# abiswas-odu/Disco

Measured on AMD Instinct MI355X. Metric: overlaps/sec (BuildGraph stage), 150 bp reads, higher is better.
Workload: dtype u64; 1 GPU; 50000000 x 150 bp synthetic reads, 30x of 50 x 5000000 bp uniform-random contigs, both strands, error-free, min-overlap 40 (k=39), transitive reduction on, seed 42; reads=50000000, read_len=150, min_overlap=40, parallelism=1 GPU, e_pre=903537181, e_out=45314794, n_contained=4685156, cap_bind_sites=0, asymmetric_pairs=0, probes=5550000000, kmer_hits=2220071992

## Files before the change

### disco_amd/build.py

```python
from __future__ import annotations

import os
import shutil
import subprocess

HERE = os.path.dirname(os.path.abspath(__file__))
ROOT = os.path.dirname(HERE)
LIB = os.path.join(HERE, "libdisco_hip.so")
BUILDG = os.path.join(HERE, "bin", "buildG")

HIP_SOURCES = [os.path.join(HERE, "csrc", "disco_hip.hip")]
HIP_DEPS = HIP_SOURCES + [os.path.join(HERE, "csrc", f) for f in sorted(f for f in os.listdir(os.path.join(HERE, "csrc")) if f.endswith(".h"))] + [
    os.path.join(ROOT, "include", "disco_hip.h"), os.path.join(ROOT, "include", "disco_hip_test.h"), os.path.join(ROOT, "include", "disco_hip_inspect.h")]
HOST_SOURCES = [os.path.join(HERE, "host", f) for f in ("buildg_main.cpp", "fastx.cpp", "writer.cpp", "parsimple.cpp")]


def _hipcc() -> str:
    for cand in (shutil.which("hipcc"), "/opt/rocm/bin/hipcc"):
        if cand and os.path.exists(cand):
            return cand
    raise RuntimeError("hipcc not found: the HIP extension cannot be built")


def _stale(target: str, deps) -> bool:
    if not os.path.exists(target):
        return True
    t = os.path.getmtime(target)
    return any(os.path.exists(d) and os.path.getmtime(d) > t for d in deps)


def vgpr_spills(remarks: str) -> dict:
    out, name = {}, None
    for line in remarks.splitlines():
        if "Function Name:" in line:
            name = line.split("Function Name:")[1].split("[")[0].strip()
        elif "VGPRs Spill:" in line and name:
            n = int(line.split("VGPRs Spill:")[1].split("[")[0])
            if n:
                out[name] = n
    return out


def build_lib(force: bool = False, verbose: bool = False) -> str:
    if force or _stale(LIB, HIP_DEPS):
        tmp = LIB + ".tmp"
        cmd = [_hipcc(), "--offload-arch=gfx950", "-O3", "-std=c++17", "-fPIC", "-shared", "-pthread", "-Rpass-analysis=kernel-resource-usage",
               "-o", tmp] + HIP_SOURCES + ["-L/opt/rocm/lib", "-lrccl", "-lrocprofiler-sdk-roctx", "-Wl,-rpath,/opt/rocm/lib"]
        if verbose:
            print(" ".join(cmd))
        r = subprocess.run(cmd, stdout=subprocess.PIPE, stderr=subprocess.PIPE, text=True)
        if r.returncode != 0:
            raise RuntimeError("hipcc failed:\n" + "\n".join(l for l in r.stderr.splitlines() if "-Rpass-analysis" not in l)[-4000:])
        spills = vgpr_spills(r.stderr)
        if spills and not os.environ.get("DISCO_ALLOW_SPILLS"):
            os.unlink(tmp)
            raise RuntimeError(f"kernels spill vector registers (cross-lane reads would return garbage): {spills}")
        os.replace(tmp, LIB)
    return LIB


def build_host(force: bool = False, verbose: bool = False) -> str:
    srcs = [s for s in HOST_SOURCES if os.path.exists(s)]
    if not srcs:
        return ""
    deps = srcs + [os.path.join(HERE, "host", f) for f in os.listdir(os.path.join(HERE, "host")) if f.endswith(".h")] + [LIB]
    if force or _stale(BUILDG, deps):
        os.makedirs(os.path.dirname(BUILDG), exist_ok=True)
        cmd = ["g++", "-O2", "-std=c++17", "-fopenmp", "-Wall", "-I", os.path.join(ROOT, "include"), "-o", BUILDG] + srcs + [
            "-L", HERE, "-ldisco_hip", "-lz", "-Wl,-rpath,$ORIGIN/..", "-Wl,-rpath," + HERE]
        if verbose:
            print(" ".join(cmd))
        subprocess.check_call(cmd)
    dump = os.path.join(HERE, "bin", "fastx_dump")
    dsrc = [os.path.join(HERE, "host", "fastx_dump.cpp"), os.path.join(HERE, "host", "fastx.cpp")]
    if force or _stale(dump, dsrc + [os.path.join(HERE, "host", "fastx.h")]):
        cmd = ["g++", "-O2", "-std=c++17", "-fopenmp", "-Wall", "-o", dump] + dsrc + ["-lz"]
        if verbose:
            print(" ".join(cmd))
        subprocess.check_call(cmd)
    ps = os.path.join(HERE, "bin", "parsimplify")
    psrc = [os.path.join(HERE, "host", f) for f in ("parsimplify_main.cpp", "parsimple.cpp", "fastx.cpp", "writer.cpp")]
    if force or _stale(ps, psrc + [os.path.join(HERE, "host", f) for f in ("parsimple.h", "writer.h", "fastx.h")]):
        cmd = ["g++", "-O2", "-std=c++17", "-fopenmp", "-Wall", "-I", os.path.join(ROOT, "include"), "-o", ps] + psrc + ["-lz"]
        if verbose:
            print(" ".join(cmd))
        subprocess.check_call(cmd)
    gen = os.path.join(HERE, "bin", "readgen")
    gsrc = [os.path.join(HERE, "host", "readgen_main.cpp"), os.path.join(HERE, "csrc", "readgen.h")]
    if force or _stale(gen, gsrc):
        cmd = ["g++", "-O2", "-std=c++17", "-Wall", "-o", gen, gsrc[0]]
        if verbose:
            print(" ".join(cmd))
        subprocess.check_call(cmd)
    chk = os.path.join(HERE, "bin", "inflate_check")
    csrc = [os.path.join(HERE, "host", "inflate_check.cpp"), os.path.join(HERE, "csrc", "disco_inflate.h")]
    if force or _stale(chk, csrc):
        cmd = ["g++", "-O2", "-std=c++17", "-Wall", "-o", chk, csrc[0]]
        if verbose:
            print(" ".join(cmd))
        subprocess.check_call(cmd)
    return BUILDG


def build_all(force: bool = False, verbose: bool = False):
    build_lib(force, verbose)
    build_host(force, verbose)


if __name__ == "__main__":
    build_all(force=True, verbose=True)
```

### disco_amd/buildgraph.py

```python
from __future__ import annotations

import ctypes as C
import os

import numpy as np

_HERE = os.path.dirname(os.path.abspath(__file__))
_LIBPATH = os.environ.get("DISCO_LIB") or os.path.join(_HERE, "libdisco_hip.so")
_lib = None


class DiscoError(RuntimeError):
    pass


class Params(C.Structure):
    _fields_ = [("min_overlap", C.c_uint32), ("max_edges_per_kmer", C.c_uint32), ("flags", C.c_uint32), ("max_substitutions", C.c_uint32)]


class GenSpecABI(C.Structure):
    _fields_ = [("seed", C.c_uint64), ("n_reads", C.c_uint64), ("contig_len", C.c_uint64), ("n_contigs", C.c_uint32),
                ("len_min", C.c_uint32), ("len_max", C.c_uint32), ("skew", C.c_uint32)]


# ... 47 lines not shown
    ("disco_fetch_contained_grouped", C.c_int64, [_P, _P, C.c_uint64]),
    ("disco_fetch_edges", C.c_int64, [_P, _P, C.c_uint64]),
    ("disco_fetch_edge_substitutions", C.c_int64, [_P, _P, C.c_uint64]),
    ("disco_get_counters", C.c_int, [_P, C.POINTER(Counters)]),
    ("disco_phase_ms", C.c_int, [_P, C.POINTER(C.c_float), C.c_int]),
    ("disco_memcpy_d2d", C.c_int, [_P, _P, _P, C.c_uint64]),
    ("disco_fetch_edge_files", C.c_int64, [_P, C.c_uint32, _P, C.c_uint64]),
    ("disco_partition_edges", C.c_int64, [_P, _P, C.c_uint64, C.c_uint64, C.c_uint32, _P]),
    ("disco_format_edges", C.c_int64, [_P, C.c_uint32, _P, _P, _P]),
    ("disco_fetch_edge_text", C.c_int, [_P, _P, C.c_uint64]),
    ("disco_write_edge_text", C.c_int, [_P, _P, C.c_uint32, C.c_uint32]),
    ("disco_start_contained_rows", C.c_int, [_P, C.c_int]),
    ("disco_contract_chains", C.c_int, [_P, C.c_uint32, C.POINTER(C.c_uint64), C.POINTER(C.c_uint64)]),
    ("disco_contract_chains_of", C.c_int, [_P, _P, C.c_uint64, C.c_uint32, C.POINTER(C.c_uint64), C.POINTER(C.c_uint64)]),
    ("disco_fetch_chains", C.c_int, [_P, _P, _P, _P]),
    ("disco_set_query_order", C.c_int, [_P, _P]),
    ("disco_get_query_order", C.c_int, [_P, C.POINTER(_P)]),
    ("disco_probe_run_words", C.c_int, [_P]),
    ("disco_measure_hbm", C.c_int, [_P, C.c_uint64, C.c_int, C.POINTER(C.c_double)]),
    ("disco_measure_gather", C.c_int, [_P, C.c_uint64, C.c_int, C.POINTER(C.c_double)]),
    ("disco_comm_unique_id", C.c_int, [_P, C.c_size_t]),
    ("disco_comm_init", C.c_int, [_P, _P, C.c_int, C.c_int]),
    ("disco_comm_init_local", C.c_int, [C.POINTER(_P), C.c_int]),
    ("disco_comm_rank", C.c_int, [_P]),
    ("disco_comm_world", C.c_int, [_P]),
    ("disco_comm_kind", C.c_char_p, [_P]),
    ("disco_dist_range", C.c_int, [_P, C.c_uint64, C.POINTER(C.c_uint64), C.POINTER(C.c_uint64)]),
    ("disco_dist_upload_reads", C.c_int, [_P, _P, C.c_uint32, _P, C.c_uint64]),
    ("disco_dist_generate_reads", C.c_int, [_P, C.POINTER(GenSpecABI)]),
    ("disco_dist_run_graph", C.c_int, [_P, C.c_uint32]),
    ("disco_dist_get_info", C.c_int, [_P, _P]),
    ("disco_ingest_fasta", C.c_int, [_P, C.POINTER(C.c_char_p), C.c_int, C.c_uint32, _P, _P]),
    ("disco_ingest_fetch", C.c_int, [_P, _P, _P]),
    ("disco_inflate_bgzf", C.c_int64, [_P, _P, C.c_uint64, _P, C.c_uint64]),
    ("disco_dist_ingest_fasta", C.c_int, [_P, C.POINTER(C.c_char_p), C.c_int, C.c_uint32, _P, _P]),
    ("disco_dist_ingest_fetch", C.c_int, [_P, _P, _P]),
    ("disco_inflate_bgzf_window", C.c_int64, [_P, _P, C.c_uint64, C.c_uint64, C.c_uint64, _P]),
    ("disco_format_contained", C.c_int64, [_P, C.c_uint32, _P, _P]),
    ("disco_fetch_contained_text", C.c_int, [_P, _P, C.c_uint64]),
    ("disco_write_contained_text", C.c_int, [_P, _P, C.c_uint32, C.c_uint32]),
]

ABI_VERSION = 2
FLAG_TWO_PASS_VERIFY = 1
XCHG = ("reads", "index_records", "index_shards", "contain", "row_requests", "row_data", "push", "adjacency", "twins", "queries", "hits", "keys", "reads_dealt", "contain_keys")
UNIQUE_ID_BYTES = 128
DIST_GATHER_READS = 1
DIST_KEEP_INDEX_PARTITIONED = 2


CHAIN_EDGE_DTYPE = np.dtype([("a", "<u8"), ("b", "<u8"), ("offset", "<u8"), ("orient", "<u4"), ("n_links", "<u4"), ("first_link", "<u8")])
CHAIN_LINK_DTYPE = np.dtype([("to", "<u4"), ("offset", "<u4"), ("orient", "<u4")])


class IngestFile(C.Structure):
    _fields_ = [("first_index", C.c_uint64), ("last_index", C.c_uint64), ("good", C.c_uint64), ("bad", C.c_uint64)]


class IngestInfo(C.Structure):
    _fields_ = [("n_reads", C.c_uint64), ("total_records", C.c_uint64), ("too_long", C.c_uint64), ("stride_words", C.c_uint32), ("shortest", C.c_uint32),
                ("longest", C.c_uint32), ("read_s", C.c_float), ("device_s", C.c_float)]


class DistIngestInfo(C.Structure):
    _fields_ = [("n_reads", C.c_uint64), ("total_records", C.c_uint64), ("too_long", C.c_uint64), ("stride_words", C.c_uint32), ("shortest", C.c_uint32),
                ("longest", C.c_uint32), ("world", C.c_uint32), ("share_lo", C.c_uint64), ("share_hi", C.c_uint64), ("share_reads", C.c_uint64),
                ("kept_reads", C.c_uint64), ("home_lo", C.c_uint64), ("home_hi", C.c_uint64), ("read_s", C.c_float), ("device_s", C.c_float)]


class DistInfo(C.Structure):
    _fields_ = [("world", C.c_uint32), ("rank", C.c_uint32), ("n_reads", C.c_uint64), ("own_lo", C.c_uint64), ("own_hi", C.c_uint64),
                ("n_contained", C.c_uint64), ("e_pre", C.c_uint64), ("e_out", C.c_uint64), ("e_out_local", C.c_uint64),
                ("n_contained_local", C.c_uint64), ("cap_bind_sites", C.c_uint64), ("asymmetric_pairs", C.c_uint64),
                ("dropped_hits", C.c_uint64), ("probes", C.c_uint64), ("kmer_hits", C.c_uint64), ("regime", C.c_uint32),
                ("tr_rounds", C.c_uint32), ("tr_deferred", C.c_uint64), ("bytes_sent", C.c_uint64 * len(XCHG)),
                ("ms", C.c_float * len(XCHG)), ("ms_total", C.c_float), ("kernel_ms", C.c_float), ("comm_ops", C.c_uint32),
                ("host_syncs", C.c_uint32), ("device_allocs", C.c_uint32), ("device_frees", C.c_uint32), ("arena_bytes", C.c_uint64),
                ("arena_peak", C.c_uint64), ("hbm_peak", C.c_uint64), ("own_reads", C.c_uint64), ("placement", C.c_uint32), ("reserved_", C.c_uint32)]

PHASES = ("index", "probe_kernel", "verify", "contain", "select", "csr", "twin", "trmark", "emit", "order")

INSPECT_ABI = [
    ("disco_fetch_order", C.c_int, [_P, _P, _P, C.c_uint64, C.POINTER(C.c_uint64), C.POINTER(C.c_int)]),
]
_inspect_bound = False


def _bind_inspect(L):
    global _inspect_bound
    if not _inspect_bound:
        for name, res, args in INSPECT_ABI:
            fn = getattr(L, name)
            fn.restype = res
            fn.argtypes = args
        _inspect_bound = True


def lib_path() -> str:
    return _LIBPATH


def load():
    global _lib
    if _lib is None:
        if not os.path.exists(_LIBPATH):
            raise DiscoError(f"{_LIBPATH} is missing: build it with `python -m disco_amd.build` (hipcc, gfx950). "
                             "There is no CPU fallback.")
        L = C.CDLL(_LIBPATH)
        L.disco_abi_version.restype = C.c_int
        if L.disco_abi_version() != ABI_VERSION:
            raise DiscoError(f"{_LIBPATH} speaks ABI version {L.disco_abi_version()}, this mirror was written against {ABI_VERSION}: rebuild "
                             "(`python -m disco_amd.build`)")
        for name, res, args in ABI:
            fn = getattr(L, name)
            fn.restype = res
            fn.argtypes = args
        _lib = L
    return _lib


class BuildGraph:

    def __init__(self, min_overlap: int = 40, device: int = 0, max_edges_per_kmer: int = 4, flags: int = 0, max_substitutions: int = 0):
        self.L = load()
        self.min_overlap = min_overlap
        self._h = _P()
        p = Params(min_overlap, max_edges_per_kmer, flags, max_substitutions)
        rc = self.L.disco_create(device, C.byref(p), C.byref(self._h))
        if rc != 0:
            raise DiscoError(f"disco_create failed ({rc}): {self.L.disco_last_error(None).decode()}")

    def _chk(self, rc):
        if rc < 0:
            raise DiscoError(f"libdisco_hip error {rc}: {self.L.disco_last_error(self._h).decode()}")
        return rc

    def close(self):
        if self._h:
            self.L.disco_destroy(self._h)
            self._h = _P()

    def __del__(self):
        try:
            self.close()
        except Exception:
            pass

    def __enter__(self):
        return self

    def __exit__(self, *a):
        self.close()

    def set_stream(self, stream_ptr: int | None):
        self._chk(self.L.disco_set_stream(self._h, _P(stream_ptr) if stream_ptr else None))

    def synchronize(self):
        self._chk(self.L.disco_synchronize(self._h))

    def upload_reads(self, packed: np.ndarray, lens: np.ndarray):
        packed = np.ascontiguousarray(packed, dtype=np.uint64)
        lens = np.ascontiguousarray(lens, dtype=np.uint16)
        assert packed.ndim == 2 and packed.shape[0] == lens.shape[0]
        self._keep = (packed, lens)
        self._chk(self.L.disco_upload_reads(self._h, packed.ctypes.data, packed.shape[1], lens.ctypes.data, packed.shape[0]))

# ... 142 lines not shown
        self._chk(self.L.disco_fetch_edge_text(self._h, buf.ctypes.data, nb))
        return buf[:nb].tobytes(), off

    def write_edge_text(self, fds, threads: int = 8):
        arr = (C.c_int * len(fds))(*fds)
        self._chk(self.L.disco_write_edge_text(self._h, arr, len(fds), threads))

    def format_contained(self, n_files: int = 1, file_index=None):
        off = np.zeros(n_files + 1, dtype=np.uint64)
        fi = None if file_index is None else np.ascontiguousarray(file_index, dtype=np.uint64)
        nb = self._chk(self.L.disco_format_contained(self._h, n_files, None if fi is None else fi.ctypes.data, off.ctypes.data))
        buf = np.empty(max(nb, 1), dtype=np.uint8)
        self._chk(self.L.disco_fetch_contained_text(self._h, buf.ctypes.data, nb))
        return buf[:nb].tobytes(), off

    def write_contained_text(self, fds, threads: int = 8):
        arr = (C.c_int * len(fds))(*fds)
        self._chk(self.L.disco_write_contained_text(self._h, arr, len(fds), threads))

    def start_contained_rows(self, grouped: bool = False):
        self._chk(self.L.disco_start_contained_rows(self._h, 1 if grouped else 0))

    def contract_chains(self, min_overlap_simplify: int = 0, edges=None):
        nc, nl = C.c_uint64(), C.c_uint64()
        if edges is None:
            self._chk(self.L.disco_contract_chains(self._h, min_overlap_simplify, C.byref(nc), C.byref(nl)))
            ne = int(self.L.disco_fetch_edges(self._h, None, 0))
        else:
            edges = np.ascontiguousarray(edges, dtype=EDGE_DTYPE)
            self._chk(self.L.disco_contract_chains_of(self._h, edges.ctypes.data, len(edges), min_overlap_simplify, C.byref(nc), C.byref(nl)))
            ne = len(edges)
        comp = np.zeros(nc.value, dtype=CHAIN_EDGE_DTYPE)
        links = np.zeros(nl.value, dtype=CHAIN_LINK_DTYPE)
        absorbed = np.zeros(ne, dtype=np.uint8)
        self._chk(self.L.disco_fetch_chains(self._h, comp.ctypes.data if len(comp) else None, links.ctypes.data if len(links) else None,
                                            absorbed.ctypes.data if ne else None))
        return comp, links, absorbed

    def fetch_edge_substitutions(self) -> np.ndarray:
        n = self._chk(self.L.disco_fetch_edge_substitutions(self._h, None, 0))
        out = np.zeros(n, dtype=np.uint16)
        if n:
            self._chk(self.L.disco_fetch_edge_substitutions(self._h, out.ctypes.data, n))
        return out

    def phase_ms(self) -> dict:
        a = (C.c_float * len(PHASES))()
        self._chk(self.L.disco_phase_ms(self._h, a, len(PHASES)))
        return {n: float(a[i]) for i, n in enumerate(PHASES)}

    def fetch_edge_files(self, n_files: int):
        n = int(self.L.disco_fetch_edges(self._h, None, 0))
        out = np.zeros(max(n, 1), dtype=np.uint16)
        self._chk(self.L.disco_fetch_edge_files(self._h, n_files, out.ctypes.data, n))
        return out[:n]

    def partition_edges(self, edges: np.ndarray, n_nodes: int, n_files: int):
        edges = np.ascontiguousarray(edges, dtype=EDGE_DTYPE)
        out = np.zeros(max(len(edges), 1), dtype=np.uint16)
        self._chk(self.L.disco_partition_edges(self._h, edges.ctypes.data, len(edges), n_nodes, n_files, out.ctypes.data))
        return out[:len(edges)]

    def get_query_order(self) -> int:
        out = _P()
        self._chk(self.L.disco_get_query_order(self._h, C.byref(out)))
        return out.value or 0

    def set_query_order(self, d_order_ptr: int):
        self._chk(self.L.disco_set_query_order(self._h, _P(d_order_ptr)))

    def probe_run_words(self) -> int:
        return int(self.L.disco_probe_run_words(self._h))

    def fetch_order(self):
        _bind_inspect(self.L)
        n, bits = C.c_uint64(0), C.c_int(0)
        one = np.zeros(1, dtype=np.uint64)
        rc = self.L.disco_fetch_order(self._h, one.ctypes.data, one.ctypes.data, 0, C.byref(n), C.byref(bits))
        if n.value == 0:
            self._chk(rc)
        order, keys = np.zeros(max(n.value, 1), dtype=np.uint64), np.zeros(max(n.value, 1), dtype=np.uint32)
        self._chk(self.L.disco_fetch_order(self._h, order.ctypes.data, keys.ctypes.data, len(order), C.byref(n), C.byref(bits)))
        return order[:n.value], keys[:n.value], bits.value

    def measure_hbm(self, nbytes: int = 4 << 30, reps: int = 5) -> float:
        out = C.c_double(0.0)
        self._chk(self.L.disco_measure_hbm(self._h, nbytes, reps, C.byref(out)))
        return out.value

    def measure_gather(self, nbytes: int = 3 << 30, reps: int = 3) -> float:
        out = C.c_double(0.0)
        self._chk(self.L.disco_measure_gather(self._h, nbytes, reps, C.byref(out)))
        return out.value

    def memcpy_d2d(self, dst_ptr: int, src_ptr: int, nbytes: int):
        self._chk(self.L.disco_memcpy_d2d(self._h, _P(dst_ptr), _P(src_ptr), nbytes))

    @staticmethod
    def comm_unique_id() -> bytes:
        buf = C.create_string_buffer(UNIQUE_ID_BYTES)
        rc = load().disco_comm_unique_id(buf, UNIQUE_ID_BYTES)
        if rc != 0:
            raise DiscoError(f"disco_comm_unique_id failed ({rc})")
        return buf.raw

    def comm_init(self, unique_id: bytes, world: int, rank: int):
        self._chk(self.L.disco_comm_init(self._h, C.c_char_p(unique_id), world, rank))

    @staticmethod
    def comm_init_local(graphs):
        arr = (_P * len(graphs))(*[g._h for g in graphs])
        rc = load().disco_comm_init_local(arr, len(graphs))
        if rc != 0:
            raise DiscoError(f"disco_comm_init_local failed ({rc})")

    @property
    def rank(self) -> int:
        return int(self.L.disco_comm_rank(self._h))

    @property
    def world(self) -> int:
        return int(self.L.disco_comm_world(self._h))

    @property
    def transport(self) -> str:
        return self.L.disco_comm_kind(self._h).decode()

    def dist_range(self, n_total: int):
        lo, hi = C.c_uint64(), C.c_uint64()
        self._chk(self.L.disco_dist_range(self._h, n_total, C.byref(lo), C.byref(hi)))
        return lo.value, hi.value

    def dist_upload_reads(self, packed_own: np.ndarray, lens_own: np.ndarray, n_total: int, stride_words: int | None = None):
        packed_own = np.ascontiguousarray(packed_own, dtype=np.uint64)
        lens_own = np.ascontiguousarray(lens_own, dtype=np.uint16)
        self._keep = (packed_own, lens_own)
        stride = int(stride_words if stride_words is not None else packed_own.shape[1])
        self._chk(self.L.disco_dist_upload_reads(self._h, packed_own.ctypes.data, stride, lens_own.ctypes.data, n_total))

    def dist_upload_ascii(self, reads):
        n = len(reads)
        lo, hi = self.dist_range(n)
        stride = int((max((len(r) for r in reads), default=1) + 31) // 32)
        packed = np.zeros((hi - lo, stride), dtype=np.uint64)
        lens = np.fromiter((len(r) for r in reads[lo:hi]), dtype=np.uint16, count=hi - lo)
        for i, r in enumerate(reads[lo:hi]):
            b = r.encode()
            if self.L.disco_pack_ascii(b, len(b), packed[i].ctypes.data) != 0:
                raise DiscoError(f"read {lo + i} contains a non-ACGT base")
        self.dist_upload_reads(packed, lens, n, stride)

    def dist_generate_reads(self, spec):
        s = GenSpecABI(spec.seed, spec.n_reads, spec.contig_len, spec.n_contigs, spec.len_min, spec.len_max, int(spec.skew_word if hasattr(spec, "skew_word") else getattr(spec, "skew", 0)))
        self._chk(self.L.disco_dist_generate_reads(self._h, C.byref(s)))

    def ingest_fasta(self, paths, threads: int = 16):
        arr = (C.c_char_p * len(paths))(*[os.fsencode(p) for p in paths])
        info, files = IngestInfo(), (IngestFile * len(paths))()
        rc = self.L.disco_ingest_fasta(self._h, arr, len(paths), threads, C.byref(info), files)
        if rc == -6:
            return None
        self._chk(rc)
        return ({n: getattr(info, n) for n, _ in IngestInfo._fields_}, [{n: getattr(f, n) for n, _ in IngestFile._fields_} for f in files])

    def inflate_bgzf(self, data: bytes):
        data = bytes(data)
# ... 110 lines not shown
```

### disco_amd/csrc/disco_chains.h

```cpp
#ifndef DISCO_CHAINS_H_
#define DISCO_CHAINS_H_

#include "disco_kernels.h"

#define CH_NIL 0xFFFFFFFFu

struct ChainView {
    const u64 *src, *ent;
    const u8 *valid;
    const u64 *pos;
    const u16 *len;
    u64 n_slots;
    u32 min_ovl;
};

__device__ __forceinline__ bool ch_kept(const ChainView &g, u64 s)
{
    if (!g.valid[s]) return false;
    return (u32)g.len[g.src[s]] - ADJ_OFF(g.ent[s]) >= g.min_ovl;
}
__device__ __forceinline__ u32 ch_src(const ChainView &g, u32 h) { return (h & 1) ? (u32)ADJ_DST(g.ent[h >> 1]) : (u32)g.src[h >> 1]; }
__device__ __forceinline__ u32 ch_dst(const ChainView &g, u32 h) { return (h & 1) ? (u32)g.src[h >> 1] : (u32)ADJ_DST(g.ent[h >> 1]); }
__device__ __forceinline__ u32 ch_twin(u32 o) { return ((o >> 1) ^ 1u) | (((o & 1u) ^ 1u) << 1); }
__device__ __forceinline__ u32 ch_orient(const ChainView &g, u32 h)
{
    const u32 o = ADJ_ORI(g.ent[h >> 1]);
    return (h & 1) ? ch_twin(o) : o;
}
__device__ __forceinline__ u32 ch_offset(const ChainView &g, u32 h)
{
    const u64 e = g.ent[h >> 1];
    return (h & 1) ? (u32)((int)ADJ_DLEN(e) + (int)ADJ_OFF(e) - (int)g.len[g.src[h >> 1]]) : ADJ_OFF(e);
}

__global__ void ch_degree_kernel(ChainView g, u32 *__restrict__ deg, u32 *__restrict__ he)
{
    u64 s = (u64)blockIdx.x * blockDim.x + threadIdx.x;
    for (; s < g.n_slots; s += (u64)gridDim.x * blockDim.x) {
        if (!ch_kept(g, s)) continue;
        const u32 a = (u32)g.src[s], b = (u32)ADJ_DST(g.ent[s]);
        const u32 ka = atomicAdd(&deg[a], 1u), kb = atomicAdd(&deg[b], 1u);
        if (ka < 2) he[2ull * a + ka] = (u32)(2 * s);
        if (kb < 2) he[2ull * b + kb] = (u32)(2 * s + 1);
    }
}

__global__ void ch_internal_kernel(ChainView g, const u32 *__restrict__ deg, const u32 *__restrict__ he, u64 n, u8 *__restrict__ internal)
{
    u64 v = (u64)blockIdx.x * blockDim.x + threadIdx.x;
    for (; v < n; v += (u64)gridDim.x * blockDim.x) {
        u8 in = 0;
        if (deg[v] == 2) {
            const u32 h0 = he[2 * v], h1 = he[2 * v + 1];
            if ((h0 >> 1) != (h1 >> 1) && ch_dst(g, h0) != (u32)v && ch_dst(g, h1) != (u32)v)
                in = (((ch_orient(g, h0) >> 1) & 1u) != ((ch_orient(g, h1) >> 1) & 1u)) ? 1 : 0;
        }
        internal[v] = in;
    }
}

struct ChRank {
    u32 nxt, cnt, last, pad;
    u64 sum;
};

__global__ void ch_init_kernel(ChainView g, const u8 *__restrict__ internal, const u32 *__restrict__ he, ChRank *__restrict__ r)
{
    u64 s = (u64)blockIdx.x * blockDim.x + threadIdx.x;
    for (; s < g.n_slots; s += (u64)gridDim.x * blockDim.x) {
        const bool kept = ch_kept(g, s);
        for (u32 d = 0; d < 2; d++) {
            const u32 h = (u32)(2 * s + d);
            ChRank x;
            x.nxt = CH_NIL;
            x.cnt = 1;
            x.last = h;
            x.pad = 0;
            x.sum = 0;
            if (kept) {
                const u32 v = ch_dst(g, h);
                x.sum = ch_offset(g, h);
                if (internal[v]) x.nxt = (he[2ull * v] == (h ^ 1u)) ? he[2ull * v + 1] : he[2ull * v];
            }
            r[h] = x;
        }
    }
}

__global__ void ch_jump_kernel(const ChRank *__restrict__ old, ChRank *__restrict__ fresh, u64 n_half, u32 *__restrict__ live)
{
    u64 h = (u64)blockIdx.x * blockDim.x + threadIdx.x;
    u32 mine = 0;
    for (; h < n_half; h += (u64)gridDim.x * blockDim.x) {
        ChRank x = old[h];
        if (x.nxt != CH_NIL) {
            const ChRank y = old[x.nxt];
            x.cnt += y.cnt;
            x.sum += y.sum;
            x.last = y.last;
            x.nxt = y.nxt;
            mine++;
        }
        fresh[h] = x;
    }
    if (mine) atomicAdd(live, mine);
}

__device__ __forceinline__ u64 ch_rankid(const ChainView &g, u32 h) { return 2 * g.pos[h >> 1] + (h & 1u); }

struct ChSlot {
    u32 head;
    u32 mine;
    u32 index;
    bool in_chain;
};
__device__ __forceinline__ ChSlot ch_slot(const ChainView &g, const u8 *internal, const ChRank *r, u64 s)
{
    ChSlot o;
    o.in_chain = false;
    o.head = o.mine = o.index = 0;
    if (!ch_kept(g, s)) return o;
    const u32 h0 = (u32)(2 * s), h1 = h0 + 1;
    if (!internal[ch_dst(g, h0)] && !internal[ch_dst(g, h1)]) return o;
    const ChRank r0 = r[h0], r1 = r[h1];
    if (r0.nxt != CH_NIL || r1.nxt != CH_NIL) return o;
    const u32 H0 = r1.last ^ 1u, T0 = r0.last;
    const bool dir0 = !(ch_rankid(g, H0) > ch_rankid(g, T0 ^ 1u));
    o.in_chain = true;
    o.head = dir0 ? H0 : (T0 ^ 1u);
    o.mine = dir0 ? h0 : h1;
    o.index = (dir0 ? r1.cnt : r0.cnt) - 1u;
    return o;
}

__global__ void ch_heads_kernel(ChainView g, const u8 *__restrict__ internal, const ChRank *__restrict__ r, u8 *__restrict__ is_head, u32 *__restrict__ links_of,
                                u8 *__restrict__ dead)
{
    u64 s = (u64)blockIdx.x * blockDim.x + threadIdx.x;
    for (; s < g.n_slots; s += (u64)gridDim.x * blockDim.x) {
        const ChSlot c = ch_slot(g, internal, r, s);
        const bool head = c.in_chain && c.index == 0;
        is_head[s] = head ? 1 : 0;
        links_of[s] = head ? r[c.head].cnt : 0u;
        if (c.in_chain) dead[g.pos[s]] = 1;
    }
}

struct ChainEdgeOut {
    u64 a, b, offset;
    u32 orient, n_links;
    u64 first_link;
};
struct ChainLinkOut {
    u32 to, offset, orient;
};

__global__ void ch_emit_kernel(ChainView g, const u8 *__restrict__ internal, const ChRank *__restrict__ r, const u64 *__restrict__ comp_id,
                               const u64 *__restrict__ link_start, ChainEdgeOut *__restrict__ comp, ChainLinkOut *__restrict__ links)
{
    u64 s = (u64)blockIdx.x * blockDim.x + threadIdx.x;
    for (; s < g.n_slots; s += (u64)gridDim.x * blockDim.x) {
        const ChSlot c = ch_slot(g, internal, r, s);
        if (!c.in_chain) continue;
        const u64 hs = c.head >> 1;
        const u64 first = link_start[hs];
        ChainLinkOut l;
        l.to = ch_dst(g, c.mine);
        l.offset = ch_offset(g, c.mine);
        l.orient = ch_orient(g, c.mine);
        links[first + c.index] = l;
        if (c.index == 0) {
            const ChRank rh = r[c.head];
            ChainEdgeOut e;
            e.a = ch_src(g, c.head);
            e.b = ch_dst(g, rh.last);
            e.offset = rh.sum;
            e.orient = (ch_orient(g, c.head) & 2u) | (ch_orient(g, rh.last) & 1u);
            e.n_links = rh.cnt;
            e.first_link = first;
            comp[comp_id[hs]] = e;
        }
    }
}

#endif
```

### disco_amd/csrc/disco_device.h

```cpp
#ifndef DISCO_DEVICE_H_
#define DISCO_DEVICE_H_

#include <hip/hip_runtime.h>
#include <stdint.h>

typedef unsigned long long u64;
typedef unsigned int u32;
typedef unsigned short u16;
typedef unsigned char u8;

#define DISCO_WAVE 64
#define DISCO_NOKEY 0x7FFFFFFFFFFFFFFFull

#define PAY_LEN(p) ((u32)((p)&0x7FFFu))
#define PAY_SUFFIX(p) ((u32)(((p) >> 15) & 1u))
#define PAY_REV(p) ((u32)(((p) >> 16) & 1u))
#define PAY_T(p) ((u32)(((p) >> 17) & 0x3Fu))
#define PAY_ID(p) (((p) >> 23) & 0x7FFFFFFFull)
#define PAY_FP(p) ((u32)((p) >> 54))
#define KEY_FP(key) ((u32)((key)&0x3FFu))
#define PAY_MAKE(key, id, t, rev, suf, len) \
    (((u64)KEY_FP(key) << 54) | ((u64)(id) << 23) | ((u64)(t) << 17) | ((u64)(rev) << 16) | ((u64)(suf) << 15) | (u64)(len))

#define HIT_MAKE(j, id, suf, rev, len) (((u64)(j) << 48) | ((u64)(id) << 17) | ((u64)(suf) << 16) | ((u64)(rev) << 15) | (u64)(len))
#define HIT_J(h) ((u32)((h) >> 48) & 0x7FFFu)
#define HIT_ID(h) (((h) >> 17) & 0x7FFFFFFFull)
#define HIT_SUFFIX(h) ((u32)(((h) >> 16) & 1u))
#define HIT_REV(h) ((u32)(((h) >> 15) & 1u))
#define HIT_LEN(h) ((u32)((h)&0x7FFFu))
#define HIT_HIDDEN_BIT (1ull << 63)
#define HIT_HIDDEN(h) ((u32)((h) >> 63))
#define HIT_SORT_KEY(h) (((h) << 1) | ((h) >> 63))
#define HIT_FROM_SORT_KEY(x) (((x) >> 1) | ((x) << 63))

#define ADJ_MAKE(off, dst, o, dlen) (((u64)(off) << 49) | ((u64)(dst) << 18) | ((u64)(o) << 16) | (u64)(dlen))
#define ADJ_OFF(e) ((u32)((e) >> 49) & 0x7FFFu)
#define ADJ_DST(e) (((e) >> 18) & 0x7FFFFFFFull)
#define ADJ_ORI(e) ((u32)(((e) >> 16) & 3u))
#define ADJ_DLEN(e) ((u32)((e)&0x7FFFu))

#define CKEY_MAKE(a, j, suf, rev) (((u64)(a) << 17) | ((u64)(j) << 2) | ((u64)(suf) << 1) | (u64)(rev))
#define CKEY_SUPER(c) ((c) >> 17)
#define CKEY_J(c) ((u32)((c) >> 2) & 0x7FFFu)
#define CKEY_SUFFIX(c) ((u32)(((c) >> 1) & 1u))
#define CKEY_REV(c) ((u32)((c)&1u))

__host__ __device__ __forceinline__ u32 disco_hit_type(u32 is_suffix, u32 rev)
{
    return is_suffix ? (rev ? 2u : 1u) : (rev ? 3u : 0u);
}

__host__ __device__ __forceinline__ void disco_map_type(u32 type, u32 len1, u32 k, u32 j, u32 *orient, u32 *offset)
{
    switch (type) {
    case 0: *orient = 3; *offset = j; break;
    case 1: *orient = 0; *offset = len1 - (k + j); break;
    case 2: *orient = 2; *offset = j; break;
    default: *orient = 1; *offset = len1 - (k + j); break;
    }
}

__host__ __device__ __forceinline__ void disco_map_hit(u32 is_suffix, u32 rev, u32 len1, u32 k, u32 j, u32 *orient, u32 *offset)
{
    const u32 same = (is_suffix ^ rev ^ 1u) & 1u;
    *orient = (same << 1) | ((is_suffix ^ 1u) & 1u);
    *offset = same ? j : len1 - (k + j);
}

__host__ __device__ __forceinline__ u32 disco_twin_orient(u32 o) { return o == 0 ? 3u : (o == 3 ? 0u : o); }

__host__ __device__ __forceinline__ u64 disco_hash64(u64 x)
{
    x ^= x >> 33;
    x *= 0xFF51AFD7ED558CCDull;
    x ^= x >> 33;
    x *= 0xC4CEB9FE1A85EC53ull;
    x ^= x >> 33;
    return x;
}

#if defined(__HIPCC__)

__device__ __forceinline__ u64 lane_mask_lt()
{
    u32 l = __lane_id();
    return l ? (~0ull >> (64 - l)) : 0ull;
}
__device__ __forceinline__ u32 rank_below(u64 mask) { return __builtin_amdgcn_mbcnt_hi((u32)(mask >> 32), __builtin_amdgcn_mbcnt_lo((u32)mask, 0u)); }

__device__ __forceinline__ u32 row_prefix_min(u32 x)
{
    u32 y;
// ... 269 lines not shown
```

### disco_amd/csrc/disco_hip.hip

```cpp
#include <hip/hip_runtime.h>
#include <rocprofiler-sdk-roctx/roctx.h>

#include <algorithm>
#include <atomic>
#include <chrono>
#include <cstdarg>
#include <cstdio>
#include <cstdlib>
#include <cstring>
#include <fcntl.h>
#include <sys/mman.h>
#include <sys/stat.h>
#include <unistd.h>
#include <string>
#include <memory>
#include <thread>
#include <map>
#include <mutex>
#include <vector>

#include "../../include/disco_hip.h"
#include "../../include/disco_hip_test.h"
#include "../../include/disco_hip_inspect.h"
#include "disco_kernels.h"
// ... 172 lines not shown
    DevBuf<u32> d_big_cnt;
    u32 *d_n_big = nullptr;
    DevBuf<u32> d_runs;
    u64 runs_lo = 0, runs_n = 0;
    int runs_lpr = 0;
    DevBuf<u64> d_slow_list;
    u32 *d_n_slow = nullptr;
    u64 big_rows = 0, slow_rows = 0;
    const u64 *d_order = nullptr;
    const u64 *d_order_used = nullptr;
    bool order_external = false;
    DevBuf<u32> d_ocnt, d_okey, d_oslot;
    DevBuf<u64> d_order_own;
    bool order_counted = false;
    bool order_items = false;
    int order_id_bits = 0;
    bool es_big_counted = false, tr_big_counted = false;
    bool contained_count_pending = false;
    bool order_ready = false;
    hipStream_t aux_stream = nullptr;
    hipEvent_t ev_crows = nullptr;
    DevBuf<u32> d_cpos, d_crow_id;
    DevBuf<u64> d_crow_key;
    DevBuf<u64> d_tile2;
    u64 *d_total2 = nullptr;
    void *h_crows = nullptr;
    DevBuf<u32> d_crow_len;
    u64 crows_hcap = 0, crows_n = 0;
    bool crows_pending = false;
    bool crows_in_ring = false;
    DevBuf<u32> d_cgrp_cur, d_cgrp_id;
    DevBuf<u64> d_cgrp_key, d_cgrp_big;
    u64 h_cgrp_big = 0;
    bool cgrp_pending = false;
    DevBuf<u32> d_fetch_src;
    DevBuf<u64> d_fetch_ent;
    DevBuf<u32> d_rec_of_read;
    std::vector<u64> ingest_id_base, ingest_rec_base;
    u64 ingest_n = 0;
    void *h_ring = nullptr;
    std::vector<u64> text_off;
    DevBuf<char> d_ctext;
    std::vector<u64> ctext_off;
    u64 ctext_bytes = 0;
    DevBuf<u8> d_ingest;
    std::thread hits_prealloc;
    DevBuf<u64> prealloc;
    u64 prealloc_asked = 0;
    size_t ring_half = 0;
    hipEvent_t ev_ring[2] = {nullptr, nullptr};
    hipStream_t copy_stream = nullptr;
    hipEvent_t ev_copied[3] = {nullptr, nullptr, nullptr}, ev_unpacked[3] = {nullptr, nullptr, nullptr};
    bool index_counted = false;
    u64 order_counted_lo = 0, order_counted_hi = 0;
    int order_counted_bits = 0;
    DevBuf<u32> d_asked;
    u64 order_q_lo = 0, order_q_hi = 0;
    DevBuf<ulonglong2> d_meta_ord;
    u64 dropped_local = 0;
    ProbeRare h_probe_rare;
    DevBuf<ProbeRare> d_probe_rare;
    u32 max_len = 0, min_len = 0;
    bool two_pass_last = false;
    bool contained_done = false;

    DevBuf<u8> d_contained;
    DevBuf<u64> d_cbits;
    DevBuf<u64> d_dropbits;
    DevBuf<u64> d_drop_node, d_drop_key;
    u64 n_drop_items = 0;
    u64 drop_lo = 0, drop_hi = 0;
    u64 n_contained = 0;

    DevBuf<u64> d_adj_ref;
    u64 *d_adj = nullptr;
    DevBuf<u64> d_adj_own;
    DevBuf<u64> d_adj_spare;
    DevBuf<u64> d_start_tmp;
    u64 adj_total = 0;
    bool flags_pending = false;
    bool adj_imported = false;
    u64 adj_span = 0;
    bool half_complete = false;
    DevBuf<u32> d_extra_cnt;
    DevBuf<u64> d_extra_node, d_extra_key;
    u32 *d_n_extra = nullptr;
    u32 n_extra = 0;
    u64 asym_local = 0;
    u64 dropped = 0;

    DevBuf<u64> d_half;
    DevBuf<u32> d_hcnt;
    bool use_half = false;
    DevBuf<u64> d_wide;
    DevBuf<u32> d_n_wide;
    u32 n_wide = 0;
    DevBuf<u8> d_out_valid;
    DevBuf<u64> d_out_pos;
    u64 *h_stage = nullptr;
    hipEvent_t ev_stage[2] = {nullptr, nullptr};
    DevBuf<ChainEdgeOut> d_ch_comp;
    DevBuf<ChainLinkOut> d_ch_links;
    DevBuf<u8> d_ch_dead;
    u64 ch_comp_n = 0, ch_links_n = 0, ch_edges_n = 0;
    bool ch_ready = false;
    DevBuf<char> d_text;
    u64 text_bytes = 0;
    DevBuf<u64> d_out_src, d_out_ent;
    u64 out_used = 0;
    u64 n_out = 0;

    hipEvent_t ev0[DISCO_PH_SLOTS] = {nullptr}, ev1[DISCO_PH_SLOTS] = {nullptr};
    bool ev_pending[DISCO_PH_SLOTS] = {false};
    float ph_ms[DISCO_PH_SLOTS] = {0};

    int phase = 0;

    DiscoComm *comm = nullptr;
    DiscoComm *comm_bulk = nullptr;
    hipStream_t bulk_stream = nullptr;
    hipEvent_t ev_bulk = nullptr;
    bool wait_bulk_before_verify = false;
    u64 per = 0;
    u64 n_alloc = 0;
    bool part_index = false;
    u64 part_blo = 0, part_bhi = 0, part_nrec = 0;
    DevBuf<u64> d_pq_start;
    bool dist_reads = false;
    bool dist_active = false;
    DevBuf<u64> d_route;
    DevBuf<ulonglong2> d_x16a, d_x16b;
    DevBuf<u32> d_req_flat, d_req_s, d_req_r;
    DevBuf<u32> d_rdeg_s, d_rdeg_r, d_rdata_s;
    DevBuf<u64> d_rpos;
    DevBuf<u32> d_nadj32_own;
    u64 nadj_used = 0;
    DevBuf<u32> d_deg_tmp;
    DevBuf<u64> d_list_n;
    DevBuf<u64> d_dense;
    ulonglong2 *d_push_r = nullptr;
    u64 n_push_r = 0;
    bool loci = false;
    bool runs_by_pos = false;
    DevBuf<u8> d_otab;
    DevBuf<u32> d_own_ids;
    u64 n_own = 0;
    u64 home_lo = 0, home_hi = 0;
    u64 home_probes = 0;
    DevBuf<u64> d_cb_all;
    hipEvent_t ev_keys = nullptr, ev_keys_go = nullptr;
    bool keys_pending = false;
    disco_dist_info dinfo{};
    bool time_exchanges = false;
    unsigned dist_passes = 0;
};

static int fail(disco_ctx *c, int code, const char *fmt, ...)
{
    char buf[512];
    va_list ap;
    va_start(ap, fmt);
    vsnprintf(buf, sizeof buf, fmt, ap);
    va_end(ap);
    if (c) c->err = buf;
    else g_create_error = buf;
    return code;
}

#define HIPCHK(c, call)                                                                                          \
    do {                                                                                                         \
        hipError_t e_ = (call);                                                                                  \
        if (e_ != hipSuccess) return fail((c), e_ == hipErrorOutOfMemory ? DISCO_E_NOMEM : DISCO_E_HIP, "%s failed: %s (%s:%d)", #call, hipGetErrorString(e_), __FILE__, __LINE__); \
    } while (0)

#define CHK(expr)                    \
    do {                             \
        int rc_ = (expr);            \
        if (rc_ != DISCO_OK) return rc_; \
    } while (0)

static void ph_begin(disco_ctx *c, int id)
{
    (void)hipEventRecord(c->ev0[id], c->stream);
}
static void ph_end(disco_ctx *c, int id)
{
    (void)hipEventRecord(c->ev1[id], c->stream);
    c->ev_pending[id] = true;
}
static void ph_collect(disco_ctx *c)
{
    for (int i = 0; i < DISCO_PH_SLOTS; i++)
// ... 795 lines not shown
static ProbeFn probe_mode_pick(bool ldsrow, bool row17, bool longk, bool long_class)
{
    if constexpr (PMODE != 0) {
        if (long_class) return longk ? probe_kernel<PMODE, false, false, true, true> : row17 ? probe_kernel<PMODE, false, true, false, true> : probe_kernel<PMODE, false, false, false, true>;
    }
    if constexpr (PMODE != 2) {
        if (!ldsrow) return longk ? probe_kernel<PMODE, false, false, true> : row17 ? probe_kernel<PMODE, false, true> : probe_kernel<PMODE, false, false>;
    }
    return longk ? probe_kernel<PMODE, true, false, true> : row17 ? probe_kernel<PMODE, true, true> : probe_kernel<PMODE, true, false>;
}
static ProbeKernel probe_pick(const disco_ctx *c, int mode, bool use_runs)
{
    const bool ldsrow = c->S <= PROBE_ACAP;
    const bool row17 = c->k - view(c).m == 16 && !getenv("DISCO_NO_ROW17");
    const bool longk = c->k > 64;
    const bool long_class = c->two_class && c->S_ext > PROBE_ACAP;
    ProbeKernel k;
    if (mode == 0 && use_runs) k.runs = c->runs_lpr == 16 ? probe_runs_kernel<16> : probe_runs_kernel<32>;
    else if (mode == 0) k.plain = probe_mode_pick<0>(ldsrow, row17, longk, long_class);
    else if (mode == 1) k.plain = probe_mode_pick<1>(ldsrow, row17, longk, long_class);
    else k.plain = probe_mode_pick<2>(ldsrow, row17, longk, long_class);
    return k;
}

typedef void (*VerifyFn)(VerifyArgs);
template <bool INEXACT>
static VerifyFn verify_rows_pick(int S, bool short_rows)
{
    if (S == VERIFY_SW) return short_rows ? verify_kernel<5, 0, INEXACT> : verify_kernel<8, 0, INEXACT>;
    return S == 16 ? verify_kernel<16, 0, INEXACT> : S == 24 ? verify_kernel<24, 0, INEXACT> : S == 32 ? verify_kernel<32, 0, INEXACT> : verify_kernel<0, 0, INEXACT>;
}
template <int MODE>
static VerifyFn verify_pass_pick(bool flat, bool short_rows)
{
    if (flat) return short_rows ? verify_flat_kernel<5, MODE> : verify_flat_kernel<8, MODE>;
    return short_rows ? verify_kernel<5, MODE> : verify_kernel<8, MODE>;
}
static VerifyFn verify_pick(const disco_ctx *c, int mode, bool flat, bool inexact, int *cap)
{
    const bool short_rows = c->max_len <= 160;
    *cap = 32;
    if (mode == 1) return verify_pass_pick<1>(flat, short_rows);
    if (mode == 2) return verify_pass_pick<2>(flat, short_rows);
    if (inexact) return verify_rows_pick<true>(c->S, short_rows);
    if (!flat) return verify_rows_pick<false>(c->S, short_rows);
    const char *vce = getenv("DISCO_VERIFY_CACHE");
    const bool vcache = vce ? atoi(vce) != 0 : true;
    if (!vcache) return short_rows ? verify_flat_kernel<5> : verify_flat_kernel<8>;
    if (short_rows) *cap = 16;
    return short_rows ? verify_flat_kernel<5, 0, true> : verify_flat_kernel<8, 0, true>;
}
static void verify_launch(disco_ctx *c, const VerifyArgs &va, u64 nq, int mode, bool flat, bool inexact)
{
    int cap = 0;
    const VerifyFn k = verify_pick(c, mode, flat, inexact, &cap);
    wq_launch(c, k, nq, "DISCO_VERIFY_WAVES", cap, va);
}

typedef void (*EdgeSelFn)(EdgeSelArgs);
#ifndef SEL_SMALL_ROWS
#define SEL_SMALL_ROWS 4
#define SEL_SMALL_NB 3
#endif
static EdgeSelFn edge_select_pick(bool big, bool flat, bool small)
{
    if (big) return edge_select_kernel<true>;
    if (flat) return small ? edge_select_flat_kernel<SEL_SMALL_ROWS, SEL_SMALL_NB, true> : edge_select_flat_kernel<4, 4>;
    return edge_select_kernel<false>;
}

typedef void (*TrFn)(TrArgs);
static TrFn tr_pick(bool big, bool defer, bool small, bool lists)
{
    if (big) return defer ? transitive_mark_kernel<true, true> : transitive_mark_kernel<true, false>;
    if (defer) return lists ? transitive_mark_kernel<false, true, TR_CAP_SMALL, true> : transitive_mark_kernel<false, true, TR_CAP_SMALL>;
#if defined(TR_EXP_DEFER_SINGLE)
    if (small) return transitive_mark_kernel<false, true, TR_CAP_SMALL>;
#else
    if (small) return lists ? transitive_mark_kernel<false, false, TR_CAP_SMALL, true> : transitive_mark_kernel<false, false, TR_CAP_SMALL>;
#endif
    return transitive_mark_kernel<false, false>;
}

static int tr_args_begin(disco_ctx *c, TrArgs *a)
{
    a->v = view(c);
    a->ref = c->d_adj_ref;
    a->adj = c->d_adj;
    a->big_list = c->d_big_list;
    a->n_big = c->d_n_big;
    a->big_cap = c->d_big_list.cap;
    a->scratch = nullptr;
    a->hcap = 0;
    a->half = nullptr;
    a->hcnt = nullptr;
    if (c->use_half) {
        CHK(ensure(c, c->d_half, c->n * HALF_CAP));
        CHK(ensure(c, c->d_hcnt, c->n));
        HIPCHK(c, hipMemsetAsync(c->d_hcnt, 0, std::max<u64>(c->n, 1) * sizeof(u32), c->stream));
        CHK(ensure(c, c->d_wide, std::min<u64>(c->n, c->n / 32 + 4096)));
        CHK(ensure(c, c->d_n_wide, 1));
        HIPCHK(c, hipMemsetAsync(c->d_n_wide, 0, sizeof(u32), c->stream));
        a->half = c->d_half;
        a->hcnt = c->d_hcnt;
    }
    a->wide_list = c->d_wide;
    a->n_wide = c->d_n_wide;
    a->wide_cap = c->d_wide.cap;
    return DISCO_OK;
}

static int tr_big_nodes(disco_ctx *c, TrArgs *a, u32 n_big, bool defer, const char *what)
{
    CHK(zero_counter(c, CTR_MAX_DEG));
    hipLaunchKernelGGL(list_max_degree_kernel, dim3(flat_grid(c, n_big)), dim3(256), 0, c->stream, c->d_big_list, (u64)n_big, c->d_adj_ref, c->d_ctr + CTR_MAX_DEG);
    HIPCHK(c, hipGetLastError());
    CHK(read_counters(c));
    const u64 maxd = c->h_ctr[CTR_MAX_DEG];
    u64 hcap = 64;
    while (hcap < 2 * maxd) hcap <<= 1;
    const int g2 = (int)std::min<u64>(n_big, (u64)c->n_cu * 8);
    const u64 per = hcap * 8 + hcap * 4 + hcap;
    DevBuf<u8> scratch;
    CHK(ensure(c, scratch, (u64)g2 * per));
    a->scratch = (u64 *)scratch.p;
    a->hcap = hcap;
    a->adj = c->d_adj;
    HIPCHK(c, hipMemsetAsync(c->d_wq, 0, sizeof(u64) * WQ_WORDS, c->stream));
    hipLaunchKernelGGL(tr_pick(true, defer, false, false), dim3(g2), dim3(64), 0, c->stream, *a);
    const hipError_t e = hipGetLastError();
    const int rc = read_counters(c);
    release(c, scratch);
    if (e != hipSuccess) return fail(c, DISCO_E_HIP, "transitive_mark_kernel (%s): %s", what, hipGetErrorString(e));
    return rc;
}

static int dist_mark_contained(disco_ctx *c);
static int dist_partitioned_probe(disco_ctx *c);

extern "C" {

int disco_abi_version(void) { return DISCO_ABI_VERSION; }

int disco_create(int device, const disco_params *p, disco_ctx **out)
{
    if (!p || !out) return fail(nullptr, DISCO_E_ARG, "disco_create: null argument");
    if (p->min_overlap < 2 || p->min_overlap - 1 > DISCO_MAX_K)
        return fail(nullptr, DISCO_E_UNSUPPORTED, "disco_create: min_overlap %u unsupported (k = min_overlap-1 must be in [1,%d])", p->min_overlap, DISCO_MAX_K);
    int ndev = 0;
    hipError_t e = hipGetDeviceCount(&ndev);
    if (e != hipSuccess || ndev <= 0) return fail(nullptr, DISCO_E_HIP, "disco_create: no HIP device (%s)", hipGetErrorString(e));
    if (device < 0 || device >= ndev) return fail(nullptr, DISCO_E_ARG, "disco_create: device %d out of range (%d devices)", device, ndev);
    disco_ctx *c = new (std::nothrow) disco_ctx();
    if (!c) return fail(nullptr, DISCO_E_NOMEM, "disco_create: out of host memory");
    c->device = device;
    c->prm = *p;
    if (c->prm.max_edges_per_kmer == 0) c->prm.max_edges_per_kmer = 4;
    if (c->prm.max_substitutions > 32767) c->prm.max_substitutions = 32767;
    c->k = (int)p->min_overlap - 1;
#define CREATE_CHK(call)                                                                              \
    do {                                                                                              \
        hipError_t e2 = (call);                                                                       \
        if (e2 != hipSuccess) {                                                                       \
            int rc = fail(nullptr, DISCO_E_HIP, "disco_create: %s failed: %s", #call, hipGetErrorString(e2)); \
            delete c;                                                                                 \
            return rc;                                                                                \
        }                                                                                             \
    } while (0)
    CREATE_CHK(hipSetDevice(device));
    hipDeviceProp_t prop;
    CREATE_CHK(hipGetDeviceProperties(&prop, device));
    c->n_cu = prop.multiProcessorCount > 0 ? prop.multiProcessorCount : 256;
    CREATE_CHK(hipStreamCreateWithFlags(&c->own_stream, hipStreamNonBlocking));
    c->stream = c->own_stream;
    CREATE_CHK(hipMalloc((void **)&c->d_ctr, sizeof(u64) * CTR_COUNT));
    CREATE_CHK(hipMemset(c->d_ctr, 0, sizeof(u64) * CTR_COUNT));
    CREATE_CHK(hipMalloc((void **)&c->d_total, sizeof(u64)));
    CREATE_CHK(hipMalloc((void **)&c->d_wq, sizeof(u64) * WQ_WORDS));
    CREATE_CHK(hipMalloc((void **)&c->d_bump, sizeof(u64)));
    CREATE_CHK(hipMalloc((void **)&c->d_n_big, sizeof(u32)));
    CREATE_CHK(hipMalloc((void **)&c->d_n_slow, sizeof(u32)));
    CREATE_CHK(hipMalloc((void **)&c->d_n_extra, sizeof(u32)));
    for (int i = 0; i < DISCO_PH_SLOTS; i++) {
        CREATE_CHK(hipEventCreate(&c->ev0[i]));
        CREATE_CHK(hipEventCreate(&c->ev1[i]));
    }
#undef CREATE_CHK
    *out = c;
// ... 1866 lines not shown
    if (c->phase < 5) return fail(c, DISCO_E_STATE, "disco_adjacency_size: select edges first");
    *n_entries = c->adj_total;
    return DISCO_OK;
}

int disco_export_adjacency(disco_ctx *c, void *d_deg_u32, void *d_entries_u64)
{
    if (!c || !d_deg_u32) return DISCO_E_ARG;
    if (c->phase < 5 || c->adj_imported) return fail(c, DISCO_E_STATE, "disco_export_adjacency: needs the locally selected edges");
    HIPCHK(c, hipSetDevice(c->device));
    const u64 nq = c->q_hi - c->q_lo;
    ph_begin(c, DISCO_PH_CSR);
    if (nq) hipLaunchKernelGGL(deg_from_ref_kernel, dim3(flat_grid(c, nq)), dim3(256), 0, c->stream, c->d_adj_ref, c->q_lo, c->q_hi, (u32 *)d_deg_u32);
    HIPCHK(c, hipGetLastError());
    if (nq && c->adj_total && d_entries_u64) {
        CHK(ensure(c, c->d_start_tmp, c->n + 1));
        u64 *start = c->d_start_tmp;
        u64 total = 0;
        int rc = scan_exclusive<u32, u64>(c, (const u32 *)d_deg_u32, nq, start, true, &total);
        if (rc == DISCO_OK && total != c->adj_total) rc = fail(c, DISCO_E_STATE, "disco_export_adjacency: degree sum %llu != %llu", (unsigned long long)total, (unsigned long long)c->adj_total);
        if (rc == DISCO_OK) hipLaunchKernelGGL(rows_gather_kernel, dim3(wave_grid(c, nq, 16)), dim3(64), 0, c->stream, c->d_adj, c->d_adj_ref, c->q_lo, c->q_hi, start, (u64 *)d_entries_u64,
                                              (c->phase == 5 && c->prm.max_substitutions != 0) ? 0ull : (u64)ADJ_FLAG);
        hipError_t e = hipStreamSynchronize(c->stream);
        CHK(rc);
        if (e != hipSuccess) return fail(c, DISCO_E_HIP, "disco_export_adjacency: %s", hipGetErrorString(e));
    }
    ph_end(c, DISCO_PH_CSR);
    HIPCHK(c, hipStreamSynchronize(c->stream));
    ph_collect(c);
    return DISCO_OK;
}





int disco_import_adjacency(disco_ctx *c, const void *d_deg_u32_all, const void *d_entries_u64_all, uint64_t n_entries_all)
{
    if (!c || !d_deg_u32_all) return DISCO_E_ARG;
    if (c->phase < 5) return fail(c, DISCO_E_STATE, "disco_import_adjacency: select edges first");
    HIPCHK(c, hipSetDevice(c->device));
    CHK(ensure(c, c->d_start_tmp, c->n + 1));
    u64 *start = c->d_start_tmp;
    u64 total = 0;
    CHK((scan_exclusive<u32, u64>(c, (const u32 *)d_deg_u32_all, c->n, start, true, &total)));
    if (total != n_entries_all)
        return fail(c, DISCO_E_ARG, "disco_import_adjacency: degrees sum to %llu but %llu entries were passed", (unsigned long long)total, (unsigned long long)n_entries_all);
    CHK(ensure(c, c->d_adj_own, total));
    c->d_adj = c->d_adj_own;
    c->adj_total = total;
    if (total) HIPCHK(c, hipMemcpyAsync(c->d_adj, d_entries_u64_all, total * 8, hipMemcpyDeviceToDevice, c->stream));
    if (c->n) hipLaunchKernelGGL(ref_from_start_kernel, dim3(flat_grid(c, c->n)), dim3(256), 0, c->stream, start, (const u32 *)d_deg_u32_all, c->n, c->d_adj_ref);
    HIPCHK(c, hipGetLastError());
    HIPCHK(c, hipStreamSynchronize(c->stream));
    c->adj_imported = true;
    c->tr_big_counted = false;
    c->adj_span = total;
    c->half_complete = false;
    c->phase = 5;
    return DISCO_OK;
}




int disco_transitive_mark(disco_ctx *c)
{
    DISCO_TRACE("disco_transitive_mark");
    if (!c) return DISCO_E_ARG;
    if (c->phase < 6) return fail(c, DISCO_E_STATE, "disco_transitive_mark: build edges first");
    HIPCHK(c, hipSetDevice(c->device));
    const u64 nq = c->q_hi - c->q_lo;
    HIPCHK(c, hipMemsetAsync(c->d_n_big, 0, sizeof(u32), c->stream));
    CHK(zero_counter(c, CTR_OVERFLOW));
    const bool counted_nodes = c->tr_big_counted && c->q_lo == 0 && c->q_hi == c->n && !getenv("DISCO_COUNT_BIG_ROWS");
    const bool tr_small = env_int("DISCO_TR_SMALL", counted_nodes && c->h_ctr[CTR_TR_MID] * 100 <= nq ? 1 : 0) != 0 && counted_nodes;
    if (counted_nodes) {
        const u64 need = c->h_ctr[tr_small ? CTR_TR_MID : CTR_TR_BIG] + 1024;
        if (need > 0xFFFFFFFFull) return fail(c, DISCO_E_CAPACITY, "more than 2^32 big nodes");
        CHK(grow_big_lists(c, need));
    } else
        CHK(ensure_big_cap(c, nullptr, c->d_adj_ref, TR_CAP));
    c->use_half = !getenv("DISCO_NO_HALF");
    TrArgs a;
    CHK(tr_args_begin(c, &a));
    a.order = (c->d_order_used && c->order_q_lo == c->q_lo && c->order_q_hi == c->q_hi && !c->adj_imported && !getenv("DISCO_TR_NO_ORDER")) ? c->d_order_used : nullptr;
    a.all_flags = (c->adj_imported || !c->use_half || c->q_lo != 0 || c->q_hi != c->n) ? 1u : 0u;
    ph_begin(c, DISCO_PH_TRMARK);
    const bool lists = a.half && a.hcnt && !a.all_flags;
    if (nq) wq_launch(c, tr_pick(false, false, tr_small, lists), nq, "DISCO_TR_WAVES", 32, a);
    ph_end(c, DISCO_PH_TRMARK);
    HIPCHK(c, hipGetLastError());
    u32 n_big = 0;
    HIPCHK(c, hipMemcpyAsync(&n_big, c->d_n_big, sizeof(u32), hipMemcpyDeviceToHost, c->stream));
    c->n_wide = 0;
    if (c->use_half) HIPCHK(c, hipMemcpyAsync(&c->n_wide, c->d_n_wide, sizeof(u32), hipMemcpyDeviceToHost, c->stream));
    CHK(read_counters(c));
    ph_collect(c);
    if (c->h_ctr[CTR_OVERFLOW]) return fail(c, DISCO_E_CAPACITY, "transitive marking: big-node list overflow (%u nodes)", n_big);
    if (n_big) {
        CHK(tr_big_nodes(c, &a, n_big, false, "big nodes"));
        if (c->h_ctr[CTR_OVERFLOW]) return fail(c, DISCO_E_CAPACITY, "transitive marking (big nodes): list overflow");
    }
    if (n_big && c->use_half) HIPCHK(c, hipMemcpy(&c->n_wide, c->d_n_wide, sizeof(u32), hipMemcpyDeviceToHost));
    c->flags_pending = false;
    c->phase = 7;
    return DISCO_OK;
}


int disco_emit_edges(disco_ctx *c, uint64_t *n_out)
{
    DISCO_TRACE("disco_emit_edges");
    if (!c) return DISCO_E_ARG;
    if (c->phase < 7) return fail(c, DISCO_E_STATE, "disco_emit_edges: run disco_transitive_mark first");
    HIPCHK(c, hipSetDevice(c->device));
    const u64 nq = c->q_hi - c->q_lo;
    ph_begin(c, DISCO_PH_EMIT);
    const int grid = wq_grid(c, emit_kernel, nq, "DISCO_EMIT_WAVES");
    const u64 n_push = c->dist_active ? c->n_push_r : 0;
    const int grid_push = (int)std::max<u64>(std::min<u64>((n_push + 63) / 64, (u64)c->n_cu * 16), 1);
    const u64 nwaves = (u64)grid * 2 + (n_push ? (u64)grid_push : 0);
    u64 want = std::max<u64>(2 * nq, 1024) + n_push + nwaves * EMIT_CHUNK;
    for (int attempt = 0; attempt < 6; attempt++) {
        CHK(ensure_group(c, want, want, c->d_out_src, c->d_out_ent));
        HIPCHK(c, hipMemsetAsync(c->d_bump, 0, sizeof(u64), c->stream));
        const bool half_emit = c->use_half && c->half_complete;
        if (half_emit && nq) {
            EmitHalfArgs h;
            h.v = view(c);
            h.ref = c->d_adj_ref;
            h.adj = c->d_adj;
            h.half = c->d_half;
            h.hcnt = c->d_hcnt;
            h.out_src = c->d_out_src;
            h.out_ent = c->d_out_ent;
            h.out_cap = c->d_out_src.cap;
            h.bump = c->d_bump;
            h.local_only = c->dist_active ? 1u : 0u;
            h.own = own_set(c);
            h.order = nullptr;
            const int gh = wq_grid(c, emit_half_kernel, (nq + 63) / 64, "DISCO_EMIT_WAVES");
            hipLaunchKernelGGL(emit_half_kernel, dim3(gh), dim3(64), 0, c->stream, h);
        }
        EmitArgs a;
        a.v = view(c);
        a.ref = c->d_adj_ref;
        a.adj = c->d_adj;
        a.hcnt = half_emit ? c->d_hcnt : nullptr;
        a.half = half_emit ? c->d_half : nullptr;
        const bool listed = half_emit && c->n_wide <= c->d_wide.cap;
        a.list = listed ? c->d_wide : nullptr;
        a.n_list = listed ? c->n_wide : 0;
        a.out_src = c->d_out_src;
        a.out_ent = c->d_out_ent;
        a.out_cap = c->d_out_src.cap;
        a.bump = c->d_bump;
        a.local_only = c->dist_active ? 1u : 0u;
        a.own = own_set(c);
        HIPCHK(c, hipMemsetAsync(c->d_wq, 0, sizeof(u64) * WQ_WORDS, c->stream));
        if (nq && !(listed && c->n_wide == 0)) hipLaunchKernelGGL(emit_kernel, dim3(grid), dim3(64), 0, c->stream, a);
        if (n_push) {
            EmitRecvArgs pr;
            pr.items = c->d_push_r;
            pr.n_items = n_push;
            pr.ref = c->d_adj_ref;
            pr.adj = c->d_adj;
            pr.half = c->d_half;
            pr.hcnt = c->d_hcnt;
            pr.out_src = c->d_out_src;
            pr.out_ent = c->d_out_ent;
            pr.out_cap = c->d_out_src.cap;
            pr.bump = c->d_bump;
            pr.wq = c->d_wq;
            HIPCHK(c, hipMemsetAsync(c->d_wq, 0, sizeof(u64) * WQ_WORDS, c->stream));
            hipLaunchKernelGGL(emit_push_recv_kernel, dim3(grid_push), dim3(64), 0, c->stream, pr);
        }
        HIPCHK(c, hipGetLastError());
        u64 used = 0;
        HIPCHK(c, hipMemcpyAsync(&used, c->d_bump, sizeof(u64), hipMemcpyDeviceToHost, c->stream));
        HIPCHK(c, hipStreamSynchronize(c->stream));
        if (used <= c->d_out_src.cap) {
            c->out_used = used;
            break;
        }
        want = used + used / 8 + nwaves * EMIT_CHUNK;
        if (attempt == 5) return fail(c, DISCO_E_CAPACITY, "disco_emit_edges: output buffer could not be sized");
    }
    u64 total = 0;
    if (c->out_used) {
        if (c->out_used > c->d_out_valid.cap || c->out_used + 1 > c->d_out_pos.cap) {
            release(c, c->d_out_valid);
            release(c, c->d_out_pos);
            int rc = ensure(c, c->d_out_valid, c->d_out_src.cap);
            if (rc == DISCO_OK) rc = ensure(c, c->d_out_pos, c->d_out_src.cap + 1);
            if (rc != DISCO_OK) {
                release(c, c->d_out_valid);
                return rc;
            }
        }
        hipLaunchKernelGGL(emit_valid_kernel, dim3(flat_grid(c, c->out_used)), dim3(256), 0, c->stream, c->d_out_src, c->out_used, c->d_out_valid);
        CHK((scan_exclusive<u8, u64>(c, c->d_out_valid, c->out_used, c->d_out_pos, true, nullptr)));
        HIPCHK(c, hipMemcpyAsync(&total, c->d_total, sizeof(u64), hipMemcpyDeviceToHost, c->stream));
    }
    ph_end(c, DISCO_PH_EMIT);
    HIPCHK(c, hipStreamSynchronize(c->stream));
    ph_collect(c);
    c->n_out = total;
    if (n_out) *n_out = total;
    c->phase = 8;
    return DISCO_OK;
}

int disco_transitive_reduce(disco_ctx *c, uint64_t *n_out)
{
    CHK(disco_transitive_mark(c));
    return disco_emit_edges(c, n_out);
}

int disco_run_graph(disco_ctx *c)
{
    DISCO_TRACE("disco_run_graph");
    const bool verbose = getenv("DISCO_VERBOSE") != nullptr;
    auto now = [] { return std::chrono::steady_clock::now(); };
    auto ms = [](std::chrono::steady_clock::time_point a, std::chrono::steady_clock::time_point b) { return std::chrono::duration<double, std::milli>(b - a).count(); };
    auto t0 = now();
    CHK(disco_build_index(c));
    auto t1 = now();
    CHK(disco_probe(c));
    auto t2 = now();
    {
        CHK(ensure(c, c->d_contained, c->n_alloc));
        CHK(ensure(c, c->d_cbits, c->n_alloc / 64 + 1));
        CHK(zero_counter(c, CTR_N_CONTAINED));
        ph_begin(c, DISCO_PH_CONTAIN);
        if (c->n) hipLaunchKernelGGL(contain_flags_kernel, dim3(flat_grid(c, c->n)), dim3(256), 0, c->stream, c->d_best, c->n, c->d_contained, c->d_cbits, c->d_ctr);
        HIPCHK(c, hipGetLastError());
        ph_end(c, DISCO_PH_CONTAIN);
        c->contained_count_pending = true;
        c->phase = 4;
        c->crows_pending = c->cgrp_pending = false;
    }
    auto t3 = now();
    CHK(disco_build_edges(c, nullptr));
    auto t4 = now();
    int rc = disco_transitive_reduce(c, nullptr);
    auto t5 = now();
    if (verbose)
        fprintf(stderr, "[disco] host wall ms: index %.1f probe %.1f contain %.1f edges %.1f reduce %.1f\n", ms(t0, t1), ms(t1, t2), ms(t2, t3), ms(t3, t4), ms(t4, t5));
    return rc;
}

static int ensure_host_len(disco_ctx *c)
{
    std::lock_guard<std::mutex> lk(c->h_len_mu);
    if (c->h_len_ok && c->h_len.size() == c->n) return DISCO_OK;
    c->h_len.resize(c->n);
    if (c->n) HIPCHK(c, hipMemcpy(c->h_len.data(), c->d_len, c->n * 2, hipMemcpyDeviceToHost));
    c->h_len_ok = true;
    return DISCO_OK;
}

int64_t disco_fetch_contained(disco_ctx *c, disco_contained_row *out, uint64_t cap)
{
    DISCO_TRACE("disco_fetch_contained");
    if (!c) return DISCO_E_ARG;
    if (c->phase < 4) return fail(c, DISCO_E_STATE, "disco_fetch_contained: run disco_mark_contained first");
    HIPCHK(c, hipSetDevice(c->device));
    const u64 nc = c->n_contained;
    if (!out) return (int64_t)nc;
    if (cap < nc) return fail(c, DISCO_E_ARG, "disco_fetch_contained: need room for %llu rows", (unsigned long long)nc);
    if (nc == 0) return 0;
    auto decode = [&](auto id_of, const u64 *keys_h, const u32 *lens_h) {
// ... 10 lines not shown
                r.len2 = lens_h ? (lens_h[i] & 0xFFFFu) : hlen[r.contained];
                r.len1 = lens_h ? (lens_h[i] >> 16) : hlen[r.super];
                u32 orient, off;
                disco_map_type(r.type, r.len1, kk, r.j, &orient, &off);
                r.orient = orient;
                r.start = off;
            }
        });
    };
    CHK(start_contained_rows(c, false));
    if (c->crows_pending && c->crows_n == nc) {
        HIPCHK(c, hipEventSynchronize(c->ev_crows));
        const u64 *hkey = (const u64 *)c->h_crows;
        const u32 *hid = (const u32 *)(hkey + c->crows_hcap);
        decode([hid](u64 i) { return (u64)hid[i]; }, hkey, hid + c->crows_hcap);
        return (int64_t)nc;
    }
    CHK(ensure_host_len(c));
    CHK(settle_keys(c));
    DevBuf<u64> pos, ids, keys;
    std::vector<u64> hid(nc), hkey(nc);
    auto gather = [&]() -> int {
        CHK(ensure(c, pos, c->n + 1));
        CHK(ensure(c, ids, nc));
        CHK(ensure(c, keys, nc));
        CHK((scan_exclusive<u8, u64>(c, c->d_contained, c->n, pos, false, nullptr)));
        hipLaunchKernelGGL(contain_rows_kernel, dim3(flat_grid(c, c->n)), dim3(256), 0, c->stream, c->d_best, c->d_contained, pos, c->n, ids, keys);
        HIPCHK(c, hipMemcpyAsync(hid.data(), ids, nc * 8, hipMemcpyDeviceToHost, c->stream));
        HIPCHK(c, hipMemcpyAsync(hkey.data(), keys, nc * 8, hipMemcpyDeviceToHost, c->stream));
        HIPCHK(c, hipStreamSynchronize(c->stream));
        return DISCO_OK;
    };
    const int grc = gather();
    release(c, pos);
    release(c, ids);
    release(c, keys);
    CHK(grc);
    for (u64 i = 0; i < nc; i++)
        if (CKEY_SUPER(hkey[i]) >= c->n || hid[i] >= c->n)
            return fail(c, DISCO_E_STATE, "disco_fetch_contained: row %llu of %llu: read %llu has the key %llx (no containing read)", (unsigned long long)i, (unsigned long long)nc,
                        (unsigned long long)hid[i], (unsigned long long)hkey[i]);
    decode([&hid](u64 i) { return hid[i]; }, hkey.data(), nullptr);
    return (int64_t)nc;
}

int64_t disco_fetch_contained_grouped(disco_ctx *c, disco_contained_row *out, uint64_t cap)
{
    DISCO_TRACE("disco_fetch_contained_grouped");
    if (!c) return DISCO_E_ARG;
    if (c->phase < 4) return fail(c, DISCO_E_STATE, "disco_fetch_contained_grouped: run disco_mark_contained first");
    HIPCHK(c, hipSetDevice(c->device));
    const u64 nc = c->n_contained;
    if (!out) return (int64_t)nc;
    if (cap < nc) return fail(c, DISCO_E_ARG, "disco_fetch_contained_grouped: need room for %llu rows", (unsigned long long)nc);
    if (nc == 0) return 0;
    if (getenv("DISCO_NO_GROUPED_ROWS")) return fail(c, DISCO_E_UNSUPPORTED, "disco_fetch_contained_grouped: switched off (DISCO_NO_GROUPED_ROWS)");
    CHK(start_contained_rows(c, true));
    if (!(c->cgrp_pending && c->crows_pending && c->crows_n == nc))
        return fail(c, DISCO_E_UNSUPPORTED, "disco_fetch_contained_grouped: the rows were not grouped on the device (sort what disco_fetch_contained returns)");
    HIPCHK(c, hipStreamSynchronize(c->aux_stream));
    if (c->h_cgrp_big) return fail(c, DISCO_E_UNSUPPORTED, "disco_fetch_contained_grouped: a containing read has more than %d rows (sort what disco_fetch_contained returns)", CROW_GROUP_MAX);
    const u64 *hkey = (const u64 *)((const char *)c->h_crows + c->crows_hcap * 16);
    const u32 *hid = (const u32 *)(hkey + c->crows_hcap), *hln = hid + c->crows_hcap;
    const u32 kk = (u32)c->k;
    parallel_for(nc, [&, kk, hkey, hid, hln](u64 b, u64 e_) {
        for (u64 i = b; i < e_; i++) {
            const u64 key = hkey[i];
            disco_contained_row &r = out[i];
            r.contained = hid[i];
            r.super = CKEY_SUPER(key);
            r.j = CKEY_J(key);
            r.type = disco_hit_type(CKEY_SUFFIX(key), CKEY_REV(key));
            r.len2 = hln[i] & 0xFFFFu;
            r.len1 = hln[i] >> 16;
            u32 orient, off;
            disco_map_type(r.type, r.len1, kk, r.j, &orient, &off);
            r.orient = orient;
            r.start = off;
        }
    });
    return (int64_t)nc;
}

int64_t disco_fetch_edges(disco_ctx *c, disco_edge *out, uint64_t cap)
{
    DISCO_TRACE("disco_fetch_edges");
    if (!c) return DISCO_E_ARG;
    if (c->phase < 8) return fail(c, DISCO_E_STATE, "disco_fetch_edges: run disco_transitive_reduce first");
    HIPCHK(c, hipSetDevice(c->device));
    const u64 ne = c->n_out;
    if (!out) return (int64_t)ne;
    if (cap < ne) return fail(c, DISCO_E_ARG, "disco_fetch_edges: need room for %llu edges", (unsigned long long)ne);
    if (ne == 0) return 0;
    CHK(ensure_host_len(c));
    CHK(ensure_group(c, ne, ne + ne / 8 + 1024, c->d_fetch_src, c->d_fetch_ent));
    u32 *csrc = c->d_fetch_src;
    u64 *cent = c->d_fetch_ent;
    hipLaunchKernelGGL(emit_compact32_kernel, dim3(flat_grid(c, c->out_used)), dim3(256), 0, c->stream, c->d_out_src, c->d_out_ent, c->d_out_valid, c->d_out_pos, c->out_used, csrc, cent);
    const u64 CHUNK = 1ull << 22;
    if (!c->h_stage) {
        if (hipHostMalloc((void **)&c->h_stage, 4 * CHUNK * sizeof(u64)) != hipSuccess) c->h_stage = nullptr;
        for (int i = 0; i < 2 && c->h_stage; i++)
            if (hipEventCreateWithFlags(&c->ev_stage[i], hipEventDisableTiming) != hipSuccess) {
                (void)hipHostFree(c->h_stage);
                c->h_stage = nullptr;
            }
    }
    const u16 *hlen = c->h_len.data();
    auto convert = [&](const u32 *hsp, const u64 *hep, u64 base, u64 cnt) {
        parallel_for(cnt, [&, hlen, hsp, hep, base](u64 b, u64 e_) {
            for (u64 i = b; i < e_; i++) {
                disco_edge &e = out[base + i];
                e.src = hsp[i];
                e.dst = ADJ_DST(hep[i]);
                e.orient = ADJ_ORI(hep[i]);
                e.offset = ADJ_OFF(hep[i]);
                e.len_src = hlen[e.src];
                e.len_dst = ADJ_DLEN(hep[i]);
            }
        });
    };
    bool ok = true;
    if (c->h_stage) {
        const u64 nch = (ne + CHUNK - 1) / CHUNK;
        auto half_ent = [&](u64 k) { return c->h_stage + (k & 1) * 2 * CHUNK; };
        auto half_src = [&](u64 k) { return (u32 *)(c->h_stage + (k & 1) * 2 * CHUNK + CHUNK); };
        auto issue = [&](u64 k) {
            const u64 cnt = std::min(CHUNK, ne - k * CHUNK);
            ok = ok && hipMemcpyAsync(half_src(k), csrc + k * CHUNK, cnt * 4, hipMemcpyDeviceToHost, c->stream) == hipSuccess &&
                 hipMemcpyAsync(half_ent(k), cent + k * CHUNK, cnt * 8, hipMemcpyDeviceToHost, c->stream) == hipSuccess &&
                 hipEventRecord(c->ev_stage[k & 1], c->stream) == hipSuccess;
        };
        issue(0);
        for (u64 k = 0; k < nch && ok; k++) {
            ok = hipEventSynchronize(c->ev_stage[k & 1]) == hipSuccess;
            if (k + 1 < nch) issue(k + 1);
            if (ok) convert(half_src(k), half_ent(k), k * CHUNK, std::min(CHUNK, ne - k * CHUNK));
        }
        ok = (hipStreamSynchronize(c->stream) == hipSuccess) && ok;
    } else {
        std::unique_ptr<u32[]> hs(new u32[ne]);
        std::unique_ptr<u64[]> he(new u64[ne]);
        ok = hipMemcpyAsync(hs.get(), csrc, ne * 4, hipMemcpyDeviceToHost, c->stream) == hipSuccess &&
             hipMemcpyAsync(he.get(), cent, ne * 8, hipMemcpyDeviceToHost, c->stream) == hipSuccess && hipStreamSynchronize(c->stream) == hipSuccess;
        if (ok) convert(hs.get(), he.get(), 0, ne);
    }
    if (!ok) return fail(c, DISCO_E_HIP, "disco_fetch_edges: copy failed");
    return (int64_t)ne;
}

int64_t disco_fetch_edge_substitutions(disco_ctx *c, uint16_t *out, uint64_t cap)
{
    if (!c) return DISCO_E_ARG;
    if (c->phase < 8) return fail(c, DISCO_E_STATE, "disco_fetch_edge_substitutions: run disco_transitive_reduce first");
    HIPCHK(c, hipSetDevice(c->device));
    const u64 ne = c->n_out;
    if (!out) return (int64_t)ne;
    if (cap < ne) return fail(c, DISCO_E_ARG, "disco_fetch_edge_substitutions: need room for %llu edges", (unsigned long long)ne);
    if (ne == 0) return 0;
    if (c->prm.max_substitutions == 0) {
        memset(out, 0, ne * sizeof(uint16_t));
        return (int64_t)ne;
    }
    DevBuf<u16> subs;
    CHK(ensure(c, subs, ne));
    hipLaunchKernelGGL(edge_subs_kernel, dim3(flat_grid(c, c->out_used)), dim3(256), 0, c->stream, c->d_out_src, c->d_out_ent, c->d_out_valid, c->d_out_pos,
                       c->out_used, c->d_reads, c->d_len, c->S, subs);
    hipError_t e1 = hipMemcpyAsync(out, subs, ne * sizeof(u16), hipMemcpyDeviceToHost, c->stream);
    hipError_t e2 = hipStreamSynchronize(c->stream);
    release(c, subs);
    if (e1 != hipSuccess || e2 != hipSuccess) return fail(c, DISCO_E_HIP, "disco_fetch_edge_substitutions: copy failed");
    return (int64_t)ne;
}

static int64_t partition_edges(disco_ctx *c, const u64 *d_src, const u64 *d_ent, const u8 *d_valid, const u64 *d_pos, u64 n_slots, u64 ne, u64 n,
                               uint32_t n_files, uint16_t *out)
{
    DISCO_TRACE("partition_edges");
    DevBuf<u32> parent, cnt, d_nlist;
    DevBuf<u16> cfile, efile;
    DevBuf<u64> list;
    const u32 list_cap = n_files * 64 + 64;
    int rc = DISCO_OK;
    auto cleanup = [&]() {
        release(c, parent);
        release(c, cnt);
        release(c, cfile);
        release(c, efile);
        release(c, list);
        release(c, d_nlist);
    };
#define PART_CHK(x)            \
    do {                       \
        rc = (x);              \
        if (rc != DISCO_OK) {  \
            cleanup();         \
            return rc;         \
        }                      \
    } while (0)
    PART_CHK(ensure(c, parent, n));
    PART_CHK(ensure(c, cnt, n));
    PART_CHK(ensure(c, cfile, n));
    PART_CHK(ensure(c, efile, ne));
    PART_CHK(ensure(c, list, list_cap));
    PART_CHK(ensure(c, d_nlist, 1));
    hipLaunchKernelGGL(uf_init_kernel, dim3(flat_grid(c, n)), dim3(256), 0, c->stream, parent, n);
    hipLaunchKernelGGL(uf_hook_kernel, dim3(flat_grid(c, n_slots)), dim3(256), 0, c->stream, d_src, d_ent, d_valid, n_slots, parent);
    hipLaunchKernelGGL(uf_compress_kernel, dim3(flat_grid(c, n)), dim3(256), 0, c->stream, parent, n);
    (void)hipMemsetAsync(cnt, 0, n * sizeof(u32), c->stream);
    (void)hipMemsetAsync(cfile, 0xFF, n * sizeof(u16), c->stream);
    (void)hipMemsetAsync(d_nlist, 0, sizeof(u32), c->stream);
    hipLaunchKernelGGL(uf_count_kernel, dim3(flat_grid(c, n_slots)), dim3(256), 0, c->stream, d_src, d_valid, n_slots, parent, cnt);
    const u32 thr = (u32)std::max<u64>(ne / ((u64)n_files * 64), 1);
    hipLaunchKernelGGL(uf_big_kernel, dim3(flat_grid(c, n)), dim3(256), 0, c->stream, cnt, n, thr, list, d_nlist, list_cap);
    u32 n_list = 0;
    std::vector<u64> hl(list_cap);
    if (hipMemcpyAsync(&n_list, d_nlist, sizeof(u32), hipMemcpyDeviceToHost, c->stream) != hipSuccess ||
        hipMemcpyAsync(hl.data(), list, list_cap * sizeof(u64), hipMemcpyDeviceToHost, c->stream) != hipSuccess ||
        hipStreamSynchronize(c->stream) != hipSuccess) {
        cleanup();
        return fail(c, DISCO_E_HIP, "edge partition: %s", hipGetErrorString(hipGetLastError()));
    }
    n_list = std::min(n_list, list_cap);
    hl.resize(n_list);
    std::sort(hl.begin(), hl.end(), [](u64 a, u64 b) { return (u32)a != (u32)b ? (u32)a > (u32)b : a < b; });
    std::vector<u64> load(n_files, 0);
    for (u64 &e : hl) {
        const u32 f = (u32)(std::min_element(load.begin(), load.end()) - load.begin());
        load[f] += (u32)e;
        e = (e & 0xFFFFFFFF00000000ull) | f;
    }
    if (n_list) {
        if (hipMemcpyAsync(list, hl.data(), n_list * sizeof(u64), hipMemcpyHostToDevice, c->stream) != hipSuccess) {
            cleanup();
            return fail(c, DISCO_E_HIP, "edge partition: upload failed");
        }
        hipLaunchKernelGGL(uf_assign_kernel, dim3((n_list + 255) / 256), dim3(256), 0, c->stream, list, n_list, cfile);
    }
    hipLaunchKernelGGL(uf_edge_file_kernel, dim3(flat_grid(c, n_slots)), dim3(256), 0, c->stream, d_src, d_valid, d_pos, n_slots, parent, cfile, n_files, efile);
    hipError_t e1 = hipMemcpyAsync(out, efile, ne * sizeof(u16), hipMemcpyDeviceToHost, c->stream);
    hipError_t e2 = hipStreamSynchronize(c->stream);
    cleanup();
#undef PART_CHK
    if (e1 != hipSuccess || e2 != hipSuccess) return fail(c, DISCO_E_HIP, "edge partition: copy failed");
    return (int64_t)ne;
}

int64_t disco_fetch_edge_files(disco_ctx *c, uint32_t n_files, uint16_t *out, uint64_t cap)
{
    DISCO_TRACE("disco_fetch_edge_files");
    if (!c || !out || n_files == 0) return DISCO_E_ARG;
    if (n_files > 0xFFFEu) return fail(c, DISCO_E_ARG, "disco_fetch_edge_files: at most 65534 files (%u asked for)", n_files);
    if (c->phase < 8) return fail(c, DISCO_E_STATE, "disco_fetch_edge_files: run disco_transitive_reduce first");
    HIPCHK(c, hipSetDevice(c->device));
    const u64 ne = c->n_out;
    if (cap < ne) return fail(c, DISCO_E_ARG, "disco_fetch_edge_files: need room for %llu edges", (unsigned long long)ne);
    if (ne == 0) return 0;
    return partition_edges(c, c->d_out_src, c->d_out_ent, c->d_out_valid, c->d_out_pos, c->out_used, ne, c->n, n_files, out);
}

int64_t disco_partition_edges(disco_ctx *c, const disco_edge *edges, uint64_t n_edges, uint64_t n_nodes, uint32_t n_files, uint16_t *out)
{
    if (!c || !out || n_files == 0 || (n_edges && !edges)) return DISCO_E_ARG;
    if (n_files > 0xFFFEu) return fail(c, DISCO_E_ARG, "disco_partition_edges: at most 65534 files (%u asked for)", n_files);
    if (n_nodes >= (1ull << 31)) return fail(c, DISCO_E_UNSUPPORTED, "disco_partition_edges: more than 2^31 nodes");
    HIPCHK(c, hipSetDevice(c->device));
    if (n_edges == 0) return 0;
    DevBuf<u64> d_src, d_ent, d_pos;
    DevBuf<u8> d_valid;
    std::unique_ptr<u64[]> hs(new u64[n_edges]), he(new u64[n_edges]);
    parallel_for(n_edges, [&](u64 b, u64 e_) {
        for (u64 i = b; i < e_; i++) {
            hs[i] = edges[i].src;
            he[i] = ADJ_MAKE(0u, edges[i].dst, 0u, 0u);
        }
    });
    int rc = DISCO_OK;
    int64_t res = 0;
    do {
        if ((rc = ensure(c, d_src, n_edges)) != DISCO_OK) break;
        if ((rc = ensure(c, d_ent, n_edges)) != DISCO_OK) break;
        if ((rc = ensure(c, d_pos, n_edges)) != DISCO_OK) break;
        if ((rc = ensure(c, d_valid, n_edges)) != DISCO_OK) break;
        if (hipMemcpyAsync(d_src, hs.get(), n_edges * 8, hipMemcpyHostToDevice, c->stream) != hipSuccess ||
            hipMemcpyAsync(d_ent, he.get(), n_edges * 8, hipMemcpyHostToDevice, c->stream) != hipSuccess ||
            hipMemsetAsync(d_valid, 1, n_edges, c->stream) != hipSuccess) {
            rc = fail(c, DISCO_E_HIP, "disco_partition_edges: upload failed");
            break;
        }
        hipLaunchKernelGGL(iota_u64_kernel, dim3(flat_grid(c, n_edges)), dim3(256), 0, c->stream, d_pos, n_edges);
        res = partition_edges(c, d_src, d_ent, d_valid, d_pos, n_edges, n_edges, n_nodes, n_files, out);
    } while (0);
    release(c, d_src);
    release(c, d_ent);
    release(c, d_pos);
    release(c, d_valid);
    return rc != DISCO_OK ? rc : res;
}

int64_t disco_format_edges(disco_ctx *c, uint32_t n_files, const uint16_t *edge_file, const uint64_t *file_index, uint64_t *file_offsets)
{
    DISCO_TRACE("disco_format_edges");
    if (!c || !file_offsets || n_files == 0) return DISCO_E_ARG;
    if (c->phase < 8) return fail(c, DISCO_E_STATE, "disco_format_edges: run disco_transitive_reduce first");
    if (n_files > 256) return fail(c, DISCO_E_UNSUPPORTED, "disco_format_edges: more than 256 files (one placement pass per file)");
    if (c->prm.max_substitutions) return fail(c, DISCO_E_UNSUPPORTED, "disco_format_edges: the substitutions column is written by the host writer");
    HIPCHK(c, hipSetDevice(c->device));
    const u64 ne = c->n_out;
    for (uint32_t f = 0; f <= n_files; f++) file_offsets[f] = 0;
    c->text_bytes = 0;
    if (ne == 0) return 0;
    if (!edge_file && n_files > 1) return fail(c, DISCO_E_ARG, "disco_format_edges: the file of every edge is needed for more than one file");
    TextView g;
    g.src = c->d_out_src;
    g.ent = c->d_out_ent;
    g.valid = c->d_out_valid;
    g.pos = c->d_out_pos;
    g.len = c->d_len;
    g.n_slots = c->out_used;
    DevBuf<u64> d_findex, within, place;
    DevBuf<u8> bytes, sel;
    DevBuf<u16> efile;
    auto body = [&]() -> int {
        if (file_index) {
            CHK(ensure(c, d_findex, c->n));
            HIPCHK(c, hipMemcpyAsync(d_findex, file_index, c->n * 8, hipMemcpyHostToDevice, c->stream));
        }
        g.file_index = d_findex;
        CHK(ensure(c, bytes, ne));
        CHK(ensure(c, sel, ne));
        CHK(ensure(c, efile, ne));
        CHK(ensure(c, within, ne + 1));
        CHK(ensure(c, place, ne));
        if (edge_file) HIPCHK(c, hipMemcpyAsync(efile, edge_file, ne * sizeof(u16), hipMemcpyHostToDevice, c->stream));
        else HIPCHK(c, hipMemsetAsync(efile, 0, ne * sizeof(u16), c->stream));
        hipLaunchKernelGGL(text_measure_kernel, dim3(flat_grid(c, g.n_slots)), dim3(256), 0, c->stream, g, bytes);
        u64 base = 0;
        for (uint32_t f = 0; f < n_files; f++) {
            u64 total = 0;
            hipLaunchKernelGGL(text_select_kernel, dim3(flat_grid(c, ne)), dim3(256), 0, c->stream, bytes, efile, ne, f, sel);
            CHK((scan_exclusive<u8, u64>(c, sel, ne, within, false, &total)));
            hipLaunchKernelGGL(text_place_kernel, dim3(flat_grid(c, ne)), dim3(256), 0, c->stream, within, efile, ne, f, base, place);
            file_offsets[f] = base;
            base += total;
        }
        file_offsets[n_files] = base;
        c->text_off.assign(file_offsets, file_offsets + n_files + 1);
        CHK(ensure(c, c->d_text, std::max<u64>(base, 1)));
        hipLaunchKernelGGL(text_write_kernel, dim3(flat_grid(c, g.n_slots)), dim3(256), 0, c->stream, g, place, c->d_text);
        HIPCHK(c, hipGetLastError());
        HIPCHK(c, hipStreamSynchronize(c->stream));
        c->text_bytes = base;
        return DISCO_OK;
    };
    const int rc = body();
    release(c, d_findex);
    release(c, bytes);
    release(c, sel);
    release(c, efile);
    release(c, within);
    release(c, place);
    return rc != DISCO_OK ? rc : (int64_t)c->text_bytes;
}

int disco_fetch_edge_text(disco_ctx *c, char *out, uint64_t cap)
{
    if (!c || (!out && c->text_bytes)) return DISCO_E_ARG;
    if (cap < c->text_bytes) return fail(c, DISCO_E_ARG, "disco_fetch_edge_text: need room for %llu bytes", (unsigned long long)c->text_bytes);
    HIPCHK(c, hipSetDevice(c->device));
    if (c->text_bytes) {
        HIPCHK(c, hipMemcpyAsync(out, c->d_text, c->text_bytes, hipMemcpyDeviceToHost, c->stream));
        HIPCHK(c, hipStreamSynchronize(c->stream));
    }
    return DISCO_OK;
}

static int write_text_through_ring(disco_ctx *c, const char *who, const char *d_text, const std::vector<u64> &off, const int *fds, uint32_t n_files)
{
    const size_t HALF = 128u << 20;
    CHK(ring_back_from_rows(c));
    if (!c->h_ring) {
        if (hipHostMalloc(&c->h_ring, 2 * HALF, ring_alloc_flags()) != hipSuccess) {
            c->h_ring = nullptr;
            (void)hipGetLastError();
            return fail(c, DISCO_E_NOMEM, "%s: no pinned staging memory", who);
        }
        c->ring_half = HALF;
        for (int i = 0; i < 2; i++) HIPCHK(c, hipEventCreateWithFlags(&c->ev_ring[i], hipEventDisableTiming));
    }
    std::atomic<bool> ok{true};
    const size_t S = (HALF / n_files) & ~(size_t)4095;
    if (S == 0) return fail(c, DISCO_E_UNSUPPORTED, "%s: too many files for the staging ring", who);
    u64 longest = 0;
    for (uint32_t f = 0; f < n_files; f++) longest = std::max(longest, off[f + 1] - off[f]);
    const u64 rounds = (longest + S - 1) / S;
    auto slice = [&](uint32_t f, u64 r, u64 &lo, size_t &len) {
        const u64 fl = off[f + 1] - off[f];
        lo = std::min<u64>(r * S, fl);
        len = (size_t)(std::min<u64>((r + 1) * S, fl) - lo);
    };
// ... 179 lines not shown
    ChainView g;
    g.src = d_src;
    g.ent = d_ent;
    g.valid = d_valid;
    g.pos = d_pos;
    g.len = c->d_len;
    g.n_slots = n_slots;
    g.min_ovl = min_ovl;
    DevBuf<u32> deg, he, links_of, live;
    DevBuf<u8> internal, is_head;
    DevBuf<ChRank> ra, rb;
    DevBuf<u64> comp_id, link_start;
    const u64 n_half = 2 * n_slots;
    int rc = DISCO_OK;
    auto body = [&]() -> int {
        CHK(ensure(c, deg, n));
        CHK(ensure(c, he, 2 * n));
        CHK(ensure(c, internal, n));
        CHK(ensure(c, ra, n_half));
        CHK(ensure(c, rb, n_half));
        CHK(ensure(c, live, 1));
        HIPCHK(c, hipMemsetAsync(deg, 0, n * sizeof(u32), c->stream));
        hipLaunchKernelGGL(ch_degree_kernel, dim3(flat_grid(c, n_slots)), dim3(256), 0, c->stream, g, deg, he);
        hipLaunchKernelGGL(ch_internal_kernel, dim3(flat_grid(c, n)), dim3(256), 0, c->stream, g, deg, he, n, internal);
        hipLaunchKernelGGL(ch_init_kernel, dim3(flat_grid(c, n_slots)), dim3(256), 0, c->stream, g, internal, he, ra);
        HIPCHK(c, hipGetLastError());
        int max_rounds = 1;
        while (max_rounds < 32 && (1ull << max_rounds) < n_half) ++max_rounds;
        for (int round = 0; round < max_rounds; round++) {
            u32 h_live = 0;
            HIPCHK(c, hipMemsetAsync(live, 0, sizeof(u32), c->stream));
            hipLaunchKernelGGL(ch_jump_kernel, dim3(flat_grid(c, n_half)), dim3(256), 0, c->stream, ra, rb, n_half, live);
            HIPCHK(c, hipMemcpyAsync(&h_live, live, sizeof(u32), hipMemcpyDeviceToHost, c->stream));
            HIPCHK(c, hipStreamSynchronize(c->stream));
            std::swap(ra, rb);
            if (!h_live) break;
        }
        release(c, rb);
        release(c, deg);
        CHK(ensure(c, is_head, n_slots));
        CHK(ensure(c, links_of, n_slots));
        CHK(ensure(c, c->d_ch_dead, std::max<u64>(ne, 1)));
        HIPCHK(c, hipMemsetAsync(c->d_ch_dead, 0, std::max<u64>(ne, 1), c->stream));
        hipLaunchKernelGGL(ch_heads_kernel, dim3(flat_grid(c, n_slots)), dim3(256), 0, c->stream, g, internal, ra, is_head, links_of, c->d_ch_dead);
        CHK(ensure(c, comp_id, n_slots + 1));
        CHK(ensure(c, link_start, n_slots + 1));
        u64 n_comp = 0, n_links = 0;
        CHK((scan_exclusive<u8, u64>(c, is_head, n_slots, comp_id, false, &n_comp)));
        CHK((scan_exclusive<u32, u64>(c, links_of, n_slots, link_start, false, &n_links)));
        CHK(ensure(c, c->d_ch_comp, std::max<u64>(n_comp, 1)));
        CHK(ensure(c, c->d_ch_links, std::max<u64>(n_links, 1)));
        hipLaunchKernelGGL(ch_emit_kernel, dim3(flat_grid(c, n_slots)), dim3(256), 0, c->stream, g, internal, ra, comp_id, link_start, c->d_ch_comp, c->d_ch_links);
        HIPCHK(c, hipGetLastError());
        HIPCHK(c, hipStreamSynchronize(c->stream));
        c->ch_comp_n = n_comp;
        c->ch_links_n = n_links;
        c->ch_edges_n = ne;
        c->ch_ready = true;
        return DISCO_OK;
    };
    rc = body();
    release(c, deg);
    release(c, he);
    release(c, internal);
    release(c, ra);
    release(c, rb);
    release(c, live);
    release(c, is_head);
    release(c, links_of);
    release(c, comp_id);
    release(c, link_start);
    return rc;
}

int disco_contract_chains(disco_ctx *c, uint32_t min_overlap_simplify, uint64_t *n_composite, uint64_t *n_links)
{
    if (!c) return DISCO_E_ARG;
    if (c->phase < 8) return fail(c, DISCO_E_STATE, "disco_contract_chains: run disco_transitive_reduce first");
    HIPCHK(c, hipSetDevice(c->device));
    if (c->n_out == 0) {
        c->ch_comp_n = c->ch_links_n = c->ch_edges_n = 0;
        c->ch_ready = true;
    } else
        CHK(contract_chains(c, c->d_out_src, c->d_out_ent, c->d_out_valid, c->d_out_pos, c->out_used, c->n_out, c->n, min_overlap_simplify));
    if (n_composite) *n_composite = c->ch_comp_n;
    if (n_links) *n_links = c->ch_links_n;
    return DISCO_OK;
}

int disco_contract_chains_of(disco_ctx *c, const disco_edge *edges, uint64_t n_edges, uint32_t min_overlap_simplify, uint64_t *n_composite, uint64_t *n_links)
{
    if (!c || (n_edges && !edges)) return DISCO_E_ARG;
    if (c->phase < 1) return fail(c, DISCO_E_STATE, "disco_contract_chains_of: the context holds no reads (their lengths are needed)");
    HIPCHK(c, hipSetDevice(c->device));
    c->ch_ready = false;
    if (n_edges == 0) {
        c->ch_comp_n = c->ch_links_n = c->ch_edges_n = 0;
        c->ch_ready = true;
    } else {
        DevBuf<u64> d_src, d_ent, d_pos;
        DevBuf<u8> d_valid;
        std::unique_ptr<u64[]> hs(new u64[n_edges]), he(new u64[n_edges]);
        std::atomic<bool> bad{false};
        parallel_for(n_edges, [&](u64 b, u64 e_) {
            for (u64 i = b; i < e_; i++) {
                if (edges[i].src >= c->n || edges[i].dst >= c->n) bad.store(true, std::memory_order_relaxed);
                hs[i] = edges[i].src;
                he[i] = ADJ_MAKE(edges[i].offset, edges[i].dst, edges[i].orient, edges[i].len_dst);
            }
        });
        if (bad) return fail(c, DISCO_E_ARG, "disco_contract_chains_of: an edge names a read the context does not hold");
        int rc = DISCO_OK;
        do {
            if ((rc = ensure(c, d_src, n_edges)) != DISCO_OK) break;
            if ((rc = ensure(c, d_ent, n_edges)) != DISCO_OK) break;
            if ((rc = ensure(c, d_pos, n_edges)) != DISCO_OK) break;
            if ((rc = ensure(c, d_valid, n_edges)) != DISCO_OK) break;
            if (hipMemcpyAsync(d_src, hs.get(), n_edges * 8, hipMemcpyHostToDevice, c->stream) != hipSuccess ||
                hipMemcpyAsync(d_ent, he.get(), n_edges * 8, hipMemcpyHostToDevice, c->stream) != hipSuccess ||
                hipMemsetAsync(d_valid, 1, n_edges, c->stream) != hipSuccess) {
                rc = fail(c, DISCO_E_HIP, "disco_contract_chains_of: upload failed");
                break;
            }
            hipLaunchKernelGGL(iota_u64_kernel, dim3(flat_grid(c, n_edges)), dim3(256), 0, c->stream, d_pos, n_edges);
            rc = contract_chains(c, d_src, d_ent, d_valid, d_pos, n_edges, n_edges, c->n, min_overlap_simplify);
        } while (0);
        release(c, d_src);
        release(c, d_ent);
        release(c, d_pos);
        release(c, d_valid);
        if (rc != DISCO_OK) return rc;
    }
    if (n_composite) *n_composite = c->ch_comp_n;
    if (n_links) *n_links = c->ch_links_n;
    return DISCO_OK;
}

int disco_fetch_chains(disco_ctx *c, disco_chain_edge *comp, disco_chain_link *links, uint8_t *edge_absorbed)
{
    if (!c) return DISCO_E_ARG;
    if (!c->ch_ready) return fail(c, DISCO_E_STATE, "disco_fetch_chains: run disco_contract_chains first");
    HIPCHK(c, hipSetDevice(c->device));
    static_assert(sizeof(disco_chain_edge) == sizeof(ChainEdgeOut) && sizeof(disco_chain_link) == sizeof(ChainLinkOut), "chain records");
    if (comp && c->ch_comp_n) HIPCHK(c, hipMemcpyAsync(comp, c->d_ch_comp, c->ch_comp_n * sizeof(ChainEdgeOut), hipMemcpyDeviceToHost, c->stream));
    if (links && c->ch_links_n) HIPCHK(c, hipMemcpyAsync(links, c->d_ch_links, c->ch_links_n * sizeof(ChainLinkOut), hipMemcpyDeviceToHost, c->stream));
    if (edge_absorbed && c->ch_edges_n) HIPCHK(c, hipMemcpyAsync(edge_absorbed, c->d_ch_dead, c->ch_edges_n, hipMemcpyDeviceToHost, c->stream));
    HIPCHK(c, hipStreamSynchronize(c->stream));
    return DISCO_OK;
}

int disco_set_query_order(disco_ctx *c, const void *d_order_u64)
{
    if (!c) return DISCO_E_ARG;
    c->d_order = (const u64 *)d_order_u64;
    c->order_external = d_order_u64 != nullptr;
    return DISCO_OK;
}

int disco_get_query_order(disco_ctx *c, const void **d_order_u64)
{
    if (!c || !d_order_u64) return DISCO_E_ARG;
    *d_order_u64 = c->d_order_used;
    return DISCO_OK;
}

int disco_phase_ms(disco_ctx *c, float *ms, int n)
{
// ... 955 lines not shown
    }
    int rc = cm->prepare(nranks, rank);
    int bulk_ready = (bulk && bulk->prepare(nranks, rank) == DISCO_OK) ? 1 : 0;
    if (rc == DISCO_OK) rc = cm->join(unique_id);
    if (rc == DISCO_OK && !one_comm) {
        struct IdMsg {
            ncclUniqueId id;
            unsigned long long ok;
        } msg;
        static_assert(sizeof(IdMsg) <= RcclComm::SMALL_VALUES * 8, "fits the staging of host_all_gather");
        memset(&msg, 0, sizeof msg);
        if (rank == 0) msg.ok = ncclGetUniqueId(&msg.id) == ncclSuccess ? 1ull : 0ull;
        void *d_id = cm->d_small;
        memcpy(cm->h_small, &msg, sizeof msg);
        if (hipMemcpyAsync(d_id, cm->h_small, sizeof msg, hipMemcpyHostToDevice, c->stream) != hipSuccess ||
            ncclBroadcast(d_id, d_id, sizeof msg, ncclInt8, 0, cm->comm, c->stream) != ncclSuccess ||
            hipMemcpyAsync(cm->h_small, d_id, sizeof msg, hipMemcpyDeviceToHost, c->stream) != hipSuccess || hipStreamSynchronize(c->stream) != hipSuccess) {
            rc = DISCO_E_HIP;
            cm->err = "broadcast of the second communicator's id failed";
        } else {
            memcpy(&msg, cm->h_small, sizeof msg);
            unsigned long long mine = (msg.ok && bulk_ready) ? 1ull : 0ull, all[DIST_MAX_WORLD];
            rc = cm->host_all_gather(&mine, 1, all, c->stream);
            bool everybody = rc == DISCO_OK;
            for (int p = 0; everybody && p < nranks; p++) everybody = all[p] != 0ull;
            if (rc == DISCO_OK && everybody) {
                const int rb = bulk->join(&msg.id);
                mine = rb == DISCO_OK ? 1ull : 0ull;
                rc = cm->host_all_gather(&mine, 1, all, c->stream);
                for (int p = 0; rc == DISCO_OK && everybody && p < nranks; p++) everybody = all[p] != 0ull;
            }
            if (rc == DISCO_OK && !everybody) {
                if (rank == 0) fprintf(stderr, "[disco] no second communicator on every rank: the reads are gathered on the first one\n");
                delete bulk;
                bulk = nullptr;
            }
        }
    }
    if (one_comm) {
        delete bulk;
        bulk = nullptr;
    }
    if (rc == DISCO_OK && bulk) {
        cm->sibling = bulk;
        bulk->sibling = cm;
    }
    if (rc != DISCO_OK) {
        fail(c, rc, "disco_comm_init: %s %s", cm->err.c_str(), bulk ? bulk->err.c_str() : "");
        delete cm;
        delete bulk;
        return rc;
    }
    return comm_attach(c, cm, bulk);
}

int disco_comm_init_local(disco_ctx *const *ctxs, int nranks)
{
    if (!ctxs || nranks < 1 || nranks > DIST_MAX_WORLD) return DISCO_E_ARG;
    for (int r = 0; r < nranks; r++)
        if (!ctxs[r]) return DISCO_E_ARG;
    auto grp = std::make_shared<LoopGroup>(nranks), grp2 = std::make_shared<LoopGroup>(nranks);
    for (int r = 0; r < nranks; r++) {
        const int rc = comm_attach(ctxs[r], new LoopComm(grp, r), new LoopComm(grp2, r));
        if (rc != DISCO_OK) return rc;
    }
    return DISCO_OK;
}

int disco_probe_run_words(const disco_ctx *c) { return c ? c->runs_lpr : 0; }

int disco_fetch_order(disco_ctx *c, uint64_t *order_words, uint32_t *keys, uint64_t cap, uint64_t *n, int *order_bits)
{
    if (!c || !order_words || !keys || !n || !order_bits) return DISCO_E_ARG;
    if (!c->order_ready || !c->d_order_own || !c->d_okey) return fail(c, DISCO_E_STATE, "disco_fetch_order: disco_build_index made no order");
    *n = c->n;
    *order_bits = c->order_counted_bits;
    if (cap < c->n) return fail(c, DISCO_E_ARG, "disco_fetch_order: room for %llu reads, %llu needed", (unsigned long long)cap, (unsigned long long)c->n);
    HIPCHK(c, hipSetDevice(c->device));
    HIPCHK(c, hipMemcpyAsync(order_words, c->d_order_own, c->n * sizeof(u64), hipMemcpyDeviceToHost, c->stream));
    HIPCHK(c, hipMemcpyAsync(keys, c->d_okey, c->n * sizeof(u32), hipMemcpyDeviceToHost, c->stream));
    HIPCHK(c, hipStreamSynchronize(c->stream));
    return DISCO_OK;
}
int disco_comm_rank(const disco_ctx *c) { return (c && c->comm) ? c->comm->rank : 0; }
int disco_comm_world(const disco_ctx *c) { return (c && c->comm) ? c->comm->world : 1; }
const char *disco_comm_kind(const disco_ctx *c) { return (c && c->comm) ? c->comm->kind() : "none"; }

int disco_dist_range(const disco_ctx *c, uint64_t n_total, uint64_t *lo, uint64_t *hi)
{
    if (!c || !lo || !hi) return DISCO_E_ARG;
    u64 per, l, h;
    dist_range(c, n_total, &per, &l, &h);
    *lo = l;
    *hi = h;
    return DISCO_OK;
}

static int dist_set_reads(disco_ctx *c, u64 n_total, uint32_t dstride)
{
    if (!c->comm) return fail(c, DISCO_E_STATE, "no communicator: call disco_comm_init / disco_comm_init_local first");
    u64 per, lo, hi;
    dist_range(c, n_total, &per, &lo, &hi);
    CHK(begin_rows(c, n_total, per * (u64)c->comm->world, 0, dstride, false));
    c->per = per;
    c->q_lo = c->home_lo = lo;
    c->q_hi = c->home_hi = hi;
    HIPCHK(c, hipMemsetAsync(c->d_reads, 0, c->n_alloc * (u64)dstride * 8, c->stream));
    c->dist_reads = true;
    c->ingest_n = 0;
    return DISCO_OK;
}

static int dist_validate(disco_ctx *c)
{
    const u64 nloc = c->q_hi - c->q_lo;
    CHK(count_lengths(c, c->q_lo, c->q_hi));
    u64 bad = c->h_ctr[CTR_BAD_LEN], ext[2] = {c->h_ctr[CTR_MAX_LEN], c->h_ctr[CTR_MIN_LEN]};
    CHK(host_reduce(c, &bad, 1));
    CHK(host_reduce(c, ext, 2, true));
    if (bad) return fail(c, DISCO_E_ARG, "%llu reads have a length outside (min_overlap=%u, min(32767, 32*stride)]", (unsigned long long)bad, c->prm.min_overlap);
    c->max_len = (u32)ext[0];
    c->min_len = 0xFFFFu - (u32)ext[1];
    CHK(ensure(c, c->d_list_n, 1));
    HIPCHK(c, hipMemsetAsync(c->d_list_n, 0, sizeof(u64), c->stream));
    if (nloc) hipLaunchKernelGGL(probes_sum_kernel, dim3(flat_grid(c, nloc)), dim3(256), 0, c->stream, c->d_len, c->q_lo, c->q_hi, (u32)c->k, c->d_list_n);
    HIPCHK(c, hipMemcpyAsync(&c->home_probes, c->d_list_n, sizeof(u64), hipMemcpyDeviceToHost, c->stream));
    HIPCHK(c, hipStreamSynchronize(c->stream));
    c->job_n_long = 0;
    c->job_short_max = c->max_len;
    if (c->max_len > (u32)DISCO_SHORT_MAX) {
        DevBuf<u64> d_ls;
        u64 hls[2] = {0, 0};
        CHK(ensure(c, d_ls, 2));
        HIPCHK(c, hipMemsetAsync(d_ls, 0, 2 * sizeof(u64), c->stream));
        if (nloc) hipLaunchKernelGGL(long_stats_kernel, dim3(flat_grid(c, nloc)), dim3(256), 0, c->stream, (const u16 *)c->d_len, c->q_lo, c->q_hi, d_ls);
        HIPCHK(c, hipMemcpyAsync(hls, d_ls, sizeof hls, hipMemcpyDeviceToHost, c->stream));
        HIPCHK(c, hipStreamSynchronize(c->stream));
        release(c, d_ls);
        CHK(host_reduce(c, &hls[0], 1));
        CHK(host_reduce(c, &hls[1], 1, true));
        c->job_n_long = hls[0];
        c->job_short_max = (u32)hls[1];
    }
    c->phase = 1;
    return DISCO_OK;
}

int disco_dist_upload_reads(disco_ctx *c, const uint64_t *packed_own, uint32_t stride_words, const uint16_t *len_own, uint64_t n_total)
{
    DISCO_TRACE("disco_dist_upload_reads");
    if (!c) return DISCO_E_ARG;
    HIPCHK(c, hipSetDevice(c->device));
    const uint32_t dstride = (stride_words + 7u) & ~7u;
    CHK(dist_set_reads(c, n_total, dstride));
    const u64 nloc = c->q_hi - c->q_lo;
    if (nloc && (!packed_own || !len_own)) return fail(c, DISCO_E_ARG, "disco_dist_upload_reads: null argument");
    if (nloc) {
        u64 *dst = c->d_reads + c->q_lo * (u64)dstride;
        if (dstride != stride_words) HIPCHK(c, hipMemsetAsync(dst, 0, nloc * (u64)dstride * 8, c->stream));
        HIPCHK(c, hipMemcpy2DAsync(dst, (size_t)dstride * 8, packed_own, (size_t)stride_words * 8, (size_t)stride_words * 8, nloc, hipMemcpyHostToDevice, c->stream));
        HIPCHK(c, hipMemcpyAsync(c->d_len + c->q_lo, len_own, nloc * 2, hipMemcpyHostToDevice, c->stream));
    }
    return dist_validate(c);
}

int disco_dist_generate_reads(disco_ctx *c, const disco_genspec_abi *s)
// ... 579 lines not shown
```

### disco_amd/csrc/disco_kernels.h

```cpp
#ifndef DISCO_KERNELS_H_
#define DISCO_KERNELS_H_

#include "disco_device.h"
#include "readgen.h"

#define PROBE_ROWCAP 512
#define PROBE_SEGW 128
#define PROBE_SEGP (PROBE_SEGW + 64)
#define PROBE_ACAP 32
#define PROBE_CHUNK 4096
#define ES_MID 1024
#define ES_DUPBITS 11
#define ES_DUPTAB (1 << ES_DUPBITS)
#ifndef ES_CAP
#define ES_CAP 256
#endif
#ifndef TR_CAP
#define TR_CAP 256
#endif
#define TR_CAP_SMALL 128
#define VERIFY_SW 8
#define ORDER_BUCKET(key, shift) (((key) * 0x9E3779B1u) >> (shift))
#define SCAN_ITEMS 16
#define SCAN_BLOCK 256
// ... 3548 lines not shown
    }
}

__global__ void merge_need_kernel(const u64 *__restrict__ ref, const u32 *__restrict__ extra_cnt, u64 n, u64 *__restrict__ need)
{
    u64 i = (u64)blockIdx.x * blockDim.x + threadIdx.x;
    for (; i < n; i += (u64)gridDim.x * blockDim.x)
        if (extra_cnt[i]) atomicAdd(need, 2ull * (REF_DEG(ref[i]) + extra_cnt[i]));
}

__global__ void __launch_bounds__(64) merge_sparse_kernel(const u64 *__restrict__ extra_node, const u64 *__restrict__ extra_key, u32 n_extra,
                                                          const u32 *__restrict__ extra_cnt, u64 *__restrict__ ref, u64 *__restrict__ adj, u64 free_base,
                                                          u64 *__restrict__ bump)
{
    const u32 lane = threadIdx.x;
    for (u32 i = blockIdx.x; i < n_extra; i += gridDim.x) {
        const u64 v = EXTRA_NODE(extra_node[i]);
        bool earlier = false;
        for (u32 t = lane; t < i; t += 64) earlier |= EXTRA_NODE(extra_node[t]) == v;
        if (__any(earlier)) continue;
        const u64 r = ref[v];
        const u32 d = REF_DEG(r), nd = d + extra_cnt[v];
        u64 p = 0;
        if (lane == 0) p = free_base + atomicAdd(bump, 2ull * nd);
        p = __shfl(p, 0);
        u64 *lo = adj + p, *up = adj + p + nd;
        for (u32 t = lane; t < d; t += 64) up[t] = adj[REF_POS(r) + t] & ~ADJ_FLAG;
        u32 at = d;
        for (u32 t0 = i; t0 < n_extra; t0 += 64) {
            const u32 t = t0 + lane;
            const bool mine = t < n_extra && EXTRA_NODE(extra_node[t]) == v;
            const u64 mk = __ballot(mine);
            if (mine) up[at + rank_below(mk)] = extra_key[t];
            at += __popcll(mk);
        }
        __syncthreads();
        wave_rank_sort(up, lo, nd, lane);
        __syncthreads();
        if (lane == 0) ref[v] = REF_MAKE(p, nd);
    }
}

#define MERGE_RANK_MAX 24
__global__ void __launch_bounds__(64) merge_rows_kernel(const u64 *__restrict__ old_ref, const u64 *__restrict__ old_adj, const u32 *__restrict__ extra_cnt,
                                                        const u64 *__restrict__ new_start, u64 *__restrict__ new_adj, u64 n, u64 *__restrict__ scratch,
                                                        u64 scratch_cap)
{
    u64 *tmp = scratch + (u64)blockIdx.x * scratch_cap;
    const u32 lane = threadIdx.x;
    for (u64 v = blockIdx.x; v < n; v += gridDim.x) {
        const u64 r = old_ref[v];
        const u64 so = REF_POS(r);
        const u32 d0 = REF_DEG(r);
        const u32 x = extra_cnt[v];
        const u64 o = new_start[v];
        const u32 d = d0 + x;
        if (d <= 64) {
            u64 e = ~0ull;
            if (lane < d0) e = old_adj[so + lane] & ~ADJ_FLAG;
            else if (lane < d) e = new_adj[o + lane];
            u32 pos = lane;
            if (x > MERGE_RANK_MAX) e = wave_bitonic_sort(e, lane);
            else
                for (u32 j = 0; j < x; j++) {
                    const u64 bj = readlane_u64(e, d0 + j);
                    const u32 rank = (u32)__popcll(__ballot(e < bj));
                    if (lane == d0 + j) pos = rank;
                    else if (lane < d0 && bj < e) pos++;
                }
            if (lane < d) new_adj[o + pos] = e;
            continue;
        }
        for (u32 i = lane; i < d0; i += 64) new_adj[o + i] = old_adj[so + i] & ~ADJ_FLAG;
        if (!x) continue;
        __syncthreads();
        wave_rank_sort(new_adj + o, tmp, d, lane);
        __syncthreads();
        for (u32 i = lane; i < d; i += 64) new_adj[o + i] = tmp[i];
        __syncthreads();
    }
}

#define HALF_CAP 4
struct TrArgs {
    DiscoView v;
    const u64 *ref;
    u64 *adj;
    u64 *half;
    u32 *hcnt;
    u64 *wide_list;
    u32 *n_wide;
    u32 wide_cap;
    u64 *big_list;
    u32 *n_big;
    u32 big_cap;
    u64 *scratch;
    u64 hcap;
    u32 all_flags;
    const u64 *order;
};

#define TR_UNAVAIL 0ull

#ifndef TR_HASH_LOAD
#define TR_HASH_LOAD 4
#endif
static_assert(TR_HASH_LOAD * 64 + 1 < 4 * TR_CAP_SMALL && TR_CAP_SMALL <= TR_CAP, "the register path's table (at most TR_HASH_LOAD x 64 four-byte slots in the space of s_hkey) needs two more slots behind it: one takes the stores of the lanes without a hit, one holds the multi-rank variant's verdict on the node");
#define TR_EMPTY 0xFFFFFFFFFFFFFFFFull
#ifdef TR_EXP_XOR_HASH
__device__ __forceinline__ u32 tr_hash(u64 id, u32 hmask) { return ((u32)id ^ ((u32)id >> 9)) & hmask; }
#else
__device__ __forceinline__ u32 tr_hash(u64 id, u32 hmask) { return (((u32)id * 0x9E3779B1u) >> 10) & hmask; }
#endif

template <bool DEFER>
__device__ __forceinline__ void tr_node(const TrArgs &a, u64 v, u32 d, u64 *hkey, u8 *hstate, u32 *sent, u32 hmask, u32 lane)
{
    const u64 vs = REF_POS(a.ref[v]);
    u64 *row = a.adj + vs;
    for (u32 i = lane; i <= hmask; i += 64) {
        hkey[i] = TR_EMPTY;
        hstate[i] = 0;
    }
    __syncthreads();
    for (u32 s = lane; s < d; s += 64) {
        u64 id = ADJ_DST(row[s]);
        u32 idx = tr_hash(id, hmask);
        for (;;) {
            u64 old = atomicCAS(&hkey[idx], TR_EMPTY, id);
            if (old == TR_EMPTY || old == id) break;
            idx = (idx + 1) & hmask;
        }
        sent[s] = idx;
    }
    __syncthreads();
    for (u32 g0 = 0; g0 < d; g0 += 64) {
        int cur = -1;
        for (;;) {
            const u32 s = g0 + lane;
            u64 mk = __ballot(s < d && !hstate[sent[s]]);
            if (cur >= 0) mk &= ~((2ull << cur) - 1ull);
            if (!mk) break;
            cur = (int)__ffsll((long long)mk) - 1;
            const u32 i = g0 + (u32)cur;
            const u64 e1 = row[i];
            const u64 u = ADJ_DST(e1);
            const u32 type1 = ADJ_ORI(e1);
            const bool in1 = (type1 == 0 || type1 == 2);
            const u64 ru = a.ref[u];
            const u64 us = REF_POS(ru);
            u32 du = REF_DEG(ru);
            if (DEFER && du == 0) {
                if (lane == 0) atomicAdd(&a.v.ctr[CTR_OVERFLOW], 1ull);
            }
            for (u32 t = lane; t < du; t += 64) {
                const u64 e2 = a.adj[us + t];
                const u32 type2 = ADJ_ORI(e2);
                const bool ok = in1 ? (type2 == 0 || type2 == 1) : (type2 == 2 || type2 == 3);
                if (!ok) continue;
                const u64 w = ADJ_DST(e2);
                u32 idx = tr_hash(w, hmask);
                for (;;) {
                    u64 kk = hkey[idx];
                    if (kk == TR_EMPTY) break;
                    if (kk == w) {
                        hstate[idx] = 1;
                        break;
                    }
                    idx = (idx + 1) & hmask;
                }
            }
            __syncthreads();
        }
    }
    u32 nfree = 0;
    for (u32 s0 = 0; s0 < d; s0 += 64) {
        const u32 s = s0 + lane;
        const bool fl = (s < d) && hstate[sent[s]];
        const bool fr = (s < d) && !fl;
        if (fl) row[s] |= ADJ_FLAG;
        const u64 mk = __ballot(fr);
        if (a.half && fr) {
            const u32 r = nfree + rank_below(mk);
            if (r < HALF_CAP) a.half[v * HALF_CAP + r] = row[s] & ~ADJ_FLAG;
        }
        nfree += __popcll(mk);
    }
    if (a.hcnt && lane == 0) {
        a.hcnt[v] = nfree;
        if (nfree > HALF_CAP) {
            const u32 idx = atomicAdd(a.n_wide, 1u);
            if (idx < a.wide_cap) a.wide_list[idx] = v;
        }
    }
    __syncthreads();
}

struct TrNodeRegs {
    u32 v;
    u64 vs;
    u32 d;
    u32 dfull;
    u64 e;
    u32 s2;
    u64 r0, r2;
    u64 p0, p2;
};

template <bool DEFER, bool LISTS>
__device__ __forceinline__ void tr_node_small(const TrArgs &a, const TrNodeRegs &nd, u64 *hkey, u8 *hstate, u32 lane)
{
    const u32 d = nd.d;
    const u64 e = nd.e;
    constexpr u32 hc = TR_HASH_LOAD * 64;
    constexpr u32 hmask = hc - 1;
    static_assert(hc == 256, "one uint4 per lane clears the table");
    u32 *ht = (u32 *)hkey;
    (void)hstate;
    ((uint4 *)ht)[lane] = make_uint4(~0u, ~0u, ~0u, ~0u);
    const u32 s2 = nd.s2;
    const u64 st0 = REF_POS(nd.r0), st2 = REF_POS(nd.r2);
    const u32 d0 = REF_DEG(nd.r0), d2 = REF_DEG(nd.r2);
    const u64 p0 = lane < d0 ? nd.p0 : 0ull;
    const u64 p2 = lane < d2 ? nd.p2 : 0ull;
    if (DEFER) ht[hc + 1] = (d0 == 0 || d2 == 0) ? 1u : 0u;
    __syncthreads();
    u32 sent = 0;
#if defined(TR_EXP) && TR_EXP == 2
    sent = lane;
    if (p0 != 0x123456789ull || p2 != 0x123456789ull) ht[lane] = 0u;
#else
    {
        const u32 id = (u32)ADJ_DST(e);
        u32 idx = tr_hash(id, hmask);
        for (;;) {
            const u32 old = atomicCAS(&ht[idx], 0xFFFFFFFFu, id);
            if (old == 0xFFFFFFFFu || old == id) break;
            idx = (idx + 1) & hmask;
        }
        sent = idx;
    }
#endif
    __syncthreads();
    const u64 dmask = d >= 64u ? ~0ull : (1ull << d) - 1ull;
    auto mark = [&](u32 want, bool act, u64 e2) {
        const u32 type2 = ADJ_ORI(e2);
        u64 pm = __ballot(act && ((type2 >> 1) == want));
        const u32 w = (u32)ADJ_DST(e2);
        u32 off = tr_hash(w, hmask) << 2;
        const u32 spare = hc << 2;
        do {
            const u32 kk = *(const u32 *)((const u8 *)ht + off);
            const u64 hm = __ballot((kk & 0x7FFFFFFFu) == w) & pm;
            const u64 fm = __ballot(kk == 0xFFFFFFFFu);
            u32 woff;
            asm volatile("v_cndmask_b32_e64 %0, %1, %2, %3" : "=v"(woff) : "v"(spare), "v"(off), "s"(hm));
            *(u32 *)((u8 *)ht + woff) = kk | 0x80000000u;
            pm &= ~(hm | fm);
            off = (off + 4u) & (hmask << 2);
        } while (pm != 0ull);
    };
    auto sweep = [&](u32 want, u64 us, u32 du, u64 pre) {
        mark(want, lane < du, pre);
        if (du > 64)
            for (u32 t0 = 64; t0 < du; t0 += 64) {
                const bool act = t0 + lane < du;
                mark(want, act, act ? a.adj[us + t0 + lane] : 0ull);
            }
    };
    u64 todo = dmask;
#if !(defined(TR_EXP) && TR_EXP >= 1)
    sweep(ADJ_ORI((u64)(u32)__builtin_amdgcn_readlane((int)(u32)e, 0)) & 1u, st0, d0, p0);
    todo = dmask & ~1ull;
    __syncthreads();
#endif
    for (;;) {
#if defined(TR_EXP) && TR_EXP >= 1
        if (p0 != 0x123456789ull || p2 != 0x123456789ull) break;
#endif
        const u32 hs = ht[sent];
        const u64 mk = __ballot((hs >> 31) == 0u) & todo;
        if (!mk) break;
        const u32 i = (u32)__ffsll((long long)mk) - 1u;
        todo = dmask & (~1ull << i);
        const u64 e1 = readlane_u64(e, i);
        const u32 want = ADJ_ORI(e1) & 1u;
        if (i == s2) sweep(want, st2, d2, p2);
        else {
            const u64 ru = a.ref[ADJ_DST(e1)];
            const u64 us = REF_POS(ru);
            const u32 du = REF_DEG(ru);
            if (DEFER && du == 0) ht[hc + 1] = 1u;
            sweep(want, us, du, (lane < du) ? a.adj[us + lane] : 0ull);
        }
        __syncthreads();
    }
    const bool keep = !DEFER || ht[hc + 1] == 0u;
    if (DEFER && !keep && lane == 0) {
        const u32 idx = atomicAdd(a.n_big, 1u);
        if (idx < a.big_cap) a.big_list[idx] = nd.v;
        else atomicAdd(&a.v.ctr[CTR_OVERFLOW], 1ull);
    }
#if defined(TR_EXP) && TR_EXP >= 1
    const bool fl = lane < d && lane >= 2u && (ht[sent & 63u] != 0x12345u);
#else
    const u32 hs_end = ht[sent];
    const bool fl = keep & (lane < d) & ((hs_end >> 31) != 0u);
#endif
    const bool fr = keep & (lane < d) & !fl;
    const u64 mk = __ballot(fr);
    if (fl && ((!LISTS && (a.all_flags || !a.half)) || __popcll(mk) > HALF_CAP)) a.adj[nd.vs + lane] = e | ADJ_FLAG;
    if ((LISTS || a.half) && fr) {
        const u32 r = rank_below(mk);
        if (r < HALF_CAP) a.half[(u64)nd.v * HALF_CAP + r] = e;
    }
    if ((LISTS || a.hcnt) && lane == 0 && keep) {
        const u32 nfree = __popcll(mk);
        a.hcnt[nd.v] = nfree;
        if (nfree > HALF_CAP) {
            const u32 idx = atomicAdd(a.n_wide, 1u);
            if (idx < a.wide_cap) a.wide_list[idx] = nd.v;
        }
    }
    __syncthreads();
}

#ifndef TR_WAVES_PER_SIMD
#define TR_WAVES_PER_SIMD 6
#endif
template <bool BIG, bool DEFER, int CAP = TR_CAP, bool LISTS = false>
__global__ void __launch_bounds__(64, (CAP == TR_CAP_SMALL && !BIG) ? 8 : TR_WAVES_PER_SIMD) transitive_mark_kernel(TrArgs a)
{
    __shared__ u64 s_hkey[BIG ? 1 : 2 * CAP];
    __shared__ u32 s_ent[BIG ? 1 : CAP];
    __shared__ u8 s_state[BIG ? 1 : 2 * CAP];
    __shared__ u64 s_mid[(BIG || DEFER) ? 1 : 64];
    const u32 lane = threadIdx.x;
    const u64 n_items = BIG ? (u64)min(*a.n_big, a.big_cap) : (a.v.q_hi - a.v.q_lo);
    u64 *hkey = s_hkey;
    u32 *sent = s_ent;
    u8 *hstate = s_state;
    if (BIG) {
        u8 *base = (u8 *)a.scratch + (u64)blockIdx.x * (a.hcap * 8 + a.hcap * 4 + a.hcap);
        hkey = (u64 *)base;
        sent = (u32 *)(base + a.hcap * 8);
        hstate = base + a.hcap * 8 + a.hcap * 4;
    }
    const u32 n_last = (u32)(a.v.n - 1);
    const u32 lane8 = lane << 3;
    u64 cbeg = 0, cend = 0;
    u64 rv_chunk = 0;
    u32 v_chunk = 0;
    u32 ccnt = 0;
    auto stage_row = [&](u32 t) {
        TrNodeRegs r;
        const bool ok = t < ccnt;
        const u32 tc = ok ? t : ccnt - 1u;
        const u64 rv = readlane_u64(rv_chunk, tc);
        r.v = (u32)__builtin_amdgcn_readlane((int)v_chunk, (int)tc);
        r.vs = REF_POS(rv);
        r.dfull = ok ? REF_DEG(rv) : 0u;
        r.d = (r.dfull <= 64) ? r.dfull : 0u;
        r.e = *(const u64 *)((const u8 *)(a.adj + r.vs) + (lane < r.d ? lane8 : 0u));
        r.s2 = 0;
        r.r0 = r.r2 = r.p0 = r.p2 = 0;
        return r;
    };
    auto stage_refs = [&](TrNodeRegs &r) {
        r.e &= ~ADJ_FLAG;
        const u32 side0 = ADJ_ORI(readlane_u64(r.e, 0)) >> 1;
        const u64 om = __ballot((ADJ_ORI(r.e) >> 1) != side0);
        r.s2 = om ? (u32)__ffsll((long long)om) - 1u : 0u;
        const u64 e0 = readlane_u64(r.e, 0), e2 = readlane_u64(r.e, r.s2);
        r.r0 = a.ref[min((u32)ADJ_DST(e0), n_last)];
        r.r2 = a.ref[min((u32)ADJ_DST(e2), n_last)];
    };
    auto stage_rows = [&](TrNodeRegs &r) {
        r.r0 = uniform_u64(r.r0);
        r.r2 = uniform_u64(r.r2);
        const u32 d0 = REF_DEG(r.r0), d2 = REF_DEG(r.r2);
        r.p0 = *(const u64 *)((const u8 *)(a.adj + REF_POS(r.r0)) + (lane < d0 ? lane8 : 0u));
        r.p2 = *(const u64 *)((const u8 *)(a.adj + REF_POS(r.r2)) + (lane < d2 ? lane8 : 0u));
    };
#if defined(WQ_SPLIT_ALL)
    WqSplit wqs;
    while (BIG ? wq_grab<1>(a.v.wq, n_items, cbeg, cend) : wq_grab_split(a.v.wq, n_items, cbeg, cend, wqs)) {
#else
    while (BIG ? wq_grab<1>(a.v.wq, n_items, cbeg, cend) : wq_grab(a.v.wq, n_items, cbeg, cend)) {
#endif
    if (BIG) {
        for (u64 it = cbeg; it < cend; it++) {
            const u64 v = a.big_list[it];
            const u32 d = REF_DEG(a.ref[v]);
            if (d == 0) continue;
            tr_node<DEFER>(a, v, d, hkey, hstate, sent, (u32)a.hcap - 1, lane);
        }
        continue;
    }
    {
        const u64 idx = cbeg + lane, ic = idx < cend ? idx : cend - 1;
        v_chunk = (u32)(a.order ? ORDER_ID(a.order[ic]) : a.v.q_lo + ic);
        rv_chunk = a.ref[v_chunk];
    }
    ccnt = (u32)(cend - cbeg);
    TrNodeRegs n0 = stage_row(0), n1 = stage_row(1), n2 = stage_row(2), n3;
    stage_refs(n0);
    stage_refs(n1);
    stage_rows(n0);
    u32 n_mid = 0;
    auto step = [&](TrNodeRegs &A, TrNodeRegs &B, TrNodeRegs &C, TrNodeRegs &D, u32 t) {
        stage_rows(B);
        stage_refs(C);
        D = stage_row(t + 3);
        if (A.d != 0)
            tr_node_small<DEFER, LISTS>(a, A, s_hkey, s_state, lane);
        else if (A.dfull != 0) {
            if (!DEFER && A.dfull <= (u32)CAP) {
                if (lane == 0) s_mid[n_mid] = A.v;
                n_mid++;
            } else if (lane == 0) {
                u32 idx = atomicAdd(a.n_big, 1u);
                if (idx < a.big_cap) a.big_list[idx] = A.v;
                else atomicAdd(&a.v.ctr[CTR_OVERFLOW], 1ull);
            }
        }
    };
    for (u32 t = 0; t < ccnt; t += 4) {
        step(n0, n1, n2, n3, t);
        step(n1, n2, n3, n0, t + 1);
        step(n2, n3, n0, n1, t + 2);
        step(n3, n0, n1, n2, t + 3);
    }
    if (!DEFER && n_mid) {
        __syncthreads();
        for (u32 x = 0; x < n_mid; x++) {
            const u64 v = s_mid[x];
            const u32 dv = REF_DEG(a.ref[v]);
            u32 hc = 64;
            while (hc < 2 * dv) hc <<= 1;
            tr_node<DEFER>(a, v, dv, hkey, hstate, sent, hc - 1, lane);
        }
        __syncthreads();
    }
    }
}

#define EMIT_CHUNK 256
struct EmitArgs {
    DiscoView v;
    const u64 *ref;
    const u64 *adj;
    const u32 *hcnt;
    const u64 *half;
    const u64 *list;
    u64 n_list;
    u64 *out_src;
    u64 *out_ent;
    u64 out_cap;
    u64 *bump;
    u32 local_only;
    OwnSet own;
};

__global__ void __launch_bounds__(64) emit_kernel(EmitArgs a)
{
    const u32 lane = threadIdx.x;
    u64 chunk_base = 0;
    u32 chunk_used = EMIT_CHUNK;
    bool have_chunk = false;
    auto close_chunk = [&]() {
        if (have_chunk)
            for (u32 i = chunk_used + lane; i < EMIT_CHUNK; i += 64)
                if (chunk_base + i < a.out_cap) a.out_src[chunk_base + i] = ~0ull;
    };
    u64 cbeg = 0, cend = 0;
    while (wq_grab(a.v.wq, a.list ? a.n_list : a.own.count(), cbeg, cend))
    for (u64 it = cbeg; it < cend; it++) {
        const u64 v = a.list ? a.list[it] : a.own.node(it);
        if (!a.own.mine(v)) continue;
        if (a.hcnt && a.hcnt[v] <= HALF_CAP) continue;
        const u64 rv = a.ref[v];
        const u32 d = REF_DEG(rv);
        if (d == 0) continue;
        const u64 vs = REF_POS(rv);
        const u32 Lv = a.v.len[v];
        for (u32 s0 = 0; s0 < d; s0 += 64) {
            const u32 s = s0 + lane;
            bool keep = false;
            u64 e = 0;
            if (s < d) {
                e = a.adj[vs + s];
                const u64 w = ADJ_DST(e);
                if (v < w && !(e & ADJ_FLAG) && (!a.local_only || a.own.mine(w))) {
                    const u32 Lw = ADJ_DLEN(e);
                    const u64 twin = ADJ_MAKE(Lw + ADJ_OFF(e) - Lv, v, disco_twin_orient(ADJ_ORI(e)), Lv);
                    const u32 cw = a.hcnt ? a.hcnt[w] : HALF_CAP + 1;
                    if (cw <= HALF_CAP) {
                        const u64 *hw = a.half + w * HALF_CAP;
                        for (u32 r = 0; r < cw; r++) keep |= (hw[r] == twin);
                    } else {
                        const u64 rw = a.ref[w];
                        const u64 *roww = a.adj + REF_POS(rw);
                        const int ti = adj_find(roww, REF_DEG(rw), twin);
                        keep = (ti >= 0) && !(roww[ti] & ADJ_FLAG);
                    }
                }
            }
            const u64 mk = __ballot(keep);
            const u32 cnt = __popcll(mk);
            if (cnt) {
                if (chunk_used + cnt > EMIT_CHUNK) {
                    close_chunk();
                    u64 base = 0;
                    if (lane == 0) base = atomicAdd(a.bump, (u64)EMIT_CHUNK);
                    chunk_base = uniform_u64(base);
                    chunk_used = 0;
                    have_chunk = true;
                }
                if (keep) {
                    const u64 pos = chunk_base + chunk_used + rank_below(mk);
                    if (pos < a.out_cap) {
                        a.out_src[pos] = v;
                        a.out_ent[pos] = e & ~ADJ_FLAG;
                    }
                }
                chunk_used += cnt;
            }
        }
    }
    close_chunk();
}

struct EmitHalfArgs {
    DiscoView v;
    const u64 *ref;
    const u64 *adj;
    const u64 *half;
    const u32 *hcnt;
    u64 *out_src;
    u64 *out_ent;
    u64 out_cap;
    u64 *bump;
    u32 local_only;
    OwnSet own;
    const u64 *order;
};

__global__ void __launch_bounds__(64) emit_half_kernel(EmitHalfArgs a)
{
    const u32 lane = threadIdx.x;
    u64 chunk_base = 0;
    u32 chunk_used = EMIT_CHUNK;
    bool have_chunk = false;
    auto close_chunk = [&]() {
        if (have_chunk)
            for (u32 i = chunk_used + lane; i < EMIT_CHUNK; i += 64)
                if (chunk_base + i < a.out_cap) a.out_src[chunk_base + i] = ~0ull;
    };
    const u64 nq = a.own.count();
    u64 cbeg = 0, cend = 0;
    while (wq_grab(a.v.wq, (nq + 63) / 64, cbeg, cend))
    for (u64 blk = cbeg; blk < cend; blk++) {
        const bool live = blk * 64 + lane < nq;
        const u64 v = a.order ? ORDER_ID(a.order[live ? blk * 64 + lane : 0]) : a.own.node_by_id(live ? blk * 64 + lane : 0);
        const u32 cnt = live ? a.hcnt[v] : 0u;
        const u32 Lv = live ? (u32)a.v.len[v] : 0u;
#pragma unroll
        for (u32 r = 0; r < HALF_CAP; r++) {
            bool keep = false;
            u64 e = 0;
            if (cnt <= HALF_CAP && r < cnt) {
                e = a.half[v * HALF_CAP + r];
                const u64 w = ADJ_DST(e);
                if (v < w && (!a.local_only || a.own.otab || w < a.own.hi)) {
                    const u64 twin = ADJ_MAKE(ADJ_DLEN(e) + ADJ_OFF(e) - Lv, v, disco_twin_orient(ADJ_ORI(e)), Lv);
                    const u32 cw = a.hcnt[w];
                    if (cw <= HALF_CAP) {
                        const ulonglong2 *hw = (const ulonglong2 *)(a.half + w * HALF_CAP);
                        const ulonglong2 h0 = hw[0], h1 = hw[1];
                        keep = (cw > 0 && h0.x == twin) || (cw > 1 && h0.y == twin) || (cw > 2 && h1.x == twin) || (cw > 3 && h1.y == twin);
                    } else {
                        const u64 rw = a.ref[w];
                        const u64 *roww = a.adj + REF_POS(rw);
                        const int ti = adj_find(roww, REF_DEG(rw), twin);
                        keep = (ti >= 0) && !(roww[ti] & ADJ_FLAG);
                    }
                }
            }
            const u64 mk = __ballot(keep);
            const u32 kc = __popcll(mk);
            if (kc) {
                if (chunk_used + kc > EMIT_CHUNK) {
                    close_chunk();
                    u64 base = 0;
                    if (lane == 0) base = atomicAdd(a.bump, (u64)EMIT_CHUNK);
                    chunk_base = uniform_u64(base);
                    chunk_used = 0;
                    have_chunk = true;
                }
                if (keep) {
                    const u64 pos = chunk_base + chunk_used + rank_below(mk);
                    if (pos < a.out_cap) {
                        a.out_src[pos] = v;
                        a.out_ent[pos] = e;
                    }
                }
                chunk_used += kc;
            }
        }
    }
    close_chunk();
}

__global__ void emit_valid_kernel(const u64 *__restrict__ out_src, u64 n, u8 *__restrict__ valid)
{
    u64 i = (u64)blockIdx.x * blockDim.x + threadIdx.x;
    for (; i < n; i += (u64)gridDim.x * blockDim.x) valid[i] = out_src[i] != ~0ull;
}

__global__ void emit_compact32_kernel(const u64 *__restrict__ out_src, const u64 *__restrict__ out_ent, const u8 *__restrict__ valid,
                                      const u64 *__restrict__ pos, u64 n, u32 *__restrict__ dst_src, u64 *__restrict__ dst_ent)
{
    u64 i = (u64)blockIdx.x * blockDim.x + threadIdx.x;
    for (; i < n; i += (u64)gridDim.x * blockDim.x)
        if (valid[i]) {
            dst_src[pos[i]] = (u32)out_src[i];
            dst_ent[pos[i]] = out_ent[i];
        }
}

__global__ void emit_compact_kernel(const u64 *__restrict__ out_src, const u64 *__restrict__ out_ent, const u8 *__restrict__ valid,
                                    const u64 *__restrict__ pos, u64 n, u64 *__restrict__ dst_src, u64 *__restrict__ dst_ent)
{
    u64 i = (u64)blockIdx.x * blockDim.x + threadIdx.x;
    for (; i < n; i += (u64)gridDim.x * blockDim.x)
        if (valid[i]) {
            dst_src[pos[i]] = out_src[i];
            dst_ent[pos[i]] = out_ent[i];
        }
}

__global__ void edge_subs_kernel(const u64 *__restrict__ out_src, const u64 *__restrict__ out_ent, const u8 *__restrict__ valid,
                                 const u64 *__restrict__ pos, u64 n, const u64 *__restrict__ reads, const u16 *__restrict__ len, int S,
                                 u16 *__restrict__ subs)
{
    u64 i = (u64)blockIdx.x * blockDim.x + threadIdx.x;
    for (; i < n; i += (u64)gridDim.x * blockDim.x)
        if (valid[i]) {
            const u64 src = out_src[i], e = out_ent[i];
            const int l1 = (int)len[src], l2 = (int)ADJ_DLEN(e), off = (int)ADJ_OFF(e), ovl = l1 - off;
            const u32 o = ADJ_ORI(e);
            const u32 rev = (o == 1 || o == 2);
            subs[pos[i]] = (u16)seg_mismatches<false>(reads + src * S, reads + ADJ_DST(e) * S, S, l2, o >= 2 ? off : 0, o >= 2 ? 0 : l2 - ovl, ovl, rev);
        }
}

__device__ __forceinline__ u32 uf_load(const u32 *p) { return __hip_atomic_load(p, __ATOMIC_RELAXED, __HIP_MEMORY_SCOPE_AGENT); }

__device__ __forceinline__ u32 uf_find(u32 *parent, u32 x)
{
    for (;;) {
        const u32 p = uf_load(&parent[x]);
        if (p == x) return x;
        const u32 g = uf_load(&parent[p]);
        if (g != p) __hip_atomic_store(&parent[x], g, __ATOMIC_RELAXED, __HIP_MEMORY_SCOPE_AGENT);
        x = p;
    }
}

__global__ void uf_init_kernel(u32 *parent, u64 n)
{
    u64 i = (u64)blockIdx.x * blockDim.x + threadIdx.x;
    for (; i < n; i += (u64)gridDim.x * blockDim.x) parent[i] = (u32)i;
}

__global__ void uf_hook_kernel(const u64 *__restrict__ out_src, const u64 *__restrict__ out_ent, const u8 *__restrict__ valid, u64 n_slots, u32 *parent)
{
    u64 i = (u64)blockIdx.x * blockDim.x + threadIdx.x;
    for (; i < n_slots; i += (u64)gridDim.x * blockDim.x) {
        if (!valid[i]) continue;
        u32 a = (u32)out_src[i], b = (u32)ADJ_DST(out_ent[i]);
        for (;;) {
            a = uf_find(parent, a);
            b = uf_find(parent, b);
            if (a == b) break;
            if (a < b) {
                const u32 t = a;
                a = b;
                b = t;
            }
            if (atomicCAS(&parent[a], a, b) == a) break;
        }
    }
}

__global__ void uf_compress_kernel(u32 *parent, u64 n)
{
    u64 i = (u64)blockIdx.x * blockDim.x + threadIdx.x;
    for (; i < n; i += (u64)gridDim.x * blockDim.x) {
        u32 r = (u32)i;
        while (parent[r] != r) r = parent[r];
        parent[i] = r;
    }
}

#define UF_SLOTS 1024u
__global__ void __launch_bounds__(256) uf_count_kernel(const u64 *__restrict__ out_src, const u8 *__restrict__ valid, u64 n_slots, const u32 *__restrict__ parent, u32 *cnt)
{
    __shared__ u32 s_key[UF_SLOTS], s_val[UF_SLOTS];
    for (u32 x = threadIdx.x; x < UF_SLOTS; x += blockDim.x) {
        s_key[x] = 0xFFFFFFFFu;
        s_val[x] = 0u;
    }
    __syncthreads();
    u64 i = (u64)blockIdx.x * blockDim.x + threadIdx.x;
    for (; i < n_slots; i += (u64)gridDim.x * blockDim.x)
        if (valid[i]) {
            const u32 root = parent[(u32)out_src[i]];
            u32 idx = (root * 0x9E3779B1u) >> 22;
            bool placed = false;
            for (int t = 0; t < 8 && !placed; t++) {
                const u32 old = atomicCAS(&s_key[idx], 0xFFFFFFFFu, root);
                if (old == 0xFFFFFFFFu || old == root) {
                    atomicAdd(&s_val[idx], 1u);
                    placed = true;
                } else
                    idx = (idx + 1u) & (UF_SLOTS - 1u);
            }
            if (!placed) atomicAdd(&cnt[root], 1u);
        }
    __syncthreads();
    for (u32 x = threadIdx.x; x < UF_SLOTS; x += blockDim.x)
        if (s_val[x]) atomicAdd(&cnt[s_key[x]], s_val[x]);
}

__global__ void uf_big_kernel(const u32 *__restrict__ cnt, u64 n, u32 thr, u64 *list, u32 *n_list, u32 cap)
{
    u64 i = (u64)blockIdx.x * blockDim.x + threadIdx.x;
    for (; i < n; i += (u64)gridDim.x * blockDim.x)
        if (cnt[i] >= thr) {
            const u32 k = atomicAdd(n_list, 1u);
            if (k < cap) list[k] = (i << 32) | cnt[i];
        }
}

__global__ void uf_assign_kernel(const u64 *__restrict__ pairs, u32 n_pairs, u16 *cfile)
{
    u32 i = blockIdx.x * blockDim.x + threadIdx.x;
    if (i < n_pairs) cfile[pairs[i] >> 32] = (u16)(pairs[i] & 0xFFFF);
}

__global__ void uf_edge_file_kernel(const u64 *__restrict__ out_src, const u8 *__restrict__ valid, const u64 *__restrict__ pos, u64 n_slots,
                                    const u32 *__restrict__ parent, const u16 *__restrict__ cfile, u32 n_files, u16 *edge_file)
{
    u64 i = (u64)blockIdx.x * blockDim.x + threadIdx.x;
    for (; i < n_slots; i += (u64)gridDim.x * blockDim.x)
        if (valid[i]) {
            const u32 r = parent[(u32)out_src[i]];
            u16 f = cfile[r];
            if (f == 0xFFFFu) f = (u16)(((u64)(r * 0x9E3779B1u) * n_files) >> 32);
            edge_file[pos[i]] = f;
        }
}

__global__ void order_count_kernel(const u32 *__restrict__ okey, u64 nq, u32 shift, u32 *__restrict__ cnt, u32 *__restrict__ oslot)
{
    u64 i = (u64)blockIdx.x * blockDim.x + threadIdx.x;
    for (; i < nq; i += (u64)gridDim.x * blockDim.x) oslot[i] = atomicAdd(&cnt[ORDER_BUCKET(okey[i], shift)], 1u);
}

__global__ void order_scatter_kernel(const u32 *__restrict__ okey, const u32 *__restrict__ oslot, const u32 *__restrict__ start, u32 shift, u64 lo, u64 nq,
                                     const u16 *__restrict__ len, u64 *__restrict__ order)
{
    u64 i = (u64)blockIdx.x * blockDim.x + threadIdx.x;
    for (; i < nq; i += (u64)gridDim.x * blockDim.x) order[(u64)start[ORDER_BUCKET(okey[i], shift)] + oslot[i]] = ORDER_MAKE(lo + i, len[lo + i]);
}

__global__ void order_pack_kernel(const u64 *__restrict__ ids, u64 nq, const u16 *__restrict__ len, u64 *__restrict__ order)
{
    u64 i = (u64)blockIdx.x * blockDim.x + threadIdx.x;
    for (; i < nq; i += (u64)gridDim.x * blockDim.x) order[i] = ORDER_MAKE(ids[i], len[ids[i]]);
}

__global__ void count_above_kernel(const u32 *__restrict__ cnt, const u64 *__restrict__ ref, u64 lo, u64 hi, u32 thr, u64 *out)
{
    u64 i = lo + (u64)blockIdx.x * blockDim.x + threadIdx.x;
    u32 c = 0;
    for (; i < hi; i += (u64)gridDim.x * blockDim.x) c += (ref ? REF_DEG(ref[i]) : cnt[i]) > thr;
    for (int o = 32; o > 0; o >>= 1) c += __shfl_down(c, o);
    if ((threadIdx.x & 63) == 0 && c) atomicAdd(out, (u64)c);
}

__global__ void __launch_bounds__(256) stream_copy_kernel(const ulonglong2 *__restrict__ src, ulonglong2 *__restrict__ dst, u64 n)
{
    u64 i = (u64)blockIdx.x * blockDim.x + threadIdx.x;
    const u64 step = (u64)gridDim.x * blockDim.x;
    for (; i + 3 * step < n; i += 4 * step) {
        const ulonglong2 x0 = src[i], x1 = src[i + step], x2 = src[i + 2 * step], x3 = src[i + 3 * step];
        dst[i] = x0;
        dst[i + step] = x1;
        dst[i + 2 * step] = x2;
        dst[i + 3 * step] = x3;
    }
    for (; i < n; i += step) dst[i] = src[i];
}

__global__ void __launch_bounds__(256) gather_rows_kernel(const ulonglong2 *__restrict__ tab, u64 nrows, u32 per_lane, u64 *__restrict__ sink)
{
    const u64 tid = (u64)blockIdx.x * blockDim.x + threadIdx.x;
    u64 acc = 0;
    for (u32 it = 0; it < per_lane; it += 4) {
        ulonglong2 v[4][4];
#pragma unroll
        for (int u = 0; u < 4; u++) {
            const u64 r = disco_hash64(tid * per_lane + it + u) % nrows;
            const ulonglong2 *g = tab + r * 4;
            v[u][0] = g[0];
            v[u][1] = g[1];
            v[u][2] = g[2];
            v[u][3] = g[3];
        }
#pragma unroll
        for (int u = 0; u < 4; u++) acc ^= v[u][0].x ^ v[u][1].y ^ v[u][2].x ^ v[u][3].y;
    }
    if (acc == 0x1234567ull) sink[0] = acc;
}

__global__ void max_u32_kernel(const u32 *__restrict__ p, u64 n, u64 *__restrict__ out)
{
    u64 i = (u64)blockIdx.x * blockDim.x + threadIdx.x;
    u32 m = 0;
    for (; i < n; i += (u64)gridDim.x * blockDim.x) m = max(m, p[i]);
    for (int o = 32; o > 0; o >>= 1) m = max(m, (u32)__shfl_down(m, o));
    if ((threadIdx.x & 63) == 0 && m) atomicMax(out, (u64)m);
}

__global__ void iota_u64_kernel(u64 *p, u64 n)
{
    u64 i = (u64)blockIdx.x * blockDim.x + threadIdx.x;
    for (; i < n; i += (u64)gridDim.x * blockDim.x) p[i] = i;
}

__global__ void fill_u64_kernel(u64 *p, u64 n, u64 val)
{
// ... 6 lines not shown
```

### disco_amd/csrc/disco_text.h

```cpp
#ifndef DISCO_TEXT_H_
#define DISCO_TEXT_H_

#include "disco_kernels.h"

struct TextView {
    const u64 *src, *ent;
    const u8 *valid;
    const u64 *pos;
    const u16 *len;
    const u64 *file_index;
    u64 n_slots;
};

__device__ __forceinline__ u32 tx_digits(u64 v)
{
    u32 d = 1;
    while (v >= 10) {
        v /= 10;
        d++;
    }
    return d;
}
__device__ __forceinline__ char *tx_put(char *p, u64 v)
{
    const u32 d = tx_digits(v);
    for (u32 i = d; i-- > 0;) {
        p[i] = (char)('0' + (u32)(v % 10));
        v /= 10;
    }
    return p + d;
}
struct TextNumbers {
    u64 a, b;
    u32 orient, ovl, len1, off, len2;
};
__device__ __forceinline__ TextNumbers tx_numbers(const TextView &g, u64 s)
{
    TextNumbers t;
    const u64 src = g.src[s], e = g.ent[s], dst = ADJ_DST(e);
    t.a = g.file_index ? g.file_index[src] : src + 1;
    t.b = g.file_index ? g.file_index[dst] : dst + 1;
    t.orient = ADJ_ORI(e);
    t.len1 = g.len[src];
    t.off = ADJ_OFF(e);
    t.ovl = t.len1 - t.off;
    t.len2 = ADJ_DLEN(e);
    return t;
}

__global__ void text_measure_kernel(TextView g, u8 *__restrict__ bytes)
{
    u64 s = (u64)blockIdx.x * blockDim.x + threadIdx.x;
    for (; s < g.n_slots; s += (u64)gridDim.x * blockDim.x) {
        if (!g.valid[s]) continue;
        const TextNumbers t = tx_numbers(g, s);
        bytes[g.pos[s]] = (u8)(tx_digits(t.a) + tx_digits(t.b) + 1 + tx_digits(t.ovl) + tx_digits(t.len1) + tx_digits(t.off) + tx_digits(t.len1 - 1) + tx_digits(t.len2) +
                               tx_digits(t.ovl - 1) + 20);
    }
}

__global__ void text_select_kernel(const u8 *__restrict__ bytes, const u16 *__restrict__ efile, u64 ne, u32 file, u8 *__restrict__ out)
{
    u64 i = (u64)blockIdx.x * blockDim.x + threadIdx.x;
    for (; i < ne; i += (u64)gridDim.x * blockDim.x) out[i] = efile[i] == file ? bytes[i] : (u8)0;
}
__global__ void text_place_kernel(const u64 *__restrict__ within, const u16 *__restrict__ efile, u64 ne, u32 file, u64 base, u64 *__restrict__ place)
{
    u64 i = (u64)blockIdx.x * blockDim.x + threadIdx.x;
    for (; i < ne; i += (u64)gridDim.x * blockDim.x)
        if (efile[i] == file) place[i] = base + within[i];
}

__global__ void text_write_kernel(TextView g, const u64 *__restrict__ place, char *__restrict__ text)
{
    u64 s = (u64)blockIdx.x * blockDim.x + threadIdx.x;
    for (; s < g.n_slots; s += (u64)gridDim.x * blockDim.x) {
        if (!g.valid[s]) continue;
        const TextNumbers t = tx_numbers(g, s);
        char *p = text + place[g.pos[s]];
        p = tx_put(p, t.a); *p++ = '\t';
        p = tx_put(p, t.b); *p++ = '\t';
        *p++ = (char)('0' + t.orient); *p++ = ',';
        p = tx_put(p, t.ovl); *p++ = ','; *p++ = '0'; *p++ = ','; *p++ = '0'; *p++ = ',';
        p = tx_put(p, t.len1); *p++ = ',';
        p = tx_put(p, t.off); *p++ = ',';
        p = tx_put(p, t.len1 - 1); *p++ = ',';
        p = tx_put(p, t.len2); *p++ = ','; *p++ = '0'; *p++ = ',';
        p = tx_put(p, t.ovl - 1); *p++ = ','; *p++ = 'N'; *p++ = 'A'; *p++ = ','; *p++ = '2'; *p++ = '\n';
    }
}

#define CWORD_MAKE(j, id, suf, rev) (((u64)(j) << 33) | ((u64)(id) << 2) | ((u64)(suf) << 1) | (u64)(rev))
#define CWORD_J(w) ((u32)((w) >> 33) & 0x7FFFu)
#define CWORD_ID(w) (((w) >> 2) & 0x7FFFFFFFull)
#define CGRP_LDS_MAX 4096u
#define CGRP_BLOCK 256
enum { CGRP_N_LDS = 0, CGRP_N_GLOBAL = 1, CGRP_LARGEST = 2, CGRP_BAD_KEYS = 3, CGRP_CTRS = 4 };

__global__ void cgrp_count_kernel(const u64 *__restrict__ best, const u8 *__restrict__ contained, u64 n, u32 *__restrict__ cnt, u32 *__restrict__ ctr)
{
    u64 i = (u64)blockIdx.x * blockDim.x + threadIdx.x;
    for (; i < n; i += (u64)gridDim.x * blockDim.x)
        if (contained[i]) {
            const u64 s = CKEY_SUPER(best[i]);
            if (s < n) atomicAdd(&cnt[s], 1u);
            else atomicAdd(&ctr[CGRP_BAD_KEYS], 1u);
        }
}
__global__ void cgrp_place_kernel(const u64 *__restrict__ best, const u8 *__restrict__ contained, u64 n, u64 nc, u32 *__restrict__ cursor, u64 *__restrict__ word,
                                  u32 *__restrict__ sup)
{
    u64 i = (u64)blockIdx.x * blockDim.x + threadIdx.x;
    for (; i < n; i += (u64)gridDim.x * blockDim.x)
        if (contained[i]) {
            const u64 key = best[i], s = CKEY_SUPER(key);
            if (s >= n) continue;
            const u32 at = atomicAdd(&cursor[s], 1u);
            if (at >= nc) continue;
            word[at] = CWORD_MAKE(CKEY_J(key), i, CKEY_SUFFIX(key), CKEY_REV(key));
            sup[at] = (u32)s;
        }
}

struct CgrpLists {
    u32 *lds, *glb;
    u32 *ctr;
    u32 cap;
};
__global__ void cgrp_sort_small_kernel(const u32 *__restrict__ gend, u64 n, u64 *__restrict__ word, CgrpLists L)
{
    u64 s = (u64)blockIdx.x * blockDim.x + threadIdx.x;
    u32 largest = 0;
    for (; s < n; s += (u64)gridDim.x * blockDim.x) {
        const u32 b = s ? gend[s - 1] : 0u, e = gend[s], m = e - b;
        largest = m > largest ? m : largest;
        if (m < 2) continue;
        if (m > CROW_GROUP_MAX) {
            const bool in_lds = m <= CGRP_LDS_MAX;
            const u32 at = atomicAdd(&L.ctr[in_lds ? CGRP_N_LDS : CGRP_N_GLOBAL], 1u);
            if (at < L.cap) (in_lds ? L.lds : L.glb)[at] = (u32)s;
            continue;
        }
        for (u32 a = b + 1; a < e; a++) {
            const u64 w = word[a];
            u32 q = a;
            while (q > b && word[q - 1] > w) {
                word[q] = word[q - 1];
                q--;
            }
            word[q] = w;
        }
    }
    for (int o = 32; o > 0; o >>= 1) {
        const u32 x = __shfl_down(largest, o);
        largest = x > largest ? x : largest;
    }
    if ((threadIdx.x & 63) == 0 && largest > __atomic_load_n(&L.ctr[CGRP_LARGEST], __ATOMIC_RELAXED)) atomicMax(&L.ctr[CGRP_LARGEST], largest);
}

__host__ __device__ __forceinline__ void cgrp_step(u64 *h, u32 m, u32 P, u32 k2, u32 j2, u32 tid, u32 nt)
{
    for (u32 t = tid; t < P / 2; t += nt) {
// ... 149 lines not shown
```

### include/disco_hip_inspect.h

```cpp
#ifndef DISCO_HIP_INSPECT_H_
#define DISCO_HIP_INSPECT_H_

#include "disco_hip.h"

#ifdef __cplusplus
extern "C" {
#endif

int disco_fetch_order(disco_ctx *ctx, uint64_t *order_words, uint32_t *keys, uint64_t cap, uint64_t *n, int *order_bits);

#ifdef __cplusplus
}
#endif
#endif
```

Measured before the change: 10.97 billion overlaps/s.

## Encode survivor lists self-delimiting and emit edges densely without compaction

Transitive-reduction marking now writes each node's surviving half-edges with an end-of-list bit in the entry word, which removes the separate per-node count array and its memset. When the run is single-device and uses half lists, emit writes edges densely through new list and dense emit kernels. The valid/pos compaction arrays are then released, and downstream fetch, text, partition and chain kernels accept null valid/pos. This removes a counter array, the compaction pass and its indirection, at the cost of reserving bit 15 in entries and extra branching on null pointers.

```diff
diff --git a/disco_amd/build.py b/disco_amd/build.py
--- a/disco_amd/build.py
+++ b/disco_amd/build.py
@@ -99,6 +99,13 @@
         if verbose:
             print(" ".join(cmd))
         subprocess.check_call(cmd)
+    sv = os.path.join(HERE, "bin", "survivor_check")
+    ssrc = [os.path.join(HERE, "host", "survivor_check.cpp"), os.path.join(HERE, "csrc", "disco_survivor.h")]
+    if force or _stale(sv, ssrc):
+        cmd = ["g++", "-O2", "-std=c++17", "-Wall", "-o", sv, ssrc[0]]
+        if verbose:
+            print(" ".join(cmd))
+        subprocess.check_call(cmd)
     return BUILDG
 
 
diff --git a/disco_amd/buildgraph.py b/disco_amd/buildgraph.py
--- a/disco_amd/buildgraph.py
+++ b/disco_amd/buildgraph.py
@@ -153,6 +153,7 @@
 
 INSPECT_ABI = [
     ("disco_fetch_order", C.c_int, [_P, _P, _P, C.c_uint64, C.POINTER(C.c_uint64), C.POINTER(C.c_int)]),
+    ("disco_fetch_survivor_layout", C.c_int, [_P, _P, C.c_uint64, C.POINTER(C.c_uint64), C.POINTER(C.c_int), C.POINTER(C.c_uint64)]),
 ]
 _inspect_bound = False
 
@@ -461,6 +462,17 @@
         order, keys = np.zeros(max(n.value, 1), dtype=np.uint64), np.zeros(max(n.value, 1), dtype=np.uint32)
         self._chk(self.L.disco_fetch_order(self._h, order.ctypes.data, keys.ctypes.data, len(order), C.byref(n), C.byref(bits)))
         return order[:n.value], keys[:n.value], bits.value
+
+    def fetch_survivor_layout(self, lengths: bool = True):
+        _bind_inspect(self.L)
+        n, dense, used = C.c_uint64(0), C.c_int(0), C.c_uint64(0)
+        self._chk(self.L.disco_fetch_survivor_layout(self._h, None, 0, C.byref(n), C.byref(dense), C.byref(used)))
+        lens = None
+        if lengths:
+            lens = np.zeros(max(n.value, 1), dtype=np.uint8)
+            self._chk(self.L.disco_fetch_survivor_layout(self._h, lens.ctypes.data, len(lens), C.byref(n), C.byref(dense), C.byref(used)))
+            lens = lens[:n.value]
+        return lens, bool(dense.value), used.value
 
     def measure_hbm(self, nbytes: int = 4 << 30, reps: int = 5) -> float:
         out = C.c_double(0.0)
diff --git a/disco_amd/csrc/disco_chains.h b/disco_amd/csrc/disco_chains.h
--- a/disco_amd/csrc/disco_chains.h
+++ b/disco_amd/csrc/disco_chains.h
@@ -16,7 +16,7 @@
 
 __device__ __forceinline__ bool ch_kept(const ChainView &g, u64 s)
 {
-    if (!g.valid[s]) return false;
+    if (g.valid && !g.valid[s]) return false;
     return (u32)g.len[g.src[s]] - ADJ_OFF(g.ent[s]) >= g.min_ovl;
 }
 __device__ __forceinline__ u32 ch_src(const ChainView &g, u32 h) { return (h & 1) ? (u32)ADJ_DST(g.ent[h >> 1]) : (u32)g.src[h >> 1]; }
@@ -106,7 +106,7 @@
     if (mine) atomicAdd(live, mine);
 }
 
-__device__ __forceinline__ u64 ch_rankid(const ChainView &g, u32 h) { return 2 * g.pos[h >> 1] + (h & 1u); }
+__device__ __forceinline__ u64 ch_rankid(const ChainView &g, u32 h) { return 2 * (g.pos ? g.pos[h >> 1] : (u64)(h >> 1)) + (h & 1u); }
 
 struct ChSlot {
     u32 head;
@@ -142,7 +142,7 @@
         const bool head = c.in_chain && c.index == 0;
         is_head[s] = head ? 1 : 0;
         links_of[s] = head ? r[c.head].cnt : 0u;
-        if (c.in_chain) dead[g.pos[s]] = 1;
+        if (c.in_chain) dead[g.pos ? g.pos[s] : s] = 1;
     }
 }
 
diff --git a/disco_amd/csrc/disco_device.h b/disco_amd/csrc/disco_device.h
--- a/disco_amd/csrc/disco_device.h
+++ b/disco_amd/csrc/disco_device.h
@@ -8,6 +8,8 @@
 typedef unsigned int u32;
 typedef unsigned short u16;
 typedef unsigned char u8;
+
+#include "disco_survivor.h"
 
 #define DISCO_WAVE 64
 #define DISCO_NOKEY 0x7FFFFFFFFFFFFFFFull
diff --git a/disco_amd/csrc/disco_hip.hip b/disco_amd/csrc/disco_hip.hip
--- a/disco_amd/csrc/disco_hip.hip
+++ b/disco_amd/csrc/disco_hip.hip
@@ -278,6 +278,7 @@
     bool adj_imported = false;
     u64 adj_span = 0;
     bool half_complete = false;
+    bool half_selfdel = false;
     DevBuf<u32> d_extra_cnt;
     DevBuf<u64> d_extra_node, d_extra_key;
     u32 *d_n_extra = nullptr;
@@ -304,6 +305,7 @@
     u64 text_bytes = 0;
     DevBuf<u64> d_out_src, d_out_ent;
     u64 out_used = 0;
+    bool out_dense = false;
     u64 n_out = 0;
 
     hipEvent_t ev0[DISCO_PH_SLOTS] = {nullptr}, ev1[DISCO_PH_SLOTS] = {nullptr};
@@ -1265,7 +1267,7 @@
     return transitive_mark_kernel<false, false>;
 }
 
-static int tr_args_begin(disco_ctx *c, TrArgs *a)
+static int tr_args_begin(disco_ctx *c, TrArgs *a, bool selfdel = false)
 {
     a->v = view(c);
     a->ref = c->d_adj_ref;
@@ -1279,14 +1281,17 @@
     a->hcnt = nullptr;
     if (c->use_half) {
         CHK(ensure(c, c->d_half, c->n * HALF_CAP));
-        CHK(ensure(c, c->d_hcnt, c->n));
-        HIPCHK(c, hipMemsetAsync(c->d_hcnt, 0, std::max<u64>(c->n, 1) * sizeof(u32), c->stream));
+        if (!selfdel) {
+            CHK(ensure(c, c->d_hcnt, c->n));
+            HIPCHK(c, hipMemsetAsync(c->d_hcnt, 0, std::max<u64>(c->n, 1) * sizeof(u32), c->stream));
+        }
         CHK(ensure(c, c->d_wide, std::min<u64>(c->n, c->n / 32 + 4096)));
         CHK(ensure(c, c->d_n_wide, 1));
         HIPCHK(c, hipMemsetAsync(c->d_n_wide, 0, sizeof(u32), c->stream));
         a->half = c->d_half;
-        a->hcnt = c->d_hcnt;
-    }
+        a->hcnt = selfdel ? nullptr : (u32 *)c->d_hcnt;
+    }
+    c->half_selfdel = c->use_half && selfdel;
     a->wide_list = c->d_wide;
     a->n_wide = c->d_n_wide;
     a->wide_cap = c->d_wide.cap;
@@ -3319,12 +3324,13 @@
     } else
         CHK(ensure_big_cap(c, nullptr, c->d_adj_ref, TR_CAP));
     c->use_half = !getenv("DISCO_NO_HALF");
+    const u32 all_flags = (c->adj_imported || !c->use_half || c->q_lo != 0 || c->q_hi != c->n) ? 1u : 0u;
+    const bool lists = c->use_half && !all_flags;
     TrArgs a;
-    CHK(tr_args_begin(c, &a));
+    CHK(tr_args_begin(c, &a, lists));
     a.order = (c->d_order_used && c->order_q_lo == c->q_lo && c->order_q_hi == c->q_hi && !c->adj_imported && !getenv("DISCO_TR_NO_ORDER")) ? c->d_order_used : nullptr;
-    a.all_flags = (c->adj_imported || !c->use_half || c->q_lo != 0 || c->q_hi != c->n) ? 1u : 0u;
+    a.all_flags = all_flags;
     ph_begin(c, DISCO_PH_TRMARK);
-    const bool lists = a.half && a.hcnt && !a.all_flags;
     if (nq) wq_launch(c, tr_pick(false, false, tr_small, lists), nq, "DISCO_TR_WAVES", 32, a);
     ph_end(c, DISCO_PH_TRMARK);
     HIPCHK(c, hipGetLastError());
@@ -3354,7 +3360,7 @@
     HIPCHK(c, hipSetDevice(c->device));
     const u64 nq = c->q_hi - c->q_lo;
     ph_begin(c, DISCO_PH_EMIT);
-    const int grid = wq_grid(c, emit_kernel, nq, "DISCO_EMIT_WAVES");
+    const int grid = wq_grid(c, emit_kernel<false>, nq, "DISCO_EMIT_WAVES");
     const u64 n_push = c->dist_active ? c->n_push_r : 0;
     const int grid_push = (int)std::max<u64>(std::min<u64>((n_push + 63) / 64, (u64)c->n_cu * 16), 1);
     const u64 nwaves = (u64)grid * 2 + (n_push ? (u64)grid_push : 0);
@@ -3363,13 +3369,16 @@
         CHK(ensure_group(c, want, want, c->d_out_src, c->d_out_ent));
         HIPCHK(c, hipMemsetAsync(c->d_bump, 0, sizeof(u64), c->stream));
         const bool half_emit = c->use_half && c->half_complete;
+        const bool dense = half_emit && c->half_selfdel && !c->dist_active;
+        if (half_emit && c->half_selfdel && !dense) return fail(c, DISCO_E_STATE, "disco_emit_edges: self-delimiting lists under a communicator");
+        c->out_dense = dense;
         if (half_emit && nq) {
             EmitHalfArgs h;
             h.v = view(c);
             h.ref = c->d_adj_ref;
             h.adj = c->d_adj;
             h.half = c->d_half;
-            h.hcnt = c->d_hcnt;
+            h.hcnt = dense ? nullptr : (const u32 *)c->d_hcnt;
             h.out_src = c->d_out_src;
             h.out_ent = c->d_out_ent;
             h.out_cap = c->d_out_src.cap;
@@ -3377,14 +3386,19 @@
             h.local_only = c->dist_active ? 1u : 0u;
             h.own = own_set(c);
             h.order = nullptr;
-            const int gh = wq_grid(c, emit_half_kernel, (nq + 63) / 64, "DISCO_EMIT_WAVES");
-            hipLaunchKernelGGL(emit_half_kernel, dim3(gh), dim3(64), 0, c->stream, h);
+            if (dense) {
+                const int gh = wq_grid(c, emit_half_lists_kernel, (nq + 63) / 64, "DISCO_EMIT_WAVES");
+                hipLaunchKernelGGL(emit_half_lists_kernel, dim3(gh), dim3(64), 0, c->stream, h);
+            } else {
+                const int gh = wq_grid(c, emit_half_kernel, (nq + 63) / 64, "DISCO_EMIT_WAVES");
+                hipLaunchKernelGGL(emit_half_kernel, dim3(gh), dim3(64), 0, c->stream, h);
+            }
         }
         EmitArgs a;
         a.v = view(c);
         a.ref = c->d_adj_ref;
         a.adj = c->d_adj;
-        a.hcnt = half_emit ? c->d_hcnt : nullptr;
+        a.hcnt = half_emit && !dense ? (const u32 *)c->d_hcnt : nullptr;
         a.half = half_emit ? c->d_half : nullptr;
         const bool listed = half_emit && c->n_wide <= c->d_wide.cap;
         a.list = listed ? c->d_wide : nullptr;
@@ -3396,7 +3410,10 @@
         a.local_only = c->dist_active ? 1u : 0u;
         a.own = own_set(c);
         HIPCHK(c, hipMemsetAsync(c->d_wq, 0, sizeof(u64) * WQ_WORDS, c->stream));
-        if (nq && !(listed && c->n_wide == 0)) hipLaunchKernelGGL(emit_kernel, dim3(grid), dim3(64), 0, c->stream, a);
+        if (nq && !(listed && c->n_wide == 0)) {
+            if (dense) hipLaunchKernelGGL(emit_kernel<true>, dim3(grid), dim3(64), 0, c->stream, a);
+            else hipLaunchKernelGGL(emit_kernel<false>, dim3(grid), dim3(64), 0, c->stream, a);
+        }
         if (n_push) {
             EmitRecvArgs pr;
             pr.items = c->d_push_r;
@@ -3425,7 +3442,11 @@
         if (attempt == 5) return fail(c, DISCO_E_CAPACITY, "disco_emit_edges: output buffer could not be sized");
     }
     u64 total = 0;
-    if (c->out_used) {
+    if (c->out_dense) {
+        total = c->out_used;
+        release(c, c->d_out_valid);
+        release(c, c->d_out_pos);
+    } else if (c->out_used) {
         if (c->out_used > c->d_out_valid.cap || c->out_used + 1 > c->d_out_pos.cap) {
             release(c, c->d_out_valid);
             release(c, c->d_out_pos);
@@ -3602,6 +3623,9 @@
     return (int64_t)nc;
 }
 
+static const u8 *out_valid(const disco_ctx *c) { return c->out_dense ? nullptr : (const u8 *)c->d_out_valid.p; }
+static const u64 *out_pos(const disco_ctx *c) { return c->out_dense ? nullptr : (const u64 *)c->d_out_pos.p; }
+
 int64_t disco_fetch_edges(disco_ctx *c, disco_edge *out, uint64_t cap)
 {
     DISCO_TRACE("disco_fetch_edges");
@@ -3613,10 +3637,12 @@
     if (cap < ne) return fail(c, DISCO_E_ARG, "disco_fetch_edges: need room for %llu edges", (unsigned long long)ne);
     if (ne == 0) return 0;
     CHK(ensure_host_len(c));
-    CHK(ensure_group(c, ne, ne + ne / 8 + 1024, c->d_fetch_src, c->d_fetch_ent));
+    if (c->out_dense) CHK(ensure(c, c->d_fetch_src, ne + ne / 8 + 1024));
+    else CHK(ensure_group(c, ne, ne + ne / 8 + 1024, c->d_fetch_src, c->d_fetch_ent));
     u32 *csrc = c->d_fetch_src;
-    u64 *cent = c->d_fetch_ent;
-    hipLaunchKernelGGL(emit_compact32_kernel, dim3(flat_grid(c, c->out_used)), dim3(256), 0, c->stream, c->d_out_src, c->d_out_ent, c->d_out_valid, c->d_out_pos, c->out_used, csrc, cent);
+    const u64 *cent = c->out_dense ? (const u64 *)c->d_out_ent : (const u64 *)c->d_fetch_ent;
+    if (c->out_dense) hipLaunchKernelGGL(emit_src32_kernel, dim3(flat_grid(c, ne)), dim3(256), 0, c->stream, c->d_out_src, ne, csrc);
+    else hipLaunchKernelGGL(emit_compact32_kernel, dim3(flat_grid(c, c->out_used)), dim3(256), 0, c->stream, c->d_out_src, c->d_out_ent, c->d_out_valid, c->d_out_pos, c->out_used, csrc, c->d_fetch_ent.p);
     const u64 CHUNK = 1ull << 22;
     if (!c->h_stage) {
         if (hipHostMalloc((void **)&c->h_stage, 4 * CHUNK * sizeof(u64)) != hipSuccess) c->h_stage = nullptr;
@@ -3684,7 +3710,7 @@
     }
     DevBuf<u16> subs;
     CHK(ensure(c, subs, ne));
-    hipLaunchKernelGGL(edge_subs_kernel, dim3(flat_grid(c, c->out_used)), dim3(256), 0, c->stream, c->d_out_src, c->d_out_ent, c->d_out_valid, c->d_out_pos,
+    hipLaunchKernelGGL(edge_subs_kernel, dim3(flat_grid(c, c->out_used)), dim3(256), 0, c->stream, c->d_out_src, c->d_out_ent, out_valid(c), out_pos(c),
                        c->out_used, c->d_reads, c->d_len, c->S, subs);
     hipError_t e1 = hipMemcpyAsync(out, subs, ne * sizeof(u16), hipMemcpyDeviceToHost, c->stream);
     hipError_t e2 = hipStreamSynchronize(c->stream);
@@ -3776,7 +3802,7 @@
     const u64 ne = c->n_out;
     if (cap < ne) return fail(c, DISCO_E_ARG, "disco_fetch_edge_files: need room for %llu edges", (unsigned long long)ne);
     if (ne == 0) return 0;
-    return partition_edges(c, c->d_out_src, c->d_out_ent, c->d_out_valid, c->d_out_pos, c->out_used, ne, c->n, n_files, out);
+    return partition_edges(c, c->d_out_src, c->d_out_ent, out_valid(c), out_pos(c), c->out_used, ne, c->n, n_files, out);
 }
 
 int64_t disco_partition_edges(disco_ctx *c, const disco_edge *edges, uint64_t n_edges, uint64_t n_nodes, uint32_t n_files, uint16_t *out)
@@ -3834,8 +3860,8 @@
     TextView g;
     g.src = c->d_out_src;
     g.ent = c->d_out_ent;
-    g.valid = c->d_out_valid;
-    g.pos = c->d_out_pos;
+    g.valid = out_valid(c);
+    g.pos = out_pos(c);
     g.len = c->d_len;
     g.n_slots = c->out_used;
     DevBuf<u64> d_findex, within, place;
@@ -4181,7 +4207,7 @@
         c->ch_comp_n = c->ch_links_n = c->ch_edges_n = 0;
         c->ch_ready = true;
     } else
-        CHK(contract_chains(c, c->d_out_src, c->d_out_ent, c->d_out_valid, c->d_out_pos, c->out_used, c->n_out, c->n, min_overlap_simplify));
+        CHK(contract_chains(c, c->d_out_src, c->d_out_ent, out_valid(c), out_pos(c), c->out_used, c->n_out, c->n, min_overlap_simplify));
     if (n_composite) *n_composite = c->ch_comp_n;
     if (n_links) *n_links = c->ch_links_n;
     return DISCO_OK;
@@ -5303,6 +5329,27 @@
     HIPCHK(c, hipStreamSynchronize(c->stream));
     return DISCO_OK;
 }
+int disco_fetch_survivor_layout(disco_ctx *c, uint8_t *list_len, uint64_t cap, uint64_t *n, int *dense, uint64_t *out_used)
+{
+    if (!c || !n || !dense || !out_used) return DISCO_E_ARG;
+    if (c->phase < 8) return fail(c, DISCO_E_STATE, "disco_fetch_survivor_layout: run disco_transitive_reduce first");
+    *n = c->n;
+    *dense = c->out_dense ? 1 : 0;
+    *out_used = c->out_used;
+    if (!list_len) return DISCO_OK;
+    if (cap < c->n) return fail(c, DISCO_E_ARG, "disco_fetch_survivor_layout: room for %llu nodes, %llu needed", (unsigned long long)cap, (unsigned long long)c->n);
+    if (!c->half_selfdel || !c->d_half) return fail(c, DISCO_E_STATE, "disco_fetch_survivor_layout: the last marking kept counts, not self-delimiting lists");
+    HIPCHK(c, hipSetDevice(c->device));
+    std::vector<u64> half(c->n * HALF_CAP), ref(c->n);
+    if (c->n) {
+        HIPCHK(c, hipMemcpyAsync(half.data(), c->d_half, c->n * HALF_CAP * sizeof(u64), hipMemcpyDeviceToHost, c->stream));
+        HIPCHK(c, hipMemcpyAsync(ref.data(), c->d_adj_ref, c->n * sizeof(u64), hipMemcpyDeviceToHost, c->stream));
+        HIPCHK(c, hipStreamSynchronize(c->stream));
+    }
+    for (u64 v = 0; v < c->n; v++)
+        list_len[v] = REF_DEG(ref[v]) ? (uint8_t)surv_len(half[4 * v], half[4 * v + 1], half[4 * v + 2], half[4 * v + 3]) : 0xFFu;
+    return DISCO_OK;
+}
 int disco_comm_rank(const disco_ctx *c) { return (c && c->comm) ? c->comm->rank : 0; }
 int disco_comm_world(const disco_ctx *c) { return (c && c->comm) ? c->comm->world : 1; }
 const char *disco_comm_kind(const disco_ctx *c) { return (c && c->comm) ? c->comm->kind() : "none"; }
diff --git a/disco_amd/csrc/disco_kernels.h b/disco_amd/csrc/disco_kernels.h
--- a/disco_amd/csrc/disco_kernels.h
+++ b/disco_amd/csrc/disco_kernels.h
@@ -3654,6 +3654,7 @@
 }
 
 #define HALF_CAP 4
+static_assert(HALF_CAP == SURV_CAP, "disco_survivor.h decodes lists of HALF_CAP slots");
 struct TrArgs {
     DiscoView v;
     const u64 *ref;
@@ -3745,6 +3746,10 @@
             __syncthreads();
         }
     }
+    const bool selfdel = a.half && !a.hcnt;
+    u32 ntotal = 0;
+    if (selfdel)
+        for (u32 s0 = 0; s0 < d; s0 += 64) ntotal += __popcll(__ballot((s0 + lane < d) && !hstate[sent[s0 + lane]]));
     u32 nfree = 0;
     for (u32 s0 = 0; s0 < d; s0 += 64) {
         const u32 s = s0 + lane;
@@ -3754,12 +3759,13 @@
         const u64 mk = __ballot(fr);
         if (a.half && fr) {
             const u32 r = nfree + rank_below(mk);
-            if (r < HALF_CAP) a.half[v * HALF_CAP + r] = row[s] & ~ADJ_FLAG;
+            if (r < HALF_CAP) a.half[v * HALF_CAP + r] = selfdel ? surv_encode(row[s] & ~ADJ_FLAG, r, ntotal) : (row[s] & ~ADJ_FLAG);
         }
         nfree += __popcll(mk);
     }
-    if (a.hcnt && lane == 0) {
-        a.hcnt[v] = nfree;
+    if (a.half && lane == 0) {
+        if (a.hcnt) a.hcnt[v] = nfree;
+        else if (nfree == 0) a.half[v * HALF_CAP] = SURV_NONE;
         if (nfree > HALF_CAP) {
             const u32 idx = atomicAdd(a.n_wide, 1u);
             if (idx < a.wide_cap) a.wide_list[idx] = v;
@@ -3882,12 +3888,21 @@
     const bool fr = keep & (lane < d) & !fl;
     const u64 mk = __ballot(fr);
     if (fl && ((!LISTS && (a.all_flags || !a.half)) || __popcll(mk) > HALF_CAP)) a.adj[nd.vs + lane] = e | ADJ_FLAG;
+    const u32 nfree = __popcll(mk);
+    const bool selfdel = DEFER ? false : (LISTS || (a.half && !a.hcnt));
     if ((LISTS || a.half) && fr) {
         const u32 r = rank_below(mk);
-        if (r < HALF_CAP) a.half[(u64)nd.v * HALF_CAP + r] = e;
-    }
-    if ((LISTS || a.hcnt) && lane == 0 && keep) {
-        const u32 nfree = __popcll(mk);
+        if (r < HALF_CAP) a.half[(u64)nd.v * HALF_CAP + r] = selfdel ? surv_encode(e, r, nfree) : e;
+    }
+    if (selfdel) {
+        if (nfree - 1u >= (u32)HALF_CAP && lane == 0 && keep) {
+            if (nfree == 0) a.half[(u64)nd.v * HALF_CAP] = SURV_NONE;
+            else {
+                const u32 idx = atomicAdd(a.n_wide, 1u);
+                if (idx < a.wide_cap) a.wide_list[idx] = nd.v;
+            }
+        }
+    } else if ((LISTS || a.hcnt) && lane == 0 && keep) {
         a.hcnt[nd.v] = nfree;
         if (nfree > HALF_CAP) {
             const u32 idx = atomicAdd(a.n_wide, 1u);
@@ -4034,9 +4049,45 @@
     OwnSet own;
 };
 
+struct EmitStage {
+    u64 *src, *ent;
+    u32 staged;
+    __device__ __forceinline__ void flush(u64 *bump, u64 *out_src, u64 *out_ent, u64 out_cap, u32 lane)
+    {
+        if (!staged) return;
+        __syncthreads();
+        u64 base = 0;
+        if (lane == 0) base = atomicAdd(bump, (u64)staged);
+        base = uniform_u64(base);
+        for (u32 i = lane; i < staged; i += 64)
+            if (base + i < out_cap) {
+                out_src[base + i] = src[i];
+                out_ent[base + i] = ent[i];
+            }
+        __syncthreads();
+        staged = 0;
+    }
+    __device__ __forceinline__ void append(u64 mk, bool keep, u64 v, u64 e, u64 *bump, u64 *out_src, u64 *out_ent, u64 out_cap, u32 lane)
+    {
+        const u32 kc = __popcll(mk);
+        if (!kc) return;
+        if (staged + kc > EMIT_CHUNK) flush(bump, out_src, out_ent, out_cap, lane);
+        if (keep) {
+            const u32 i = staged + rank_below(mk);
+            src[i] = v;
+            ent[i] = e;
+        }
+        staged += kc;
+    }
+};
+
+template <bool DENSE>
 __global__ void __launch_bounds__(64) emit_kernel(EmitArgs a)
 {
+    __shared__ u64 s_src[DENSE ? EMIT_CHUNK : 1], s_ent[DENSE ? EMIT_CHUNK : 1];
+    EmitStage st{s_src, s_ent, 0u};
     const u32 lane = threadIdx.x;
+    const bool selfdel = a.half && !a.hcnt;
     u64 chunk_base = 0;
     u32 chunk_used = EMIT_CHUNK;
     bool have_chunk = false;
@@ -4054,6 +4105,10 @@
         const u64 rv = a.ref[v];
         const u32 d = REF_DEG(rv);
         if (d == 0) continue;
+        if (selfdel) {
+            const u64 *hv = a.half + v * HALF_CAP;
+            if (surv_len(hv[0], hv[1], hv[2], hv[3]) <= HALF_CAP) continue;
+        }
         const u64 vs = REF_POS(rv);
         const u32 Lv = a.v.len[v];
         for (u32 s0 = 0; s0 < d; s0 += 64) {
@@ -4066,10 +4121,10 @@
                 if (v < w && !(e & ADJ_FLAG) && (!a.local_only || a.own.mine(w))) {
                     const u32 Lw = ADJ_DLEN(e);
                     const u64 twin = ADJ_MAKE(Lw + ADJ_OFF(e) - Lv, v, disco_twin_orient(ADJ_ORI(e)), Lv);
-                    const u32 cw = a.hcnt ? a.hcnt[w] : HALF_CAP + 1;
+                    const u64 *hw = a.half + w * HALF_CAP;
+                    const u32 cw = a.hcnt ? a.hcnt[w] : selfdel ? surv_len(hw[0], hw[1], hw[2], hw[3]) : HALF_CAP + 1;
                     if (cw <= HALF_CAP) {
-                        const u64 *hw = a.half + w * HALF_CAP;
-                        for (u32 r = 0; r < cw; r++) keep |= (hw[r] == twin);
+                        for (u32 r = 0; r < cw; r++) keep |= (surv_entry(hw[r]) == twin);
                     } else {
                         const u64 rw = a.ref[w];
                         const u64 *roww = a.adj + REF_POS(rw);
@@ -4079,6 +4134,10 @@
                 }
             }
             const u64 mk = __ballot(keep);
+            if (DENSE) {
+                st.append(mk, keep, v, e & ~ADJ_FLAG, a.bump, a.out_src, a.out_ent, a.out_cap, lane);
+                continue;
+            }
             const u32 cnt = __popcll(mk);
             if (cnt) {
                 if (chunk_used + cnt > EMIT_CHUNK) {
@@ -4100,7 +4159,8 @@
             }
         }
     }
-    close_chunk();
+    if (DENSE) st.flush(a.bump, a.out_src, a.out_ent, a.out_cap, lane);
+    else close_chunk();
 }
 
 struct EmitHalfArgs {
@@ -4184,6 +4244,47 @@
     close_chunk();
 }
 
+__global__ void __launch_bounds__(64) emit_half_lists_kernel(EmitHalfArgs a)
+{
+    __shared__ u64 s_src[EMIT_CHUNK], s_ent[EMIT_CHUNK];
+    EmitStage st{s_src, s_ent, 0u};
+    const u32 lane = threadIdx.x;
+    const u64 nq = a.own.count();
+    u64 cbeg = 0, cend = 0;
+    while (wq_grab(a.v.wq, (nq + 63) / 64, cbeg, cend))
+    for (u64 blk = cbeg; blk < cend; blk++) {
+        const bool live = blk * 64 + lane < nq;
+        const u64 v = a.order ? ORDER_ID(a.order[live ? blk * 64 + lane : 0]) : a.own.node_by_id(live ? blk * 64 + lane : 0);
+        const ulonglong2 *hv = (const ulonglong2 *)(a.half + v * HALF_CAP);
+        const ulonglong2 o0 = hv[0], o1 = hv[1];
+        const u64 rv = a.ref[v];
+        const u32 Lv = (u32)a.v.len[v];
+        const u64 own[HALF_CAP] = {o0.x, o0.y, o1.x, o1.y};
+        u32 cnt = (live && REF_DEG(rv) != 0) ? surv_len(own[0], own[1], own[2], own[3]) : 0u;
+        if (cnt > HALF_CAP) cnt = 0;
+#pragma unroll
+        for (u32 r = 0; r < HALF_CAP; r++) {
+            bool keep = false;
+            const u64 e = surv_entry(own[r]);
+            const u64 w = ADJ_DST(e);
+            if (r < cnt && v < w && (!a.local_only || a.own.otab || w < a.own.hi)) {
+                const u64 twin = ADJ_MAKE(ADJ_DLEN(e) + ADJ_OFF(e) - Lv, v, disco_twin_orient(ADJ_ORI(e)), Lv);
+                const ulonglong2 *hw = (const ulonglong2 *)(a.half + w * HALF_CAP);
+                const ulonglong2 h0 = hw[0], h1 = hw[1];
+                if (surv_len(h0.x, h0.y, h1.x, h1.y) <= HALF_CAP) keep = surv_has(h0.x, h0.y, h1.x, h1.y, twin);
+                else {
+                    const u64 rw = a.ref[w];
+                    const u64 *roww = a.adj + REF_POS(rw);
+                    const int ti = adj_find(roww, REF_DEG(rw), twin);
+                    keep = (ti >= 0) && !(roww[ti] & ADJ_FLAG);
+                }
+            }
+            st.append(__ballot(keep), keep, v, e, a.bump, a.out_src, a.out_ent, a.out_cap, lane);
+        }
+    }
+    st.flush(a.bump, a.out_src, a.out_ent, a.out_cap, lane);
+}
+
 __global__ void emit_valid_kernel(const u64 *__restrict__ out_src, u64 n, u8 *__restrict__ valid)
 {
     u64 i = (u64)blockIdx.x * blockDim.x + threadIdx.x;
@@ -4201,6 +4302,12 @@
         }
 }
 
+__global__ void emit_src32_kernel(const u64 *__restrict__ out_src, u64 n, u32 *__restrict__ dst_src)
+{
+    u64 i = (u64)blockIdx.x * blockDim.x + threadIdx.x;
+    for (; i < n; i += (u64)gridDim.x * blockDim.x) dst_src[i] = (u32)out_src[i];
+}
+
 __global__ void emit_compact_kernel(const u64 *__restrict__ out_src, const u64 *__restrict__ out_ent, const u8 *__restrict__ valid,
                                     const u64 *__restrict__ pos, u64 n, u64 *__restrict__ dst_src, u64 *__restrict__ dst_ent)
 {
@@ -4218,12 +4325,12 @@
 {
     u64 i = (u64)blockIdx.x * blockDim.x + threadIdx.x;
     for (; i < n; i += (u64)gridDim.x * blockDim.x)
-        if (valid[i]) {
+        if (!valid || valid[i]) {
             const u64 src = out_src[i], e = out_ent[i];
             const int l1 = (int)len[src], l2 = (int)ADJ_DLEN(e), off = (int)ADJ_OFF(e), ovl = l1 - off;
             const u32 o = ADJ_ORI(e);
             const u32 rev = (o == 1 || o == 2);
-            subs[pos[i]] = (u16)seg_mismatches<false>(reads + src * S, reads + ADJ_DST(e) * S, S, l2, o >= 2 ? off : 0, o >= 2 ? 0 : l2 - ovl, ovl, rev);
+            subs[pos ? pos[i] : i] = (u16)seg_mismatches<false>(reads + src * S, reads + ADJ_DST(e) * S, S, l2, o >= 2 ? off : 0, o >= 2 ? 0 : l2 - ovl, ovl, rev);
         }
 }
 
@@ -4250,7 +4357,7 @@
 {
     u64 i = (u64)blockIdx.x * blockDim.x + threadIdx.x;
     for (; i < n_slots; i += (u64)gridDim.x * blockDim.x) {
-        if (!valid[i]) continue;
+        if (valid && !valid[i]) continue;
         u32 a = (u32)out_src[i], b = (u32)ADJ_DST(out_ent[i]);
         for (;;) {
             a = uf_find(parent, a);
@@ -4287,7 +4394,7 @@
     __syncthreads();
     u64 i = (u64)blockIdx.x * blockDim.x + threadIdx.x;
     for (; i < n_slots; i += (u64)gridDim.x * blockDim.x)
-        if (valid[i]) {
+        if (!valid || valid[i]) {
             const u32 root = parent[(u32)out_src[i]];
             u32 idx = (root * 0x9E3779B1u) >> 22;
             bool placed = false;
@@ -4327,11 +4434,11 @@
 {
     u64 i = (u64)blockIdx.x * blockDim.x + threadIdx.x;
     for (; i < n_slots; i += (u64)gridDim.x * blockDim.x)
-        if (valid[i]) {
+        if (!valid || valid[i]) {
             const u32 r = parent[(u32)out_src[i]];
             u16 f = cfile[r];
             if (f == 0xFFFFu) f = (u16)(((u64)(r * 0x9E3779B1u) * n_files) >> 32);
-            edge_file[pos[i]] = f;
+            edge_file[pos ? pos[i] : i] = f;
         }
 }
 
diff --git a/disco_amd/csrc/disco_survivor.h b/disco_amd/csrc/disco_survivor.h
--- /dev/null
+++ b/disco_amd/csrc/disco_survivor.h
@@ -0,0 +1,31 @@
+#ifndef DISCO_SURVIVOR_H_
+#define DISCO_SURVIVOR_H_
+
+#if defined(__HIPCC__)
+#define SURV_HD __host__ __device__ __forceinline__
+#else
+#define SURV_HD inline
+#endif
+
+#define SURV_CAP 4
+#define SURV_WIDE (SURV_CAP + 1)
+#define SURV_LAST (1ull << 15)
+#define SURV_NONE SURV_LAST
+
+SURV_HD unsigned long long surv_encode(unsigned long long entry, unsigned r, unsigned n) { return (r + 1u == n) ? (entry | SURV_LAST) : entry; }
+SURV_HD unsigned long long surv_entry(unsigned long long slot) { return slot & ~SURV_LAST; }
+SURV_HD unsigned surv_len(unsigned long long s0, unsigned long long s1, unsigned long long s2, unsigned long long s3)
+{
+    if (s0 & SURV_LAST) return (s0 & 0x7FFFull) ? 1u : 0u;
+    if (s1 & SURV_LAST) return 2u;
+    if (s2 & SURV_LAST) return 3u;
+    if (s3 & SURV_LAST) return 4u;
+    return SURV_WIDE;
+}
+SURV_HD bool surv_has(unsigned long long s0, unsigned long long s1, unsigned long long s2, unsigned long long s3, unsigned long long twin)
+{
+    const bool e0 = (s0 & SURV_LAST) != 0, e1 = e0 || (s1 & SURV_LAST), e2 = e1 || (s2 & SURV_LAST), e3 = e2 || (s3 & SURV_LAST);
+    return e3 && ((surv_entry(s0) == twin) || (!e0 && surv_entry(s1) == twin) || (!e1 && surv_entry(s2) == twin) || (!e2 && surv_entry(s3) == twin));
+}
+
+#endif
diff --git a/disco_amd/csrc/disco_text.h b/disco_amd/csrc/disco_text.h
--- a/disco_amd/csrc/disco_text.h
+++ b/disco_amd/csrc/disco_text.h
@@ -52,9 +52,9 @@
 {
     u64 s = (u64)blockIdx.x * blockDim.x + threadIdx.x;
     for (; s < g.n_slots; s += (u64)gridDim.x * blockDim.x) {
-        if (!g.valid[s]) continue;
+        if (g.valid && !g.valid[s]) continue;
         const TextNumbers t = tx_numbers(g, s);
-        bytes[g.pos[s]] = (u8)(tx_digits(t.a) + tx_digits(t.b) + 1 + tx_digits(t.ovl) + tx_digits(t.len1) + tx_digits(t.off) + tx_digits(t.len1 - 1) + tx_digits(t.len2) +
+        bytes[g.pos ? g.pos[s] : s] = (u8)(tx_digits(t.a) + tx_digits(t.b) + 1 + tx_digits(t.ovl) + tx_digits(t.len1) + tx_digits(t.off) + tx_digits(t.len1 - 1) + tx_digits(t.len2) +
                                tx_digits(t.ovl - 1) + 20);
     }
 }
@@ -75,9 +75,9 @@
 {
     u64 s = (u64)blockIdx.x * blockDim.x + threadIdx.x;
     for (; s < g.n_slots; s += (u64)gridDim.x * blockDim.x) {
-        if (!g.valid[s]) continue;
+        if (g.valid && !g.valid[s]) continue;
         const TextNumbers t = tx_numbers(g, s);
-        char *p = text + place[g.pos[s]];
+        char *p = text + place[g.pos ? g.pos[s] : s];
         p = tx_put(p, t.a); *p++ = '\t';
         p = tx_put(p, t.b); *p++ = '\t';
         *p++ = (char)('0' + t.orient); *p++ = ',';
diff --git a/disco_amd/host/survivor_check.cpp b/disco_amd/host/survivor_check.cpp
--- /dev/null
+++ b/disco_amd/host/survivor_check.cpp
@@ -0,0 +1,80 @@
+#include <cstdint>
+#include <cstdio>
+#include <cstdlib>
+
+#include "../csrc/disco_survivor.h"
+
+typedef unsigned long long u64;
+
+static unsigned long checks = 0;
+#define CHECK(x)                                                          \
+    do {                                                                  \
+        ++checks;                                                         \
+        if (!(x)) {                                                       \
+            fprintf(stderr, "line %d: %s\n", __LINE__, #x);               \
+            return 1;                                                     \
+        }                                                                 \
+    } while (0)
+
+static u64 entry(u64 off, u64 dst, u64 o, u64 dlen) { return (off << 49) | (dst << 18) | (o << 16) | dlen; }
+
+static u64 rng_state = 0x9E3779B97F4A7C15ull;
+static u64 rnd()
+{
+    rng_state ^= rng_state << 7;
+    rng_state ^= rng_state >> 9;
+    return rng_state * 0x2545F4914F6CDD1Dull;
+}
+static u64 random_entry() { return entry(rnd() % 0x8000, rnd() % 0x80000000ull, rnd() & 3, 1 + rnd() % 0x7FFF); }
+
+int main()
+{
+    static_assert(SURV_CAP == 4, "four slots");
+    CHECK((SURV_NONE & 0x7FFFull) == 0 && surv_entry(SURV_NONE) == 0);
+    for (int round = 0; round < 20000; round++) {
+        u64 e[8];
+        for (u64 &x : e) x = random_entry();
+        for (unsigned i = 0; i < 8; i++) CHECK(!(e[i] & SURV_LAST));
+        const u64 other = random_entry();
+        for (unsigned n = 0; n <= 8; n++) {
+            u64 slot[SURV_CAP];
+            for (unsigned r = 0; r < SURV_CAP; r++) {
+                switch (rnd() % 5) {
+                case 0: slot[r] = random_entry(); break;
+                case 1: slot[r] = random_entry() | SURV_LAST; break;
+                case 2: slot[r] = SURV_NONE; break;
+                case 3: slot[r] = 0; break;
+                default: slot[r] = ~0ull; break;
+                }
+            }
+            for (unsigned r = 0; r < n && r < SURV_CAP; r++) slot[r] = surv_encode(e[r], r, n);
+            if (n == 0) slot[0] = SURV_NONE;
+            const unsigned len = surv_len(slot[0], slot[1], slot[2], slot[3]);
+            CHECK(len == (n <= SURV_CAP ? n : (unsigned)SURV_WIDE));
+            for (unsigned r = 0; r < n && r < SURV_CAP; r++) CHECK(surv_entry(slot[r]) == e[r]);
+            for (unsigned r = 0; r < 8; r++) {
+                const bool in_list = n <= SURV_CAP && r < n;
+                bool same_as_member = false;
+                for (unsigned q = 0; q < n && q < SURV_CAP; q++) same_as_member |= (e[q] == e[r]);
+                if (in_list) CHECK(surv_has(slot[0], slot[1], slot[2], slot[3], e[r]));
+                else if (n <= SURV_CAP && !same_as_member) CHECK(!surv_has(slot[0], slot[1], slot[2], slot[3], e[r]));
+                if (n > SURV_CAP) CHECK(!surv_has(slot[0], slot[1], slot[2], slot[3], e[r]));
+            }
+            if (n <= SURV_CAP) {
+                bool member = false;
+                for (unsigned q = 0; q < n; q++) member |= (e[q] == other);
+                CHECK(surv_has(slot[0], slot[1], slot[2], slot[3], other) == member);
+                for (unsigned r = n ? n : 1; r < SURV_CAP; r++) {
+                    u64 s2[SURV_CAP] = {slot[0], slot[1], slot[2], slot[3]};
+                    s2[r] = other;
+                    CHECK(surv_has(s2[0], s2[1], s2[2], s2[3], other) == member);
+                    s2[r] = other | SURV_LAST;
+                    CHECK(surv_has(s2[0], s2[1], s2[2], s2[3], other) == member);
+                    CHECK(surv_len(s2[0], s2[1], s2[2], s2[3]) == n);
+                }
+            }
+        }
+    }
+    printf("ok %lu checks\n", checks);
+    return 0;
+}
diff --git a/include/disco_hip_inspect.h b/include/disco_hip_inspect.h
--- a/include/disco_hip_inspect.h
+++ b/include/disco_hip_inspect.h
@@ -9,6 +9,8 @@
 
 int disco_fetch_order(disco_ctx *ctx, uint64_t *order_words, uint32_t *keys, uint64_t cap, uint64_t *n, int *order_bits);
 
+int disco_fetch_survivor_layout(disco_ctx *ctx, uint8_t *list_len, uint64_t cap, uint64_t *n, int *dense, uint64_t *out_used);
+
 #ifdef __cplusplus
 }
 #endif
```

Result: faster. 11.19 billion overlaps/s (median of 6 runs) (+2.0%).
